# weimengmeng1999/AdapterSIS

Hardware: AMD Instinct MI355X
Metric: training images/sec, ViT-L/14 588^2 adapter fine-tune (higher is better)
Workload: dtype f16; 1 GPU; vit_large/14 frozen + CAViT/CACNN adapters (n_last_blocks=4) + FeatureDecoder, 588x588, batch 12/GPU, reference_exact train.py step (fwd + decoder bwd + all-reduce + SGD), random-init weights; global_batch=12, image_size=588, parallelism=dp1, split_precision_convs=True, split_attn_out=False, precise_level=0, fold_attn_scale=True, fused_qkv=False, dead_cacnn_elided=True, c1_elided=True, ln_fold=True, mx_conv=True, mx_dense=True, conv_halo=True, fuse_cls_up=False, skipped_optimizer_steps=0

## Files before the change

adaptersis_amd/_lib.py:

```python
from __future__ import annotations

import ctypes as C
import os

_HERE = os.path.dirname(os.path.abspath(__file__))
LIB_PATH = os.path.join(_HERE, "lib", "libasis_hip.so")

ASIS_F16, ASIS_BF16, ASIS_F32 = 0, 1, 2
ASIS_EINVAL, ASIS_ELAUNCH = -1, -2
ACT_NONE, ACT_GELU, ACT_RELU, ACT_SILU_MUL, ACT_GELU_GRAD = 0, 1, 2, 3, 4


class AsisError(RuntimeError):
    pass


class GemmDesc(C.Structure):
    _fields_ = [
        ("A", C.c_void_p), ("B", C.c_void_p), ("C", C.c_void_p),
        ("lda", C.c_int64), ("ldb", C.c_int64), ("ldc", C.c_int64),
        ("strideA", C.c_int64), ("strideB", C.c_int64), ("strideC", C.c_int64),
        ("batch", C.c_int32), ("M", C.c_int32), ("N", C.c_int32), ("K", C.c_int32),
        ("bias_n", C.c_void_p), ("bias_m", C.c_void_p), ("scale_n", C.c_void_p), ("res", C.c_void_p),
        ("ldr", C.c_int64), ("strideR", C.c_int64),
        ("act", C.c_int32), ("out_f32", C.c_int32), ("dtype", C.c_int32),
        ("conv", C.c_int32),
        ("B_", C.c_int32), ("H", C.c_int32), ("W", C.c_int32), ("Cin", C.c_int32), ("OH", C.c_int32),
        ("OW", C.c_int32), ("KH", C.c_int32), ("KW", C.c_int32), ("stride", C.c_int32), ("pad", C.c_int32),
        ("stats", C.c_void_p),
        ("A_lo", C.c_void_p), ("B_lo", C.c_void_p),
        ("aux", C.c_void_p), ("ld_aux", C.c_int64),
        ("ksplit", C.c_int32),
        ("mx_amax_a", C.c_void_p), ("mx_amax_b", C.c_void_p),
        ("C_lo", C.c_void_p), ("rowstats", C.c_void_p), ("res16", C.c_void_p), ("res16_lo", C.c_void_p), ("ldr16", C.c_int64),
        ("ln_mr", C.c_void_p), ("ln_cs", C.c_void_p), ("ln_cols", C.c_int32),
    ]


class WgradDesc(C.Structure):
    _fields_ = [
        ("dy", C.c_void_p), ("x", C.c_void_p), ("out", C.c_void_p),
        ("ld_dy", C.c_int64), ("P", C.c_int64),
        ("dtype", C.c_int32), ("Cout", C.c_int32), ("CoP", C.c_int32), ("Cin", C.c_int32),
        ("B_", C.c_int32), ("H", C.c_int32), ("W", C.c_int32), ("OH", C.c_int32), ("OW", C.c_int32),
        ("KH", C.c_int32), ("KW", C.c_int32), ("stride", C.c_int32), ("pad", C.c_int32),
        ("splits", C.c_int32), ("k_per_split", C.c_int64),
    ]


_lib = None


def lib() -> C.CDLL:
    global _lib
    if _lib is not None:
        return _lib
    if not os.path.exists(LIB_PATH):
        raise AsisError(
            f"{LIB_PATH} is missing: build it with `python -m adaptersis_amd.build` "
            "(hipcc --offload-arch=gfx950). adaptersis_amd has no fallback path.")
    _lib = C.CDLL(LIB_PATH)
    _declare(_lib)
    _lib.asis_last_error.restype = _lib.asis_gemm_form_name.restype = C.c_char_p
    _lib.asis_lovasz_scratch_bytes.restype = _lib.asis_hardpixel_scratch_bytes.restype = C.c_int64
    _lib.asis_surface_quantile_scratch_bytes.restype = C.c_int64
    return _lib


_vp, _i, _i64, _f, _d = C.c_void_p, C.c_int, C.c_int64, C.c_float, C.c_double
SIGNATURES = {
    "asis_version": [],
    "asis_device_count": [],
    "asis_gemm": [_vp, C.POINTER(GemmDesc)],
    "asis_gemm_tiles_m": [_i],
    "asis_gemm_plan": [C.POINTER(GemmDesc), C.POINTER(_i), C.POINTER(_i), C.POINTER(_i), C.POINTER(_i)],
    "asis_gemm_form_name": [_i],
    "asis_absmax_f32": [_vp, _vp, _i64, _i, _i64, _vp, _i],
    "asis_bn_relu_absmax": [_vp, _vp, _vp, _vp, _i64, _i, _i, _vp],
    "asis_absmax_16": [_vp, _i, _vp, _i64, _i, _i64, _vp],
    "asis_conv3x3_halo_mx_tiles": [_i, _i, _i],
    "asis_conv3x3_halo_mx": [_vp, _i, _vp, _vp, _vp, _vp, _vp, _vp, _vp, _vp, _vp, _i, _i, _i, _i, _i],
    "asis_mx_from_pair": [_vp, _i, _vp, _vp, _i64, _vp, _i64, _i64, _i, _vp, _i],
    "asis_bn_relu_upsample_mx": [_vp, _i, _vp, _vp, _vp, _vp, _vp, _vp, _i, _i, _i, _i, _i],
    "asis_pack_conv_weight_mx": [_vp, _i, _vp, _vp, _i, _i, _i, _i, _i, _i64, _vp],
    "asis_pack_conv_weight_pair": [_vp, _i, _vp, _vp, _vp, _i, _i, _i, _i, _i, _i64, _vp],
    "asis_decoder_input_mx": [_vp, _i, _vp, _i64, _vp, _i64, _vp, _i64, _vp, _vp, _vp, _i, _i, _i, _i, _i, _i],
    "asis_ln_stats_finalize": [_vp, _vp, _i64, _i, _i, _f, _vp],
    "asis_split_stats": [_vp, _i, _vp, _i64, _vp, _vp, _i64, _vp, _i64, _i, _f],
    "asis_gemm_set_option": [C.c_char_p, _i],
    "asis_layernorm": [_vp, _i, _vp, _i64, _vp, _vp, _f, _vp, _i64, _i, _i64, _i],
    "asis_layernorm_mx": [_vp, _i, _vp, _i64, _vp, _vp, _f, _vp, _vp, _i64, _vp, _i64, _i],
    "asis_attention_fwd_seg": [_vp, _i, _vp, _vp, _i64, _vp, _i64, _vp, _i64, _i, _i, _i, _i, _i, _f, _vp],
    "asis_attention_fwd_split": [_vp, _i, _vp, _vp, _i64, _vp, _i64, _vp, _vp, _i64, _i, _i, _i, _i, _i, _f, _vp],
    "asis_attention_fwd_prescaled": [_vp, _i, _vp, _vp, _i64, _vp, _i64, _vp, _vp, _i64, _i, _i, _i, _i, _i, _vp],
    "asis_attention_fwd_qkv": [_vp, _i, _vp, _vp, _vp, _i64, _vp, _vp, _i64, _i, _i, _i, _i, _i, _f, _i, _vp],
    "asis_attention_fwd_qkv_mx": [_vp, _i, _vp, _vp, _vp, _i64, _vp, _vp, _i64, _i, _i, _i, _i, _i, _f, _i, _vp, _vp],
    "asis_attention_fwd_lse": [_vp, _i, _vp, _vp, _i64, _vp, _i64, _vp, _i64, _i, _i, _i, _f, _vp],
    "asis_transpose_tokens": [_vp, _i, _vp, _i64, _vp, _i64, _i, _i, _i],
    "asis_attention_bwd_rows": [_vp, _i, _vp, _vp, _vp, _i64, _vp, _i64, _vp, _i64, _vp, _vp, _vp, _vp, _vp, _i64, _i, _i, _i, _i,
                                _i, _f],
    "asis_msda_bwd": [_vp, _i, _vp, _vp, _i64, _vp, _vp, _vp, _vp, _vp, _vp, _i, _i, _i, _i, _i, _i, _i],
    "asis_msda_vgrad_cap": [_i, _i, _i],
    "asis_msda_value_grad": [_vp, _i, _vp, _i64, _vp, _vp, _vp, _vp, _vp, _vp, _vp, _vp, _vp, _i, _i, _i, _i, _i, _i, _i],
    "asis_msda_sampling_matrix": [_vp, _i, _vp, _i64, _vp, _vp, _vp, _vp, _i64, _i, _i, _i, _i, _i, _i],
    "asis_dwconv_bwd_nblk": [_i64],
    "asis_dwconv_gelu_bwd": [_vp, _i, _vp, _vp, _vp, _vp, _vp, _i, _vp, _vp, _vp, _vp, _i, _i, _i],
    "asis_rowblock_nblk": [_i64],
    "asis_layernorm_bwd": [_vp, _vp, _i64, _vp, _i64, _vp, _f, _vp, _i64, _vp, _i64, _vp, _i64, _i],
    "asis_gelu16": [_vp, _i, _vp, _vp, _vp, _i64],
    "asis_gelu_split": [_vp, _i, _vp, _vp, _vp, _i64],
    "asis_cast_colsum": [_vp, _i, _vp, _i64, _vp, _i64, _f, _vp, _i64, _i],
    "asis_layernorm_gather": [_vp, _i, _vp, _i64, _vp, _vp, _f, _vp, _i64, _vp, _i, _i, _i64, _i],
    "asis_scaled_index_add": [_vp, _vp, _i64, _vp, _i64, _vp, _i64, _vp, _i, _i, _i64, _i],
    "asis_gather_cast_colsum": [_vp, _i, _vp, _i64, _vp, _i64, _vp, _vp, _i, _i, _i64, _i],
    "asis_layernorm_bwd_scatter": [_vp, _vp, _i64, _vp, _i64, _vp, _f, _vp, _i64, _vp, _i64, _vp, _vp, _i, _i, _i64, _i64, _i],
    "asis_swiglu_bwd": [_vp, _i, _vp, _vp, _vp, _i64, _i],
    "asis_colsum": [_vp, _i, _vp, _i64, _vp, _i64, _i],
    "asis_ls_linear_finish": [_vp, _vp, _vp, _vp, _vp, _vp, _f, _vp, _vp, _vp, _i, _i],
    "asis_attention_fwd": [_vp, _i, _vp, _vp, _i64, _vp, _i64, _vp, _i64, _i, _i, _i, _f],
    "asis_im2col_patch": [_vp, _i, _vp, _i, _i, _i, _i, _vp, _i64],
    "asis_im2col_patch_split": [_vp, _i, _vp, _i, _i, _i, _i, _vp, _vp, _i64],
    "asis_cast_pad": [_vp, _i, _vp, _i64, _vp, _i64, _i64, _i, _f, _i],
    "asis_add_cls_pos": [_vp, _vp, _vp, _vp, _vp, _i, _i, _i],
    "asis_msda_fwd": [_vp, _i, _vp, _vp, _i64, _vp, _vp, _vp, _vp, _i, _i, _i, _i, _i, _i, _i],
    "asis_msda_fwd_split": [_vp, _i, _vp, _vp, _i64, _vp, _vp, _vp, _vp, _vp, _i, _i, _i, _i, _i, _i, _i],
    "asis_dwconv_gelu": [_vp, _i, _vp, _vp, _vp, _vp, _vp, _i, _vp, _i, _i, _i],
    "asis_conv3x3_c3": [_vp, _vp, _vp, _vp, _i, _i, _i, _i, _i, _i],
    "asis_conv3x3_smallcout_fwd": [_vp, _i, _vp, _vp, _vp, _vp, _vp, _i, _i, _i, _i, _i],
    "asis_conv3x3_smallcout_fwd_up": [_vp, _i, _vp, _vp, _vp, _vp, _vp, _vp, _i, _i, _i, _i, _i],
    "asis_conv3x3_smallcout_wgrad_up": [_vp, _i, _vp, _i, _vp, _vp, _vp, _vp, _i, _i, _i, _i, _i, _i],
    "asis_cls_lowres_nblk": [_i, _i, _i],
    "asis_cls_lowres_fwd": [_vp, _vp, _vp, _vp, _vp, _vp, _vp, _vp, _i, _i, _i, _i, _i],
    "asis_cls_lowres_bwd": [_vp, _i, _vp, _vp, _i, _vp, _vp, _vp, _vp, _vp, _vp, _vp, _vp, _vp, _i, _i, _i, _i, _i, _i],
    "asis_dgrad_lowres_nblk": [_i, _i, _i],
    "asis_dgrad_lowres_cap": [_i],
    "asis_dgrad_lowres_pack": [_vp, _i, _vp, _vp, _vp, _i, _i],
    "asis_dgrad_lowres": [_vp, _i, _vp, _vp, _vp, _vp, _vp, _vp, _vp, _vp, _vp, _vp, _vp, _i, _i, _i, _i, _i, _i],
    "asis_conv3x3_smallcout_dgrad": [_vp, _i, _vp, _vp, _i, _vp, _vp, _i, _i, _i, _i, _i],
    "asis_conv3x3_smallcout_wgrad": [_vp, _i, _vp, _i, _vp, _vp, _i, _i, _i, _i, _i, _i],
    "asis_colstats_nparts": [_i64],
    "asis_colstats": [_vp, _vp, _i64, _i, _vp],
    "asis_reduce_partials": [_vp, _vp, _i, _i, _vp],
    "asis_bn_finalize": [_vp, _vp, _d, _i, _vp, _vp, _f, _f, _vp, _vp, _vp, _vp, _vp, _vp, _vp],
    "asis_bn_eval_affine": [_vp, _vp, _vp, _vp, _vp, _f, _i, _vp, _vp],
    "asis_bn_act": [_vp, _i, _vp, _vp, _vp, _i, _vp, _vp, _i64, _i],
    "asis_bn_act_mx": [_vp, _i, _vp, _vp, _vp, _i, _vp, _vp, _vp, _i64, _i],
    "asis_bn_relu_maxpool": [_vp, _i, _vp, _vp, _vp, _vp, _vp, _i, _i, _i, _i],
    "asis_bn_relu_upsample": [_vp, _i, _vp, _vp, _vp, _vp, _vp, _i, _i, _i, _i, _i],
    "asis_pack_conv_weight": [_vp, _i, _vp, _vp, _i, _i, _i, _i, _i, _i64, _i],
    "asis_decoder_input": [_vp, _i, _vp, _i64, _vp, _i64, _vp, _i64, _vp, _vp, _i, _i, _i, _i, _i, _i],
    "asis_swiglu": [_vp, _i, _vp, _vp, _i64, _i],
    "asis_swiglu_split": [_vp, _i, _vp, _vp, _vp, _i64, _i],
    "asis_copy_channels": [_vp, _vp, _i64, _vp, _i64, _i64, _i64],
    "asis_add_f32": [_vp, _vp, _vp, _vp, _i64, _i, _i64, _i64, _i64],
    "asis_maxpool2_fwd": [_vp, _i, _vp, _vp, _vp, _vp, _vp, _i, _i, _i, _i],
    "asis_maxpool2_bwd": [_vp, _vp, _vp, _vp, _i, _i, _i, _i],
    "asis_cls_l2norm": [_vp, _vp, _vp, _vp, _i, _i, _i, _i],
    "asis_cls_l2norm_bwd": [_vp, _vp, _vp, _vp, _vp, _i, _i, _i, _i],
    "asis_mask_logits_fwd": [_vp, _vp, _vp, _vp, _vp, _f, _vp, _vp, _vp, _i, _i, _i, _i],
    "asis_mask_logits_nblk": [_i, _i],
    "asis_mask_logits_bwd": [_vp, _vp, _vp, _vp, _vp, _vp, _vp, _f, _vp, _vp, _vp, _i, _i, _i, _i],
    "asis_mask_dchat": [_vp, _vp, _vp, _vp, _vp, _i, _i, _i, _i],
    "asis_nearest_add_relu": [_vp, _i, _vp, _vp, _vp, _vp, _vp, _vp, _i, _i, _i, _i, _i, _i],
    "asis_nearest_sum": [_vp, _vp, _vp, _vp, _vp, _i, _i, _i, _i, _i, _i],
    "asis_convt2x2_scatter": [_vp, _i, _vp, _vp, _vp, _i, _i, _i, _i, _i, _i, _i, _i, _i, _i],
    "asis_convt2x2_gather": [_vp, _i, _vp, _vp, _vp, _i, _i, _i, _i, _i, _i, _i, _i, _i, _i],
    "asis_convt2x2_bias_nblk": [_i64],
    "asis_conv1x1_dgrad_small": [_vp, _i, _vp, _vp, _i64, _vp, _vp, _i64, _i, _i],
    "asis_convt2x2_bias_grad": [_vp, _vp, _vp, _i, _i, _i, _i, _i, _i, _i, _i, _i, _i],
    "asis_dice_nblk": [_i, _i],
    "asis_seg_loss_fwd": [_vp, _vp, _vp, _vp, _i, _i, _i, _i, _i, _i, _i, _i, _f, _i, _f, _vp, _vp, _vp, _vp],
    "asis_seg_loss_bwd": [_vp, _vp, _vp, _vp, _vp, _i, _i, _i, _i, _i, _i, _i, _i, _i, _vp],
    "asis_dice_fwd": [_vp, _vp, _vp, _i, _i, _i, _i, _i, _i, _i, _f, _i, _f, _vp, _vp, _vp, _vp],
    "asis_dice_bwd": [_vp, _vp, _vp, _vp, _i, _i, _i, _i, _i, _i, _i, _vp],
    "asis_ce_acc_nblk": [_i64],
    "asis_ce_acc_counts": [_vp, _vp, _vp, _vp, _i, _i, _i, _i, _i, _i, _vp, _vp],
    "asis_ce_acc": [_vp, _vp, _vp, _vp, _i, _i, _i, _i, _i, _i, _vp],
    "asis_resize_bilinear_fwd": [_vp, _vp, _i, _i, _i, _i, _i, _i, _vp],
    "asis_resize_bwd_nblk": [_i64],
    "asis_resize_bilinear_bwd": [_vp, _i, _vp, _i, _i, _i, _i, _i, _i, _i, _vp, _vp, _vp],
    "asis_reduce_rows": [_vp, _vp, _i, _i, _f, _vp],
    "asis_lovasz_tile": [],
    "asis_lovasz_scratch_bytes": [_i64, _i],
    "asis_lovasz_softmax": [_vp, _vp, _vp] + [_i] * 8 + [_f, _i] + [_vp] * 6,
    "asis_hardpixel_tile": [],
    "asis_hardpixel_scratch_bytes": [_i64],
    "asis_hardpixel_loss": [_vp] * 4 + [_i] * 8 + [_f, _f, _i64, _i, _f, _i] + [_vp] * 5,
    "asis_ew_blocks": [_i64],
    "asis_bn_bwd_nblk": [_i64, _i],
    "asis_maxpool_bn_relu_bwd": [_vp, _vp, _vp, _vp, _vp, _vp, _vp, _vp, _vp, _i, _i, _i, _i],
    "asis_dilate2": [_vp, _i, _vp, _vp, _vp, _vp, _i, _i, _i, _i, _i, _i],
    "asis_upsample_bn_relu_bwd": [_vp, _vp, _vp, _vp, _vp, _vp, _vp, _vp, _vp, _i, _i, _i, _i, _i],
    "asis_bn_bwd_apply": [_vp, _i, _vp, _vp, _vp, _vp, _vp, _vp, _vp, _d, _vp, _vp, _vp, _i64, _i],
    "asis_bn_bwd_apply_mx": [_vp, _i, _vp, _vp, _vp, _vp, _vp, _vp, _vp, _d, _vp, _vp, _vp, _vp, _i64, _i],
    "asis_bn_bwd_absmax": [_vp, _vp, _vp, _vp, _vp, _vp, _vp, _vp, _d, _vp, _i64, _i],
    "asis_wgrad_splits": [_i64, _i, _i],
    "asis_wgrad": [_vp, C.POINTER(WgradDesc)],
    "asis_conv3x3_wgrad_halo_nblk": [_i, _i, _i, _i, _i],
    "asis_conv3x3_wgrad_halo": [_vp, _i, _vp, _i64, _vp, _vp, _i, _i, _i, _i, _i, _i],
    "asis_lora_down": [_vp, _i, _vp, _i64, _i, _i, _i, _i, _vp, _vp, _i64, _i64],
    "asis_lora_wgrad_nblk": [_i64, _i],
    "asis_lora_wgrad": [_vp, _i, _vp, _i64, _vp, _i64, _i, _i, _i, _i, _vp, _i, _i64],
    "asis_sgd_momentum": [_vp, _vp, _vp, _vp, _i64, _f, _f, _f, _f, _i],
    "asis_augment": [_vp] * 13 + [_i, _i],
    "asis_augment_geo_u8": [_vp] * 12 + [_i, _i],
    "asis_clahe": [_vp] * 13 + [_i, _i, _i],
    "asis_nonrigid_map": [_vp] * 7 + [_i] + [_vp] * 3 + [_i, _i],
    "asis_nonrigid_remap": [_vp] * 6 + [_i, _i],
    "asis_frame_resize": [_vp] * 5 + [_i, _vp, _vp, _i] + [_vp] * 6 + [_i] * 5,
    "asis_predict_mask": [_vp, _vp] + [_i] * 6 + [_vp] * 9,
    "asis_predict_mask_views": [_vp] * 5 + [_i] * 5 + [_vp] * 10,
    "asis_predict_mask_tiles": [_vp] * 6 + [_i] * 4 + [_f] + [_i] * 4 + [_vp] * 10,
    "asis_surface_stats": [_vp] * 5 + [_i] * 6 + [_vp, _i] + [_vp] * 6 + [_i],
    "asis_surface_quantile_scratch_bytes": [_i, _i, _i],
    "asis_surface_quantiles": [_vp] * 4 + [_i] * 7 + [_vp, _i] + [_vp] * 3,
    "asis_dropout_f32": [_vp, _vp, _vp, _vp, _i64, C.c_uint64, _i, _f, _f, _vp, _i],
    "asis_dropout_t16": [_vp, _i, _vp, _vp, _i64, C.c_uint64, _i, _f, _i],
    "asis_dropout_mask": [_vp, _vp, _i64, C.c_uint64, _i, _f],
    "asis_softmax_dropout_fwd": [_vp, _i, _vp, _vp, _vp, _i64, _i, _i, _f, C.c_uint64, _i, _f],
    "asis_softmax_dropout_bwd": [_vp, _i, _vp, _vp, _vp, _vp, _i64, _i, _i, _f, C.c_uint64, _i, _f],
    "asis_grad_guard": [_vp, _vp, _i64, _vp, _i],
    "asis_sgd_momentum_guarded": [_vp, _vp, _vp, _vp, _i64, _f, _f, _f, _f, _i, _vp, _i],
    "asis_grad_sumsq_blocks": [_i64],
    "asis_grad_sumsq": [_vp, _vp, _i64, _vp],
    "asis_adamw_prepare": [_vp, _vp, _i, _vp, _vp, _f, _f, _d, _d],
    "asis_adamw_step": [_vp, _vp, _vp, _vp, _vp, _i64, _vp, _vp, _vp, _i, _d, _d, _d, _d, _f, _vp, _vp],
    "asis_scale_f32": [_vp, _vp, _i64, _f],
    "asis_zero": [_vp, _vp, _i64],
    "asis_grad_pack_bf16": [_vp, _vp, _i64, _vp],
    "asis_grad_unpack_bf16": [_vp, _vp, _i64, _vp],
}


def _declare(l: C.CDLL) -> None:
    for name, argtypes in SIGNATURES.items():
        fn = getattr(l, name)
        fn.argtypes = argtypes
        fn.restype = C.c_int


def check(rc: int, what: str = "") -> None:
    if rc == 0:
        return
# ... 5 lines not shown
```

adaptersis_amd/backbones/adapter_blocks.py:

```python
from __future__ import annotations

from functools import partial

import torch
import torch.nn as nn

from .. import config, ops
from ..dinov2.layers.blocks import _Packed
from .ops.modules import MSDeformAttn
from .ops.modules.ms_deform_attn import prepare_msda_geometry


def get_reference_points(spatial_shapes, device):
    reference_points_list = []
    for lvl, (H_, W_) in enumerate(spatial_shapes):
        ref_y, ref_x = torch.meshgrid(
            torch.linspace(0.5, H_ - 0.5, H_, dtype=torch.float32, device=device),
            torch.linspace(0.5, W_ - 0.5, W_, dtype=torch.float32, device=device), indexing="ij")
        ref_y = ref_y.reshape(-1)[None] / H_
        ref_x = ref_x.reshape(-1)[None] / W_
        reference_points_list.append(torch.stack((ref_x, ref_y), -1))
    reference_points = torch.cat(reference_points_list, 1)
    return reference_points[:, :, None]


def deform_inputs(x, patch_size, cnn_shapes=None):
    bs, c, h, w = x.shape
    if cnn_shapes is None:
        cnn_shapes = [(h // 8, w // 8), (h // 16, w // 16), (h // 32, w // 32)]
    cnn_shapes = [tuple(int(v) for v in s) for s in cnn_shapes]
    spatial_shapes = torch.as_tensor(cnn_shapes, dtype=torch.long, device=x.device)
    level_start_index = torch.cat((spatial_shapes.new_zeros((1,)), spatial_shapes.prod(1).cumsum(0)[:-1]))
    reference_points = get_reference_points([(h // patch_size, w // patch_size)], x.device)
    deform_inputs1 = [reference_points, spatial_shapes, level_start_index]
    spatial_shapes = torch.as_tensor([(h // patch_size, w // patch_size)], dtype=torch.long, device=x.device)
    level_start_index = torch.cat((spatial_shapes.new_zeros((1,)), spatial_shapes.prod(1).cumsum(0)[:-1]))
    reference_points = get_reference_points(cnn_shapes, x.device)
    deform_inputs2 = [reference_points, spatial_shapes, level_start_index]
    return deform_inputs1, deform_inputs2


class DWConv(nn.Module):

    def __init__(self, dim=768):
        super().__init__()
        self.dwconv = nn.Conv2d(dim, dim, 3, 1, 1, bias=True, groups=dim)


class ConvFFN(_Packed):

    def __init__(self, in_features, hidden_features=None, out_features=None, act_layer=nn.GELU, drop=0.0):
        super().__init__()
        if drop:
            raise ValueError("dropout is 0 on the AdapterSIS path (train.py:108)")
        out_features = out_features or in_features
        hidden_features = hidden_features or in_features
        if hidden_features % 8:
            raise ValueError("ConvFFN hidden width must be a multiple of 8")
        self.fc1 = nn.Linear(in_features, hidden_features)
        self.dwconv = DWConv(hidden_features)
        self.act = act_layer()
        self.fc2 = nn.Linear(hidden_features, out_features)

    def forward16(self, n16, res, B, Ntok, grids):
        dt = config.operand_dtype
        dev = n16.device
        hid = self.fc1.out_features
        h = ops.gemm(n16, self._w16("fc1", self.fc1.weight), out_f32=True, bias_n=self._f32("fc1_b", self.fc1.bias))
        key = ("grids", tuple(grids), dev)
        if self._cache.get("gkey") != key:
            sizes = [a * b for a, b in grids]
            starts = [0]
            for s in sizes[:-1]:
                starts.append(starts[-1] + s)
            self._cache["gshapes"] = torch.tensor(grids, dtype=torch.int32, device=dev)
            self._cache["gstarts"] = torch.tensor(starts, dtype=torch.int32, device=dev)
            self._cache["gkey"] = key
        w9 = self._f32_fn("dw9", self.dwconv.dwconv.weight, lambda p: p.reshape(hid, 9).t().contiguous().float())
        g = ops.dwconv_gelu(h.view(B, Ntok, hid), w9, self._f32("dwb", self.dwconv.dwconv.bias),
                            self._cache["gshapes"], self._cache["gstarts"], dt)
        return ops.gemm(g.view(B * Ntok, hid), self._w16("fc2", self.fc2.weight), out_f32=True,
                        bias_n=self._f32("fc2_b", self.fc2.bias), res=res)

    def _grid_tensors(self, grids, dev):
        key = ("grids", tuple(grids), dev)
        if self._cache.get("gkey") != key:
            sizes = [a * b for a, b in grids]
            starts = [0]
            for s in sizes[:-1]:
                starts.append(starts[-1] + s)
            self._cache["gshapes"] = torch.tensor(grids, dtype=torch.int32, device=dev)
            self._cache["gstarts"] = torch.tensor(starts, dtype=torch.int32, device=dev)
            self._cache["gkey"] = key
        return self._cache["gshapes"], self._cache["gstarts"]

    def forward16_train(self, n16, res, B, Ntok, grids):
        dt = config.operand_dtype
        hid = self.fc1.out_features
        h = ops.gemm(n16, self._w16("fc1", self.fc1.weight), out_f32=True, bias_n=self._f32("fc1_b", self.fc1.bias))
        gsh, gst = self._grid_tensors(grids, n16.device)
        w9 = self._f32_fn("dw9", self.dwconv.dwconv.weight, lambda p: p.reshape(hid, 9).t().contiguous().float())
        g = ops.dwconv_gelu(h.view(B, Ntok, hid), w9, self._f32("dwb", self.dwconv.dwconv.bias), gsh, gst, dt)
        out = ops.gemm(g.view(B * Ntok, hid), self._w16("fc2", self.fc2.weight), out_f32=True,
                       bias_n=self._f32("fc2_b", self.fc2.bias), res=res)
        return out, (n16, h, g, B, Ntok, tuple(grids))

    def backward16(self, saved, dout, inv_scale, grads, prefix):
        n16, h, g, B, Ntok, grids = saved
        dt = config.operand_dtype
        hid = self.fc1.out_features
        pre = prefix + "."
        d16, cs = ops.cast_colsum(dout, dt)
        self._linear_bwd(pre + "fc2", self.fc2, None, None, d16, cs, g.view(B * Ntok, hid), inv_scale, grads)
        dg = ops.gemm(d16, self._wT16("fc2T", self.fc2.weight), out_f32=True)
        gsh, gst = self._grid_tensors(grids, dout.device)
        w9 = self._f32_fn("dw9", self.dwconv.dwconv.weight, lambda p: p.reshape(hid, 9).t().contiguous().float())
        dh16, part = ops.dwconv_gelu_bwd(h.view(B, Ntok, hid), w9, self._f32("dwb", self.dwconv.dwconv.bias), gsh, gst,
                                         dg.view(B, Ntok, hid), dt)
        red = ops.reduce_rows(part.view(part.shape[0], 10 * hid), inv_scale).view(10, hid)
        grads[pre + "dwconv.dwconv.weight"].view(hid, 9).copy_(red[:9].t())
        grads[pre + "dwconv.dwconv.bias"].copy_(red[9])
        dh2 = dh16.view(B * Ntok, hid)
        self._linear_bwd(pre + "fc1", self.fc1, None, None, dh2, ops.colsum(dh2), n16, inv_scale, grads)
        return ops.gemm(dh2, self._wT16("fc1T", self.fc1.weight), out_f32=True)

    def _f32_fn(self, key, param, fn):
        from ..dinov2.layers.blocks import _pack
        return _pack(self._cache, key, param, fn)


class _AdapterBase(_Packed):
    def _ln16(self, name, x2d):
        ln = getattr(self, name)
        return ops.layernorm(x2d, self._f32(name + "_w", ln.weight), self._f32(name + "_b", ln.bias), ln.eps,
                             config.operand_dtype)

    def _ln_bwd(self, name, dy, x2d, inv_scale, grads, prefix, res=None):
        ln = getattr(self, name)
        D = x2d.shape[1]
        dx, part = ops.layernorm_bwd(dy, x2d, self._f32(name + "_w", ln.weight), ln.eps, res=res)
        red = ops.reduce_rows(part.view(part.shape[0], 2 * D), inv_scale)
        grads[f"{prefix}{name}.weight"].copy_(red[:D]); grads[f"{prefix}{name}.bias"].copy_(red[D:])
        return dx

    @staticmethod
    def _flat(x):
        B, N, D = x.shape
        x2 = x.reshape(B * N, D)
        if x2.dtype != torch.float32 or not x2.is_contiguous():
            x2 = x2.float().contiguous()
        return x2, B, N, D


class CACNN(_AdapterBase):
    def __init__(self, dim, num_heads=6, n_points=4, n_levels=1, deform_ratio=1.0, with_cffn=True, cffn_ratio=0.25,
                 drop=0.0, drop_path=0.0, norm_layer=partial(nn.LayerNorm, eps=1e-6), with_cp=False):
        super().__init__()
        if drop or drop_path:
            raise ValueError("drop / drop_path are 0 on the AdapterSIS path (train.py:108-109)")
        self.query_norm = norm_layer(dim)
        self.feat_norm = norm_layer(dim)
        self.attn = MSDeformAttn(d_model=dim, n_levels=n_levels, n_heads=num_heads, n_points=n_points, ratio=deform_ratio)
        self.with_cffn = with_cffn
        self.with_cp = with_cp
        if with_cffn:
            self.ffn = ConvFFN(in_features=dim, hidden_features=int(dim * cffn_ratio), drop=drop)
            self.ffn_norm = norm_layer(dim)
            self.drop_path = nn.Identity()

    def forward(self, query, reference_points, feat, spatial_shapes, level_start_index, H, W, grids=None):
        q2, B, Lq, D = self._flat(query)
        f2, _, Lin, _ = self._flat(feat)
        assert int((spatial_shapes[:, 0] * spatial_shapes[:, 1]).sum()) == Lin
        ref, shapes_i32, starts_i32 = prepare_msda_geometry(reference_points, spatial_shapes, level_start_index, Lq,
                                                            query.device)
        out = self.attn.forward16(self._ln16("query_norm", q2), self._ln16("feat_norm", f2), ref, shapes_i32,
                                  starts_i32, B, Lq, Lin, res=q2)
        if self.with_cffn:
            if grids is None:
                grids = [(H * 2 + 1, W * 2 + 1), (H, W), (H // 2, W // 2)]
            grids = [tuple(int(v) for v in g) for g in grids]
            if sum(a * b for a, b in grids) != Lq:
                raise ValueError(f"CACNN: token grids {grids} do not cover {Lq} tokens; pass grids= explicitly")
            out = self.ffn.forward16(self._ln16("ffn_norm", out), out, B, Lq, grids)
        return out.view(B, Lq, D)


    def forward16_train(self, c2, x2, g, B, Lq, Lin, grids):
        qn, fn = self._ln16("query_norm", c2), self._ln16("feat_norm", x2)
        out1, s_attn = self.attn.forward16_train(qn, fn, g["ref2"], g["shapes2"], g["starts2"], B, Lq, Lin, res=c2)
        s_ffn = None
        out = out1
        if self.with_cffn:
            out, s_ffn = self.ffn.forward16_train(self._ln16("ffn_norm", out1), out1, B, Lq, grids)
        return out, (c2, x2, out1, s_attn, s_ffn)

    def backward16(self, saved, dout, inv_scale, grads, prefix=""):
        c2, x2, out1, s_attn, s_ffn = saved
        pre = prefix + "." if prefix else ""
        d1 = dout
        if self.with_cffn:
            dn = self.ffn.backward16(s_ffn, dout, inv_scale, grads, pre + "ffn")
            d1 = self._ln_bwd("ffn_norm", dn, out1, inv_scale, grads, pre, res=dout)
        dq, dfeat = self.attn.backward16(s_attn, d1, inv_scale, grads, pre + "attn")
        dc = self._ln_bwd("query_norm", dq, c2, inv_scale, grads, pre, res=d1)
        dx = self._ln_bwd("feat_norm", dfeat, x2, inv_scale, grads, pre)
        return dc, dx


class CAViT(_AdapterBase):
    def __init__(self, dim, num_heads=6, n_points=4, n_levels=1, deform_ratio=1.0,
                 norm_layer=partial(nn.LayerNorm, eps=1e-6), init_values=0.0, with_cp=False):
        super().__init__()
        self.with_cp = with_cp
        self.query_norm = norm_layer(dim)
        self.feat_norm = norm_layer(dim)
        self.attn = MSDeformAttn(d_model=dim, n_levels=n_levels, n_heads=num_heads, n_points=n_points, ratio=deform_ratio)
        self.gamma = nn.Parameter(init_values * torch.ones((dim)), requires_grad=True)

    def forward(self, query, reference_points, feat, spatial_shapes, level_start_index):
        q2, B, Lq, D = self._flat(query)
        f2, _, Lin, _ = self._flat(feat)
        assert int((spatial_shapes[:, 0] * spatial_shapes[:, 1]).sum()) == Lin
        ref, shapes_i32, starts_i32 = prepare_msda_geometry(reference_points, spatial_shapes, level_start_index, Lq,
                                                            query.device)
        out = self.attn.forward16(self._ln16("query_norm", q2), self._ln16("feat_norm", f2), ref, shapes_i32,
                                  starts_i32, B, Lq, Lin, res=q2, scale_n=self._f32("gamma", self.gamma))
        return out.view(B, Lq, D)

    def forward16_train(self, x2, c2, g, B, Lq, Lin):
        qn, fn = self._ln16("query_norm", x2), self._ln16("feat_norm", c2)
        out, s_attn = self.attn.forward16_train(qn, fn, g["ref1"], g["shapes1"], g["starts1"], B, Lq, Lin, res=x2,
                                                scale_n=self._f32("gamma", self.gamma))
        return out, (x2, c2, s_attn)

    def backward16(self, saved, dout, inv_scale, grads, prefix=""):
        x2, c2, s_attn = saved
        pre = prefix + "." if prefix else ""
        dq, dfeat = self.attn.backward16(s_attn, dout, inv_scale, grads, pre + "attn", gamma=self.gamma,
                                         gamma_name=pre + "gamma")
        dx = self._ln_bwd("query_norm", dq, x2, inv_scale, grads, pre, res=dout)
        dc = self._ln_bwd("feat_norm", dfeat, c2, inv_scale, grads, pre)
        return dx, dc
```

adaptersis_amd/backbones/engines.py:

```python
from __future__ import annotations

import contextlib
import os
from typing import Dict, List, Optional, Sequence, Tuple

import torch
import torch.distributed as dist
from torch import nn

from .. import config, ops
from .. import lora as lora_mod
from ..dinov2.layers.blocks import _Packed, _pack, run_blocks
from ..droppath import DropPathSampler
from ..optim import SGD, AdamW, FlatBucket
from ..parallel import StageReducer, world_size
from .adapter_blocks import CACNN, CAViT, deform_inputs


class pre_vit(_Packed):

    def __init__(self, img_size=84, patch_size=14, in_chans=256, embed_dim=384, norm_layer=None, flatten_embedding=True):
        super().__init__()
        if norm_layer is not None:
            raise ValueError("pre_vit: norm_layer is never set in the reference")
        self.img_size, self.patch_size = img_size, patch_size
        self.patches_resolution = (img_size // patch_size, img_size // patch_size)
        self.num_patches = self.patches_resolution[0] * self.patches_resolution[1]
        self.in_chans, self.embed_dim, self.flatten_embedding = in_chans, embed_dim, flatten_embedding
        self.proj = nn.Conv2d(in_chans, embed_dim, kernel_size=patch_size, stride=patch_size)
        self.norm = nn.Identity()

    def forward(self, x):
        B, C, H, W = x.shape
        P = self.patch_size
        assert H % P == 0, f"Input image height {H} is not a multiple of patch height {P}"
        assert W % P == 0, f"Input image width {W} is not a multiple of patch width: {P}"
        dt = config.operand_dtype
        x16 = ops.cast_pad(x.permute(0, 2, 3, 1).contiguous().float().view(B * H * W, C), C, dt).view(B, H, W, C)
        w16 = _pack(self._cache, "w", self.proj.weight, lambda p: ops.pack_conv_weight(p.float().contiguous(), 0, dt))
        out = ops.conv_gemm(x16, w16, P, P, P, 0, bias_n=self._f32("b", self.proj.bias))
        out = out.view(B, (H // P) * (W // P), self.embed_dim)
        if not self.flatten_embedding:
            out = out.reshape(-1, H // P, W // P, self.embed_dim)
        return out


def _loss_scratch(engine, attr: str, need: int, device) -> torch.Tensor:
    scratch = getattr(engine, attr, None)
    if scratch is None or scratch.numel() < need or scratch.device != device:
        scratch = torch.empty((need,), device=device, dtype=torch.uint8)
        setattr(engine, attr, scratch)
    return scratch


def loss_and_dz(engine, logits: torch.Tensor, target: torch.Tensor, S: float):
    n_region, lmode, eps, n_ce = SegEngine.LOSSES[engine.loss_kind]
    if lmode not in (ops.LOSS_LOVASZ, ops.LOSS_TOPK, ops.LOSS_FOCAL):
        loss, coef, _ = ops.seg_loss_fwd(logits, target, n_region, lmode, eps, n_ce, None, S)
        return loss, ops.seg_loss_bwd(logits, target, coef, n_region, lmode, n_ce, None)
    if lmode != ops.LOSS_LOVASZ:
        N = target.numel()
        scratch = _loss_scratch(engine, "_hardpixel_scratch", ops.hardpixel_scratch_bytes(N), logits.device)
        if lmode == ops.LOSS_FOCAL:
            return ops.hardpixel_loss(logits, target, ops.HARDPIXEL_FOCAL, N, n_softmax=n_region,
                                      gamma=getattr(engine, "focal_gamma", 2.0), grad_scale=S, scratch=scratch)
        K = int(N * getattr(engine, "topk_percent", 10.0) / 100)
        if K < 1:
            raise ValueError(f"topk_percent selects no pixel of {N}")
        dz, dc = None, None
        if n_region:
            dc, coef, _ = ops.seg_loss_fwd(logits, target, n_region, ops.LOSS_SOFTDICE, eps, 0, None, S)
            dz = ops.seg_loss_bwd(logits, target, coef, n_region, ops.LOSS_SOFTDICE, 0, None)
        loss, dz = ops.hardpixel_loss(logits, target, ops.HARDPIXEL_CE, K, grad_scale=S, dz=dz, scratch=scratch)
        return (loss if dc is None else dc.add_(loss)), dz
    scratch = _loss_scratch(engine, "_lovasz_scratch", ops.lovasz_scratch_bytes(target.numel(), logits.shape[-1]), logits.device)
    dz, ce = None, None
    if n_ce:
        ce, coef, _ = ops.seg_loss_fwd(logits, target, 0, ops.LOSS_NONE, eps, n_ce, None, S)
        dz = ops.seg_loss_bwd(logits, target, coef, 0, ops.LOSS_NONE, n_ce, None)
    loss, _, dz = ops.lovasz_softmax(logits, target, n_region, "mean", S, dz=dz, scratch=scratch)
    return (loss if ce is None else ce.add_(loss)), dz


class SegEngine(nn.Module):

    LOSSES = {
        "dice": (2, ops.LOSS_DICE, 10e-20, 0),
        "iou": (2, ops.LOSS_IOU, 1e-6, 0),
        "softdice": (1, ops.LOSS_SOFTDICE, 1.0, 0),
        "dc_and_ce": (1, ops.LOSS_SOFTDICE, 1.0, 2),
        "tversky": (1, ops.LOSS_TVERSKY, 1.0, 0),
        "ce_dc": (1, ops.LOSS_DICE, 10e-20, 1),
        "lovasz": (1, ops.LOSS_LOVASZ, 0.0, 0),
        "ce_lovasz": (1, ops.LOSS_LOVASZ, 0.0, 1),
        "topk": (0, ops.LOSS_TOPK, 0.0, 0),
        "dc_and_topk": (1, ops.LOSS_TOPK, 1.0, 0),
        "focal": (1, ops.LOSS_FOCAL, 0.0, 0),
    }

    def __init__(self, model, backbone_encoder, cross_vit: CAViT, cross_cnn: CACNN, seg_decoder, *,
                 n_last_blocks: int = 4, num_classes: int = 2, lr: float = 0.01, momentum: float = 0.99,
                 weight_decay: float = 3e-5, mode: str = "reference_exact", process_group=None, loss: str = "dice",
                 train_encoder: bool = False, train_backbone: bool = False, optimize_backbone: bool = False,
                 blocks_per_bucket: int = 4, grad_compress: Optional[str] = None, optimizer: str = "sgd",
                 betas=(0.9, 0.999), eps: float = 1e-8, clip_grad: Optional[float] = None, no_decay: bool = True,
                 layer_decay: Optional[float] = None, topk_percent: float = 10.0, focal_gamma: float = 2.0,
                 drop_path_seed: int = 0, lora_rank: Optional[int] = None, lora_alpha: Optional[float] = None):
        super().__init__()
        if grad_compress is None:
            grad_compress = os.environ.get("ASIS_GRAD_COMPRESS", "bf16").lower()
        if grad_compress in ("", "0", "none", "off", "fp32"):
            grad_compress = None
        if mode not in ("reference_exact", "train_adapters"):
            raise ValueError("mode must be 'reference_exact' or 'train_adapters'")
        if loss not in self.LOSSES:
            raise ValueError(f"loss must be one of {sorted(self.LOSSES)}")
        self.loss_kind = loss
        if not 0.0 < topk_percent <= 100.0:
            raise ValueError("topk_percent must be in (0, 100]")
        if focal_gamma < 0.0:
            raise ValueError("focal_gamma must be >= 0")
        self.topk_percent, self.focal_gamma = float(topk_percent), float(focal_gamma)
        self.is_mla = type(seg_decoder).__name__ == "DecoderMLA"
        self.stream_only = type(seg_decoder).__name__ == "UNet"
        self.model, self.backbone_encoder = model, backbone_encoder
        self.cross_vit, self.cross_cnn, self.seg_decoder = cross_vit, cross_cnn, seg_decoder
        self.n_last_blocks, self.num_classes, self.mode = n_last_blocks, num_classes, mode
        self.patch = model.patch_size
        self.heads = model.num_heads
        self.process_group = process_group
        if train_encoder and mode != "train_adapters":
            raise ValueError("train_encoder needs mode='train_adapters'")
        self.train_encoder = train_encoder
        frozen = list(model.parameters()) + ([] if train_encoder else list(backbone_encoder.parameters()))
        if mode == "reference_exact":
            frozen += list(cross_vit.parameters()) + list(cross_cnn.parameters())
        for p in frozen:
            p.requires_grad_(False)
        order = list(seg_decoder.GRAD_ORDER)
        named = dict(seg_decoder.named_parameters())
        ordered = [(n, named[n]) for pre in order for n in named if n.startswith(pre + ".")]
        assert len(ordered) == len(named)
        self.bucket = FlatBucket(ordered)
        self.stage_ranges = [self.bucket.range_of([n for n in named if n.startswith(pre + ".")]) for pre in order]
        buckets = [self.bucket]
        self.adapter_bucket = None
        if mode == "train_adapters":
            if type(seg_decoder).__name__ not in ("FeatureDecoder", "DecoderSETR", "UNet", "DecoderMLA"):
                raise NotImplementedError("train_adapters is built for the train.py adapter flow (FeatureDecoder / UNet heads) and "
                                          "the train_mla.py flow (DecoderMLA)")
            if self.is_mla and train_backbone:
                raise NotImplementedError("the train_mla.py flow trains decoder + adapters (+ encoder); the unfrozen backbone "
                                          "(BASELINE config 4) is the train.py adapter flow")
            for p in list(cross_vit.parameters()) + list(cross_cnn.parameters()):
                p.requires_grad_(True)
            named_a = [("cross_vit." + n, p) for n, p in cross_vit.named_parameters()] + \
                      [("cross_cnn." + n, p) for n, p in cross_cnn.named_parameters()]
            self.adapter_bucket = FlatBucket(named_a)
            self.adapter_reducer = StageReducer(self.adapter_bucket.grad, [(0, self.adapter_bucket.numel)], process_group)
            buckets.append(self.adapter_bucket)
            self.encoder_bucket = None
            if train_encoder:
                for p in backbone_encoder.parameters():
                    p.requires_grad_(True)
                self.encoder_bucket = FlatBucket([("backbone_encoder." + n, p) for n, p in backbone_encoder.named_parameters()])
                self.encoder_reducer = StageReducer(self.encoder_bucket.grad, [(0, self.encoder_bucket.numel)], process_group)
                buckets.append(self.encoder_bucket)
        self.train_backbone = bool(train_backbone)
        self.split_attn_out = config.split_attn_out_policy if config.split_attn_out_policy is not None else \
            bool(self.stream_only or self.is_mla or train_backbone)
        self.precise_level = config.precise_level_policy if config.precise_level_policy is not None else \
            (2 if (self.is_mla and len(model.blocks) >= 40) else 0)
        all_parts = frozenset(("qkv", "proj", "fc1", "fc2"))
        self.precise_parts = config.precise_parts_policy if config.precise_parts_policy is not None else \
            (frozenset(("proj", "fc1")) if (config.precise_level_policy is None and self.precise_level == 2) else all_parts)
        self.vit_bucket = None
        self.lora = self.lora_bucket = None
        if lora_rank is None and lora_alpha is not None:
            raise ValueError("lora_alpha needs lora_rank")
        if lora_rank is not None:
            lora_mod.check_engine_args(mode=mode, train_backbone=train_backbone, optimize_backbone=optimize_backbone,
                                       layer_decay=layer_decay, is_mla=self.is_mla, model=model, rank=lora_rank)
            self.lora = lora_mod.LoRA(model, lora_rank, lora_alpha)
            self.lora_bucket = FlatBucket(list(self.lora.named_parameters()))
            self.vit_reducer = StageReducer(self.lora_bucket.grad, [(0, self.lora_bucket.numel)], process_group)
            self._fire_at = [0]
            buckets.append(self.lora_bucket)
        elif train_backbone:
            if mode != "train_adapters":
                raise ValueError("train_backbone needs mode='train_adapters' (the unfrozen variant of the adapter flow)")
            self.vit_bucket, self.vit_reducer, self._fire_at = make_vit_bucket(model, blocks_per_bucket, process_group,
                                                                               momentum=optimize_backbone,
                                                                               min_first_blocks=n_last_blocks,
                                                                               compress=grad_compress)
            if optimize_backbone:
                buckets.append(self.vit_bucket)
        if layer_decay is not None and not (train_backbone and optimize_backbone):
            raise ValueError("layer_decay scales the learning rates of the ViT blocks: it needs train_backbone and optimize_backbone")
        self.drop_path = make_drop_path_sampler(model, drop_path_seed, process_group)
        if self.drop_path is not None and not train_backbone:
            raise ValueError("drop_path_rate drops samples in the training forward of the ViT blocks: it needs train_backbone")
        self.optimizer = make_optimizer(optimizer, buckets, lr=lr, momentum=momentum, weight_decay=weight_decay, betas=betas, eps=eps,
                                        clip_grad=clip_grad, no_decay=no_decay, depth=len(model.blocks),
                                        layer_decay=[layer_decay if b is self.vit_bucket else None for b in buckets])
        self.reducer = StageReducer(self.bucket.grad, self.stage_ranges, process_group)
        self._geom = {}

    def _geometry(self, H, W, shapes, dev):
        key = (H, W, tuple(shapes), dev)
        g = self._geom.get(key)
        if g is None:
            d1, d2 = deform_inputs(torch.zeros(1, 3, H, W), self.patch, shapes)
            g = {"ref1": d1[0][0, :, 0, :].contiguous().to(dev), "shapes1": d1[1].to(torch.int32).to(dev),
                 "starts1": d1[2].to(torch.int32).to(dev), "ref2": d2[0][0, :, 0, :].contiguous().to(dev),
                 "shapes2": d2[1].to(torch.int32).to(dev), "starts2": d2[2].to(torch.int32).to(dev)}
            self._geom = {key: g}
        return g

    def _encoder_on_side_stream(self, inp: torch.Tensor):
        main = torch.cuda.current_stream()
        if getattr(self, "_enc_stream", None) is None:
            self._enc_stream = torch.cuda.Stream()
        side = self._enc_stream
        side.wait_stream(main)
        with torch.cuda.stream(side):
            _, c, shapes = self.backbone_encoder.forward_tokens(inp, need_c1=not config.elide_c1)
            done = torch.cuda.Event()
            done.record(side)
        c.record_stream(main)
        return c, shapes, done

    def _trunk_dual(self, xcat: torch.Tensor, Ra: int, blocks, segs) -> torch.Tensor:
        main = torch.cuda.current_stream()
        nper = 2 if config.trunk_streams >= 4 and min(b for b, _ in segs) >= 2 else 1
        if getattr(self, "_dual_streams", None) is None or len(self._dual_streams) != 2 * nper:
            self._dual_streams = tuple(torch.cuda.Stream() for _ in range(2 * nper))
        parts = []
        r0 = 0
        for (B, N) in segs:
            cuts = [0, B] if nper == 1 else [0, B // 2, B]
            for a, b in zip(cuts[:-1], cuts[1:]):
                parts.append((slice(r0 + a * N, r0 + b * N), [(b - a, N)]))
            r0 += B * N
        xs = []
        for st, (sl, _) in zip(self._dual_streams, parts):
            st.wait_stream(main)
            xcat.record_stream(st)
            xs.append(xcat[sl])
        nblk = len(blocks)
        for bi, blk in enumerate(blocks):
            for i, (st, (_, sg)) in enumerate(zip(self._dual_streams, parts)):
                with torch.cuda.stream(st):
                    R_i = xs[i][0].shape[0] if isinstance(xs[i], tuple) else xs[i].shape[0]
                    if blk.fold_ok(R_i, sg):
                        xs[i] = blk.forward_rows_fold(xs[i], sg, planes_out=bi + 1 < nblk and blocks[bi + 1].fold_ok(R_i, sg))
                    else:
                        xs[i] = blk.forward_rows(xs[i], sg)
        for st, x in zip(self._dual_streams, xs):
            main.wait_stream(st)
            x.record_stream(main)
        return torch.cat(xs, 0)

    def _cavit(self, x2, c2, g, B, Lq, Lin):
        cv = self.cross_vit
        return cv.attn.forward16(cv._ln16("query_norm", x2), cv._ln16("feat_norm", c2), g["ref1"], g["shapes1"],
                                 g["starts1"], B, Lq, Lin, res=x2, scale_n=cv._f32("gamma", cv.gamma))

    def _cacnn(self, c2, x2, g, B, Lq, Lin, grids):
        cn = self.cross_cnn
        out = cn.attn.forward16(cn._ln16("query_norm", c2), cn._ln16("feat_norm", x2), g["ref2"], g["shapes2"],
                                g["starts2"], B, Lq, Lin, res=c2)
        return cn.ffn.forward16(cn._ln16("ffn_norm", out), out, B, Lq, grids) if cn.with_cffn else out

    @torch.no_grad()
    def features(self, inp: torch.Tensor, taps: Optional[dict] = None, adapter_saves: Optional[list] = None):
        config.split_attn_out = self.split_attn_out
        config.precise_level = self.precise_level
        config.precise_parts = self.precise_parts
        m = self.model
        B, _, H, W = inp.shape
        inp = inp.float().contiguous()
        D = m.embed_dim
        h, w = H // self.patch, W // self.patch
        N = h * w
        nb = len(m.blocks)
        nl = self.n_last_blocks
        enc_done = None
        if self.train_encoder and adapter_saves is not None:
            c, shapes, esaved = self.backbone_encoder.forward_tokens_train(inp)
            self._esaved = (esaved, shapes)
        elif config.encoder_stream and inp.is_cuda:
            c, shapes, enc_done = self._encoder_on_side_stream(inp)
        else:
            _, c, shapes = self.backbone_encoder.forward_tokens(inp, need_c1=not config.elide_c1)
        c_orig = c
        Lc = c.shape[1]
        g = self._geometry(H, W, shapes, inp.device)
        Ra, Rb = B * (N + 1), B * N
        segs = [(B, N + 1), (B, N)]
        xcat = torch.empty((Ra + Rb, D), device=inp.device, dtype=torch.float32)
        tokens, _ = m.patch_embed.tokens(inp, out=xcat[Ra:])
        if not config.share_patch_embed:
            tokens, _ = m.patch_embed.tokens(inp)
        pos = m._pos_for(N, H, W)
        ops.add_cls_pos(tokens, m.cls_token.detach().reshape(-1).float().contiguous(),
                        pos.detach().reshape(-1, D).float().contiguous(), out=xcat[:Ra].view(B, N + 1, D))
        feats = []
        trunk = list(m.blocks[: nb - (nl - 1)])
        if config.dual_stream and inp.is_cuda and getattr(self, "_dual_warm", False) and nb - nl == len(trunk) - 1:
            xcat = self._trunk_dual(xcat, Ra, trunk, segs)
            feats.append(m._final_norm(xcat[:Ra].view(B, N + 1, D))[:, 1:])
            trunk = []
        self._dual_warm = True
        if trunk:
            assert nb - nl == len(trunk) - 1
            xcat = run_blocks(trunk, xcat, segs)
            feats.append(m._final_norm(xcat[:Ra].view(B, N + 1, D))[:, 1:])
        if enc_done is not None:
            torch.cuda.current_stream().wait_event(enc_done)
        if taps is not None:
            taps.update(c=c, x_b0=xcat[Ra:].view(B, N, D).clone(), shapes=shapes)
        c2d = c.view(B * Lc, D)
        train = self.mode == "train_adapters" and adapter_saves is not None
        for s in range(nl):
            bsaved = None
            if s > 0:
                blk = m.blocks[nb - (nl - 1) + s - 1]
                if train:
                    xa_s = blk.forward_rows(xcat[:Ra], [(B, N + 1)])
                    xb_s, bsaved = blk.forward_train(xcat[Ra:].view(B, N, D))
                    xcat = torch.cat([xa_s, xb_s.reshape(Rb, D)], 0)
                else:
                    xcat = run_blocks([blk], xcat, segs)
                feats.append(m._final_norm(xcat[:Ra].view(B, N + 1, D))[:, 1:])
            dead = s == nl - 1 and taps is None and config.elide_dead_cacnn
            if train:
                x2, s_cv = self.cross_vit.forward16_train(xcat[Ra:].clone(), c2d, g, B, N, Lc)
                s_cn = None
                if not dead:
                    c2d, s_cn = self.cross_cnn.forward16_train(c2d, x2, g, B, Lc, N, shapes)
                adapter_saves.append((bsaved, s_cv, s_cn))
            else:
                x2 = self._cavit(xcat[Ra:], c2d, g, B, N, Lc)
                if not dead:
                    c2d = self._cacnn(c2d, x2, g, B, Lc, N, shapes)
            x = ops.add_f32(x2.view(B, N, D), feats[s], out=xcat[Ra:].view(B, N, D))
        if taps is not None:
            taps.update(feats=feats)
        if self.stream_only:
            xs = x.reshape(B * N, D)
            hi = ops.cast_pad(xs, D, config.operand_dtype).view(B, h, w, D)
            lo = ops.cast_pad(xs, D, config.operand_dtype, part=1).view(B, h, w, D) if config.split_conv else None
            if taps is not None:
                taps.update(x_final=x, c_final=c2d.view(B, Lc, D), cat=hi)
            return hi, lo
        n4 = shapes[2][0] * shapes[2][1]
        d1 = getattr(self.seg_decoder, "decoder_1", None)
        mx = bool(config.mx_conv_on() and config.split_conv and d1 is not None and "d1" not in config.unsplit_layers and
                  ops.mx_conv_ok(B * h * w, 3 * D, d1[0].out_channels))
        cat = ops.decoder_input(x, c_orig[:, Lc - n4:], feats[-1], (h, w), shapes[2], config.operand_dtype,
                                config.split_conv, mx=mx)
        if not config.split_conv:
            cat = (cat, None)
        if taps is not None:
            taps.update(x_final=x, c_final=c2d.view(B, Lc, D), cat=cat[0])
        return cat

    @torch.no_grad()
    def features_mla(self, inp: torch.Tensor, taps: Optional[dict] = None, adapter_saves: Optional[list] = None):
        config.split_attn_out = self.split_attn_out
        config.precise_level = self.precise_level
        config.precise_parts = self.precise_parts
        m = self.model
        B, _, H, W = inp.shape
        inp = inp.float().contiguous()
        D = m.embed_dim
        h, w = H // self.patch, W // self.patch
        N = h * w
        nb = len(m.blocks)
        train = self.mode == "train_adapters" and adapter_saves is not None
        if train and self.train_encoder:
            c, shapes, esaved = self.backbone_encoder.forward_tokens_train(inp)
            self._esaved = (esaved, shapes)
        else:
            _, c, shapes = self.backbone_encoder.forward_tokens(inp, need_c1=not config.elide_c1)
        Lc = c.shape[1]
        g = self._geometry(H, W, shapes, inp.device)
        tokens = m.patch_embed(inp)
        if not config.share_patch_embed:
            m.patch_embed(inp)
        xa = ops.add_cls_pos(tokens, m.cls_token.detach().reshape(-1).float().contiguous(),
                             m._pos_for(N, H, W).detach().reshape(-1, D).float().contiguous())
        Ra = B * (N + 1)
        segs = [(B, N + 1), (B, N)]
        xcat = torch.cat([xa.view(Ra, D), tokens.reshape(B * N, D)], 0)
        xcat = run_blocks(list(m.blocks[: nb - 3]), xcat, segs)
        c2d = c.view(B * Lc, D)
        if train:
            x2, s_cv = self.cross_vit.forward16_train(xcat[Ra:].clone(), c2d, g, B, N, Lc)
            adapter_saves.append((None, s_cv, None))
        else:
            x2 = self._cavit(xcat[Ra:], c2d, g, B, N, Lc)
        outs = [x2]
        for j, bi in enumerate((nb - 3, nb - 2, nb - 2)):
            bsaved = None
            if train:
                if j < 2:
                    xa_s = m.blocks[bi].forward_rows(xcat[:Ra], [(B, N + 1)])
                    xb_s, bsaved = m.blocks[bi].forward_train(x2.view(B, N, D))
                    xcat = torch.cat([xa_s, xb_s.reshape(B * N, D)], 0)
                    x2 = xcat[Ra:]
                else:
                    xb_s, bsaved = m.blocks[bi].forward_train(x2.view(B, N, D))
                    x2 = xb_s.reshape(B * N, D)
            elif j < 2:
                xcat[Ra:].copy_(x2)
                xcat = m.blocks[bi].forward_rows(xcat, segs)
                x2 = xcat[Ra:]
            else:
                x2 = m.blocks[bi](x2.view(B, N, D)).view(B * N, D)
            if train:
                c2d, s_cn = self.cross_cnn.forward16_train(c2d, x2.contiguous(), g, B, Lc, N, shapes)
                x2, s_cv = self.cross_vit.forward16_train(x2.clone(), c2d, g, B, N, Lc)
                adapter_saves.append((bsaved, s_cv, s_cn))
            else:
                c2d = self._cacnn(c2d, x2, g, B, Lc, N, shapes)
                x2 = self._cavit(x2, c2d, g, B, N, Lc)
            outs.append(x2)
        xa = m.blocks[nb - 1](xcat[:Ra].view(B, N + 1, D))
        vit_last = m._final_norm(xa)[:, 1:]
        last = ops.add_f32(outs[3].view(B, N, D), vit_last)
        maps = [last.view(B * N, D), outs[2], outs[1], outs[0]]
        dt = config.operand_dtype
        res = []
        for t in maps:
            hi = ops.cast_pad(t, D, dt).view(B, h, w, D)
            lo = ops.cast_pad(t, D, dt, part=1).view(B, h, w, D) if config.split_conv else None
            res.append((hi, lo))
        if taps is not None:
            taps.update(mla_inputs=[t.view(B, N, D) for t in maps])
        return res

    @torch.no_grad()
    def train_step(self, inp: torch.Tensor, target: torch.Tensor, taps: Optional[dict] = None) -> torch.Tensor:
        dec = self.seg_decoder
        S = config.loss_scale
        asaves = None
        if self.is_mla:
            asaves = [] if self.mode == "train_adapters" else None
            logits, saved = dec._forward_core(self.features_mla(inp, taps, asaves), save=True, training=True)
        elif self.train_backbone:
            cat, e2e = self._features_e2e(inp, taps)
            if self.stream_only:
                logits, saved = dec._forward_core(cat[0], cat[1], save=True, training=True, need_input_grad=True)
            else:
                logits, saved = dec._forward_core(cat[0], cat[1], save=True, training=True)
        else:
            asaves = [] if self.mode == "train_adapters" else None
            cat = self.features(inp, taps, asaves)
            if self.stream_only and asaves is not None:
                logits, saved = dec._forward_core(cat[0], cat[1], save=True, training=True, need_input_grad=True)
            else:
                logits, saved = dec._forward_core(cat[0], cat[1], save=True, training=True)
        target = target.long().contiguous()
        loss, dz = loss_and_dz(self, logits, target, S)
        B, hh, ww, C = logits.shape
        r = ops.resize_bilinear_bwd(dz, hh, ww, config.operand_dtype, config.split_conv)
        d16, d_lo, bpart = r if config.split_conv else (r[0], None, r[1])
        world = world_size(self.process_group)
        inv = 1.0 / (S * world)
        self.reducer.begin()
        if self.mode == "train_adapters" and self.is_mla:
            dmaps = dec._backward_core(saved, d16, bpart, inv, self.bucket.views, stage_done=self.reducer.stage_done, d_lo=d_lo,
                                       need_input_grad=True)
            self.adapter_reducer.begin()
            dc0 = self._mla_adapter_backward(asaves, dmaps, inv)
            self.adapter_reducer.stage_done()
            if self.train_encoder:
                self.encoder_reducer.begin()
                self._encoder_backward(dc0, None, inv)
                self.encoder_reducer.stage_done()
                self.encoder_reducer.finish()
            self.adapter_reducer.finish()
        elif self.mode == "train_adapters":
            dcat = dec._backward_core(saved, d16, bpart, inv, self.bucket.views, stage_done=self.reducer.stage_done, d_lo=d_lo,
                                      need_input_grad=True)
            if self.stream_only and (self.train_backbone or self.train_encoder):
                Bq, hq, wq, Dq = dcat.shape
                full = ops.zeros((Bq, hq, wq, 3 * Dq), dcat.device, dcat.dtype)
                ops.copy_channels(dcat.view(-1, Dq), full.view(-1, 3 * Dq)[:, :Dq])
                dcat = full
            self.adapter_reducer.begin()
            if self.train_backbone:
                self.vit_reducer.begin()
                if self.train_encoder:
                    self.encoder_reducer.begin()
                self._e2e_backward(e2e, dcat, inv)
                self.vit_reducer.finish()
                if self.train_encoder:
                    self.encoder_reducer.finish()
                self.adapter_reducer.finish()
                self.reducer.finish()
                self.optimizer.step(1.0)
                if taps is not None:
                    taps.update(logits=logits, loss=loss)
                return loss.view(())
            dc0 = self._adapter_backward(asaves, dcat, inv)
            self.adapter_reducer.stage_done()
            if self.train_encoder:
                self.encoder_reducer.begin()
                self._encoder_backward(dc0, dcat, inv)
                self.encoder_reducer.stage_done()
                self.encoder_reducer.finish()
            self.adapter_reducer.finish()
        else:
            dec._backward_core(saved, d16, bpart, inv, self.bucket.views, stage_done=self.reducer.stage_done, d_lo=d_lo)
        self.reducer.finish()
        self.optimizer.step(1.0)
        if taps is not None:
            taps.update(logits=logits, loss=loss)
        return loss.view(())

    @torch.no_grad()
    def _features_e2e(self, inp: torch.Tensor, taps: Optional[dict] = None):
        config.split_attn_out = self.split_attn_out
        config.precise_level = self.precise_level
        config.precise_parts = self.precise_parts
        m = self.model
        B, _, H, W = inp.shape
        inp = inp.float().contiguous()
        D = m.embed_dim
        h, w = H // self.patch, W // self.patch
        N = h * w
        nb, nl = len(m.blocks), self.n_last_blocks
        if self.train_encoder:
            c, shapes, esaved = self.backbone_encoder.forward_tokens_train(inp)
            self._esaved = (esaved, shapes)
        else:
            _, c, shapes = self.backbone_encoder.forward_tokens(inp, need_c1=not config.elide_c1)
        c_orig = c
        Lc = c.shape[1]
        g = self._geometry(H, W, shapes, inp.device)
        tokens, a16 = m.patch_tokens_train(inp)
        xa = ops.add_cls_pos(tokens, m.cls_token.detach().reshape(-1).float().contiguous(),
                             m._pos_for(N, H, W).detach().reshape(-1, D).float().contiguous())
        Ra, Rb = B * (N + 1), B * N
        segs = [(B, N + 1), (B, N)]
        xcat = torch.cat([xa.view(Ra, D), tokens.reshape(Rb, D)], 0)
        bsaves, feats, fin, asaves = [], [], [], []
        keeps = self.drop_path.step(segs, inp.device) if self.drop_path is not None else [None] * nb
        blk_train = lambda j, xin: m.blocks[j].forward_train_rows(xin, segs) if keeps[j] is None else \
            m.blocks[j].forward_train_rows(xin, segs, keep=keeps[j])
        for i, blk in enumerate(m.blocks[: nb - (nl - 1)]):
            xcat, sv = blk_train(i, xcat)
            bsaves.append(sv)
            if i >= nb - nl:
                feats.append(m._final_norm(xcat[:Ra].view(B, N + 1, D))[:, 1:])
                fin.append(xcat)
        if taps is not None:
            taps.update(c=c, x_b0=xcat[Ra:].view(B, N, D).clone(), shapes=shapes)
        c2d = c.view(B * Lc, D)
        for s in range(nl):
            if s > 0:
                xcat, sv = blk_train(nb - nl + s, xcat)
                bsaves.append(sv)
                feats.append(m._final_norm(xcat[:Ra].view(B, N + 1, D))[:, 1:])
                fin.append(xcat)
            dead = s == nl - 1 and taps is None and config.elide_dead_cacnn
            x2, s_cv = self.cross_vit.forward16_train(xcat[Ra:].clone(), c2d, g, B, N, Lc)
            s_cn = None
            if not dead:
                c2d, s_cn = self.cross_cnn.forward16_train(c2d, x2, g, B, Lc, N, shapes)
            asaves.append((s_cv, s_cn))
            x = ops.add_f32(x2.view(B, N, D), feats[s], out=xcat[Ra:].view(B, N, D))
        if taps is not None:
            taps.update(feats=feats)
        if self.stream_only:
            xs = x.reshape(B * N, D)
            hi = ops.cast_pad(xs, D, config.operand_dtype).view(B, h, w, D)
            lo = ops.cast_pad(xs, D, config.operand_dtype, part=1).view(B, h, w, D) if config.split_conv else None
# ... 337 lines not shown
```

adaptersis_amd/config.py:

```python
import os

import torch

operand_dtype = torch.bfloat16 if os.environ.get("ASIS_OPERAND", "f16").lower() in ("bf16", "bfloat16") else torch.float16
loss_scale = float(os.environ.get("ASIS_LOSS_SCALE", 65536.0 if operand_dtype == torch.float16 else 1.0))


def set_operand_dtype(dt: torch.dtype) -> None:
    global operand_dtype
    if dt not in (torch.float16, torch.bfloat16):
        raise ValueError("operand dtype must be float16 or bfloat16")
    operand_dtype = dt

split_conv = os.environ.get("ASIS_SPLIT_CONV", "1") != "0"

precise_attention = os.environ.get("ASIS_PRECISE", "0") not in ("0", "")
fold_attn_scale = os.environ.get("ASIS_FOLD_SCALE", "1") not in ("0", "")
fused_qkv = os.environ.get("ASIS_FUSED_QKV", "0") not in ("0", "")

encoder_stream = os.environ.get("ASIS_ENC_STREAM", "1") not in ("0", "")

vt_stream = os.environ.get("ASIS_VT_STREAM", "1") not in ("0", "")

wgrad_stream = os.environ.get("ASIS_WGRAD_STREAM", "1") not in ("0", "")

unsplit_layers = set(filter(None, os.environ.get("ASIS_UNSPLIT", "").split(",")))

dual_stream = os.environ.get("ASIS_DUAL_STREAM", "1") not in ("0", "")

attn_rows = os.environ.get("ASIS_ATTN_ROWS", "1") != "0"

_so = os.environ.get("ASIS_SPLIT_O", "auto").lower()
split_attn_out_policy = None if _so == "auto" else (_so not in ("0", ""))
split_attn_out = bool(split_attn_out_policy)

_pl = os.environ.get("ASIS_PRECISE_LEVEL", "auto").lower() or "auto"
precise_level_policy = None if _pl == "auto" else int(_pl)
precise_level = int(precise_level_policy or 0)
_pa = os.environ.get("ASIS_PRECISE_ADAPTERS", "auto").lower() or "auto"


def precise_adapters_on() -> bool:
    if _pa != "auto":
        return _pa not in ("0", "")
    return operand_dtype == torch.bfloat16 and precise_level >= 2


_pp = os.environ.get("ASIS_PRECISE_PARTS", "auto").lower() or "auto"
precise_parts_policy = None if _pp == "auto" else frozenset(filter(None, _pp.replace("w12", "fc1").replace("w3", "fc2").split(",")))
precise_parts = precise_parts_policy if precise_parts_policy is not None else frozenset(("qkv", "proj", "fc1", "fc2"))
trunk_streams = int(os.environ.get("ASIS_TRUNK_STREAMS", "2") or 2)

elide_dead_cacnn = os.environ.get("ASIS_ELIDE_DEAD_CACNN", "1") not in ("0", "")
elide_c1 = os.environ.get("ASIS_ELIDE_C1", "1") not in ("0", "")
share_patch_embed = os.environ.get("ASIS_SHARE_PATCH_EMBED", "1") not in ("0", "")

ln_fold = os.environ.get("ASIS_LN_FOLD", "1") not in ("0", "")

_mx = os.environ.get("ASIS_MX_CONV", "1")
mx_conv_all = _mx == "2"
mx_conv = _mx not in ("0", "")


def mx_conv_on() -> bool:
    return mx_conv and (mx_conv_all or operand_dtype == torch.float16)


mx_dense = os.environ.get("ASIS_MX_DENSE", "1") not in ("0", "")


def mx_dense_on() -> bool:
    return mx_dense and operand_dtype == torch.float16

_DGRAD_LOWRES_ALL = ("d2", "d3", "d4")


def parse_dgrad_lowres(v: str) -> frozenset:
    v = (v or "").strip().lower()
    if v in ("", "0"):
        return frozenset()
    if v == "1":
        return frozenset(_DGRAD_LOWRES_ALL)
    keys = [k.strip() for k in v.split(",") if k.strip()]
    bad = [k for k in keys if k not in _DGRAD_LOWRES_ALL]
    if bad:
        raise ValueError(f"ASIS_DGRAD_LOWRES={v!r}: expected 0, 1 or a list of {', '.join(_DGRAD_LOWRES_ALL)} (unknown: {', '.join(bad)})")
    return frozenset(keys)


dgrad_lowres = parse_dgrad_lowres(os.environ.get("ASIS_DGRAD_LOWRES", "1"))
```

adaptersis_amd/csrc/core.hip:

```cpp
#include <stdarg.h>

#include "asis_common.h"

static thread_local char g_err[512] = "";

extern "C" void asis_set_error_(const char* fmt, ...) {
  va_list ap;
  va_start(ap, fmt);
  vsnprintf(g_err, sizeof(g_err), fmt, ap);
  va_end(ap);
}

extern "C" const char* asis_last_error(void) { return g_err; }
extern "C" int asis_version(void) { return 100; }

extern "C" int asis_device_count(void) {
  int n = 0;
  hipError_t e = hipGetDeviceCount(&n);
  if (e != hipSuccess) {
    asis_set_error_("hipGetDeviceCount: %s", hipGetErrorString(e));
    (void)hipGetLastError();
    return ASIS_ELAUNCH;
  }
  return n;
}
```

adaptersis_amd/csrc/norm.hip:

```cpp
#include "asis_common.h"
#include "row_routines.h"

namespace {

template <typename T, bool OUT_F32>
__global__ __launch_bounds__(256) void layernorm_kernel(const float* __restrict__ x, int64_t ldx,
                                                        const float* __restrict__ w, const float* __restrict__ b,
                                                        float eps, void* __restrict__ y, int64_t ldy, int64_t rows,
                                                        int D) {
  const int lane = threadIdx.x & 63;
  const int64_t row = (int64_t)blockIdx.x * 4 + (threadIdx.x >> 6);
  if (row >= rows) return;
  if (OUT_F32) ln_row<T, true>(x + row * ldx, w, b, eps, reinterpret_cast<float*>(y) + row * ldy, D, lane);
  else ln_row<T, false>(x + row * ldx, w, b, eps, reinterpret_cast<T*>(y) + row * ldy, D, lane);
}

template <typename T, bool OUT_F32, int NCH, int RPW>
__global__ __launch_bounds__(256) void layernorm_fixed_kernel(const float* __restrict__ x, int64_t ldx,
                                                              const float* __restrict__ w, const float* __restrict__ b,
                                                              float eps, void* __restrict__ y, int64_t ldy,
                                                              int64_t rows) {
  constexpr int D = 256 * NCH;
  const int lane = threadIdx.x & 63;
  const int64_t row0 = ((int64_t)blockIdx.x * 4 + (threadIdx.x >> 6)) * RPW;
  if (row0 >= rows) return;
  float4 v[RPW][NCH];
#pragma unroll
  for (int r = 0; r < RPW; ++r) {
    const int64_t row = row0 + r < rows ? row0 + r : rows - 1;
    const float4* xr = reinterpret_cast<const float4*>(x + row * ldx);
#pragma unroll
    for (int i = 0; i < NCH; ++i) v[r][i] = xr[lane + 64 * i];
  }
  float4 ww[NCH], bb[NCH];
#pragma unroll
  for (int i = 0; i < NCH; ++i) {
    ww[i] = reinterpret_cast<const float4*>(w)[lane + 64 * i];
    bb[i] = reinterpret_cast<const float4*>(b)[lane + 64 * i];
  }
  float mean[RPW], rstd[RPW];
#pragma unroll
  for (int r = 0; r < RPW; ++r) {
    float s = 0.f;
#pragma unroll
    for (int i = 0; i < NCH; ++i) s += (v[r][i].x + v[r][i].y) + (v[r][i].z + v[r][i].w);
    mean[r] = s;
  }
#pragma unroll
  for (int r = 0; r < RPW; ++r) mean[r] = wave_sum(mean[r]) / (float)D;
#pragma unroll
  for (int r = 0; r < RPW; ++r) {
    float q = 0.f;
#pragma unroll
    for (int i = 0; i < NCH; ++i) {
      const float a0 = v[r][i].x - mean[r], a1 = v[r][i].y - mean[r], a2 = v[r][i].z - mean[r],
                  a3 = v[r][i].w - mean[r];
      q += (a0 * a0 + a1 * a1) + (a2 * a2 + a3 * a3);
    }
    rstd[r] = q;
  }
#pragma unroll
  for (int r = 0; r < RPW; ++r) rstd[r] = 1.0f / sqrtf(wave_sum(rstd[r]) / (float)D + eps);
#pragma unroll
  for (int r = 0; r < RPW; ++r) {
    const int64_t row = row0 + r;
    if (row >= rows) break;
#pragma unroll
    for (int i = 0; i < NCH; ++i) {
      const int c = lane + 64 * i;
      const float o0 = (v[r][i].x - mean[r]) * rstd[r] * ww[i].x + bb[i].x;
      const float o1 = (v[r][i].y - mean[r]) * rstd[r] * ww[i].y + bb[i].y;
      const float o2 = (v[r][i].z - mean[r]) * rstd[r] * ww[i].z + bb[i].z;
      const float o3 = (v[r][i].w - mean[r]) * rstd[r] * ww[i].w + bb[i].w;
      if (OUT_F32) {
        reinterpret_cast<float4*>(reinterpret_cast<float*>(y) + row * ldy)[c] = make_float4(o0, o1, o2, o3);
      } else {
        uint2 p;
        p.x = pack2<T>(o0, o1);
        p.y = pack2<T>(o2, o3);
        reinterpret_cast<uint2*>(reinterpret_cast<T*>(y) + row * ldy)[c] = p;
      }
    }
  }
}

__global__ __launch_bounds__(256) void add_cls_pos_kernel(const float4* __restrict__ x, const float4* __restrict__ cls,
                                                          const float4* __restrict__ pos, float4* __restrict__ out,
                                                          int B, int N, int D4) {
  const int64_t total = (int64_t)B * (N + 1) * D4;
  for (int64_t i = (int64_t)blockIdx.x * blockDim.x + threadIdx.x; i < total; i += (int64_t)gridDim.x * blockDim.x) {
    const int c = (int)(i % D4);
    const int64_t r = i / D4;
    const int t = (int)(r % (N + 1));
    const int b = (int)(r / (N + 1));
    const float4 p = pos[(int64_t)t * D4 + c];
    const float4 a = (t == 0) ? cls[c] : x[((int64_t)b * N + (t - 1)) * D4 + c];
    out[i] = make_float4(a.x + p.x, a.y + p.y, a.z + p.z, a.w + p.w);
  }
}

template <typename T>
__global__ __launch_bounds__(256) void cast_pad_kernel(const float* __restrict__ src, int64_t ld_src,
                                                       T* __restrict__ dst, int64_t ld_dst, int64_t rows, int cols, float scale, int part) {
  const int cpr = (int)(ld_dst >> 3);
  const int64_t total = rows * cpr;
  for (int64_t i = (int64_t)blockIdx.x * blockDim.x + threadIdx.x; i < total; i += (int64_t)gridDim.x * blockDim.x) {
    const int64_t r = i / cpr;
    const int c0 = (int)(i - r * cpr) * 8;
    float f[8];
#pragma unroll
    for (int j = 0; j < 8; ++j) {
      f[j] = (c0 + j < cols) ? src[r * ld_src + c0 + j] * scale : 0.f;
      if (part) f[j] = lo_part<T>(f[j]);
    }
    uint4 p;
    p.x = pack2<T>(f[0], f[1]);
    p.y = pack2<T>(f[2], f[3]);
    p.z = pack2<T>(f[4], f[5]);
    p.w = pack2<T>(f[6], f[7]);
    *reinterpret_cast<uint4*>(dst + r * ld_dst + c0) = p;
  }
}

template <typename T>
__global__ __launch_bounds__(256) void im2col_patch_kernel(const float* __restrict__ img, int B, int Himg, int Wimg,
                                                           int P, T* __restrict__ out, int64_t ldk, T* __restrict__ out_lo) {
  const int gh = Himg / P, gw = Wimg / P;
  const int cpr = (int)(ldk >> 3);
  const int K = 3 * P * P;
  const int64_t total = (int64_t)B * gh * gw * cpr;
  for (int64_t i = (int64_t)blockIdx.x * blockDim.x + threadIdx.x; i < total; i += (int64_t)gridDim.x * blockDim.x) {
    const int64_t r = i / cpr;
    const int k0 = (int)(i - r * cpr) * 8;
    const int pw = (int)(r % gw);
    const int ph = (int)((r / gw) % gh);
    const int b = (int)(r / ((int64_t)gw * gh));
    float f[8];
#pragma unroll
    for (int j = 0; j < 8; ++j) {
      const int k = k0 + j;
      float v = 0.f;
      if (k < K) {
        const int c = k / (P * P);
        const int rem = k - c * P * P;
        const int ii = rem / P, jj = rem - ii * P;
        v = img[(((int64_t)b * 3 + c) * Himg + (ph * P + ii)) * Wimg + pw * P + jj];
      }
      f[j] = v;
    }
    uint4 p;
    p.x = pack2<T>(f[0], f[1]);
    p.y = pack2<T>(f[2], f[3]);
    p.z = pack2<T>(f[4], f[5]);
    p.w = pack2<T>(f[6], f[7]);
    *reinterpret_cast<uint4*>(out + r * ldk + k0) = p;
    if (out_lo) {
      uint4 q;
      q.x = pack2<T>(lo_part<T>(f[0]), lo_part<T>(f[1]));
      q.y = pack2<T>(lo_part<T>(f[2]), lo_part<T>(f[3]));
      q.z = pack2<T>(lo_part<T>(f[4]), lo_part<T>(f[5]));
      q.w = pack2<T>(lo_part<T>(f[6]), lo_part<T>(f[7]));
      *reinterpret_cast<uint4*>(out_lo + r * ldk + k0) = q;
    }
  }
}

}

template <int L>
__global__ __launch_bounds__(256) void ln_stats_finalize_kernel(const float* __restrict__ st, int64_t rows, int groups, int D,
                                                                float eps, float* __restrict__ mr) {
  const int64_t tid = (int64_t)blockIdx.x * blockDim.x + threadIdx.x;
  const int64_t row = tid / L;
  const int g = (int)(tid % L);
  const bool ok = row < rows && g < groups;
  const float2 v = ok ? reinterpret_cast<const float2*>(st)[row * groups + g] : make_float2(0.f, 0.f);
  float tot = v.x;
#pragma unroll
  for (int o = L / 2; o >= 1; o >>= 1) tot += __shfl_xor(tot, o, L);
  const float mean = tot / (float)D;
  const float n = (float)(g + 1 < groups ? 64 : D - 64 * (groups - 1));
  const float mg = v.x / n;
  const float dm = mg - mean;
  float m2 = ok ? fmaxf(v.y - v.x * mg, 0.f) + n * dm * dm : 0.f;
#pragma unroll
  for (int o = L / 2; o >= 1; o >>= 1) m2 += __shfl_xor(m2, o, L);
  if (g == 0 && row < rows) reinterpret_cast<float2*>(mr)[row] = make_float2(mean, 1.0f / sqrtf(m2 / (float)D + eps));
}

template <typename T>
__global__ __launch_bounds__(256) void split_stats_kernel(const float* __restrict__ x, int64_t ldx, T* __restrict__ hi, T* __restrict__ lo,
                                                          int64_t ld16, float* __restrict__ mr, int64_t rows, int D, float eps) {
  const int lane = threadIdx.x & 63;
  const int64_t row = (int64_t)blockIdx.x * 4 + (threadIdx.x >> 6);
  if (row >= rows) return;
  const int nchunk = D >> 2;
  const float4* xr = reinterpret_cast<const float4*>(x + row * ldx);
  float4 v[LN_MAXC];
  float s = 0.f;
#pragma unroll
  for (int i = 0; i < LN_MAXC; ++i) {
    const int c = lane + 64 * i;
    if (c < nchunk) {
      v[i] = xr[c];
      s += (v[i].x + v[i].y) + (v[i].z + v[i].w);
    }
  }
  const float mean = wave_sum(s) / (float)D;
  float q = 0.f;
#pragma unroll
  for (int i = 0; i < LN_MAXC; ++i) {
    const int c = lane + 64 * i;
    if (c < nchunk) {
      const float a0 = v[i].x - mean, a1 = v[i].y - mean, a2 = v[i].z - mean, a3 = v[i].w - mean;
      q += (a0 * a0 + a1 * a1) + (a2 * a2 + a3 * a3);
      uint2 ph, pl;
      ph.x = pack2<T>(v[i].x, v[i].y);
      ph.y = pack2<T>(v[i].z, v[i].w);
      pl.x = pack2<T>(lo_part<T>(v[i].x), lo_part<T>(v[i].y));
      pl.y = pack2<T>(lo_part<T>(v[i].z), lo_part<T>(v[i].w));
      reinterpret_cast<uint2*>(hi + row * ld16)[c] = ph;
      reinterpret_cast<uint2*>(lo + row * ld16)[c] = pl;
    }
  }
  const float rstd = 1.0f / sqrtf(wave_sum(q) / (float)D + eps);
  if (lane == 0) reinterpret_cast<float2*>(mr)[row] = make_float2(mean, rstd);
}

extern "C" int asis_ln_stats_finalize(void* stream, const float* rowstats, int64_t rows, int groups, int D, float eps, float* mr) {
  ASIS_REQUIRE(rowstats && mr && rows >= 0 && groups >= 1 && groups <= 32 && D > 64 * (groups - 1) && D <= 64 * groups,
               "asis_ln_stats_finalize: bad arguments (rows %ld, groups %d <= 32, D %d)", (long)rows, groups, D);
  if (rows == 0) return ASIS_OK;
  hipStream_t s = reinterpret_cast<hipStream_t>(stream);
  if (groups <= 16)
    hipLaunchKernelGGL((ln_stats_finalize_kernel<16>), dim3((unsigned)asis_cdiv(rows * 16, 256)), dim3(256), 0, s, rowstats, rows, groups, D,
                       eps, mr);
  else
    hipLaunchKernelGGL((ln_stats_finalize_kernel<32>), dim3((unsigned)asis_cdiv(rows * 32, 256)), dim3(256), 0, s, rowstats, rows, groups, D,
                       eps, mr);
  ASIS_CHECK_LAUNCH("asis_ln_stats_finalize");
  return ASIS_OK;
}

extern "C" int asis_split_stats(void* stream, int dtype, const float* x, int64_t ldx, void* hi, void* lo, int64_t ld16, float* mr,
                                int64_t rows, int D, float eps) {
  ASIS_REQUIRE(x && hi && lo && mr, "asis_split_stats: null pointer");
  ASIS_REQUIRE(D > 0 && D % 4 == 0 && D <= 256 * LN_MAXC, "asis_split_stats: D=%d must be a multiple of 4 and <= %d", D, 256 * LN_MAXC);
  ASIS_REQUIRE(ldx % 4 == 0 && ldx >= D && ld16 % 4 == 0 && ld16 >= D, "asis_split_stats: row strides must be multiples of 4 and >= D");
  ASIS_REQUIRE(asis_aligned16(x) && (((uintptr_t)hi) & 7) == 0 && (((uintptr_t)lo) & 7) == 0, "asis_split_stats: misaligned pointers");
  ASIS_DT_OK(dtype, "asis_split_stats");
  if (rows <= 0) return ASIS_OK;
  hipStream_t s = reinterpret_cast<hipStream_t>(stream);
  dim3 grid((unsigned)asis_cdiv(rows, 4)), block(256);
  if (int rc = asis_dispatch16(dtype, "asis_split_stats", [&](auto t) {
        using T = decltype(t);
        hipLaunchKernelGGL((split_stats_kernel<T>), grid, block, 0, s, x, ldx, static_cast<T*>(hi), static_cast<T*>(lo), ld16, mr, rows, D, eps);
      })) return rc;
  ASIS_CHECK_LAUNCH("asis_split_stats");
  return ASIS_OK;
}

extern "C" int asis_layernorm(void* stream, int dtype, const float* x, int64_t ldx, const float* w, const float* b,
                              float eps, void* y, int64_t ldy, int out_f32, int64_t rows, int D) {
  ASIS_REQUIRE(x && w && b && y, "asis_layernorm: null pointer");
  ASIS_REQUIRE(D > 0 && D % 4 == 0 && D <= 256 * LN_MAXC, "asis_layernorm: D=%d must be a multiple of 4 and <= %d", D,
               256 * LN_MAXC);
  ASIS_REQUIRE(ldx % 4 == 0 && ldx >= D && ldy % 4 == 0 && ldy >= D, "asis_layernorm: row strides must be multiples of 4 and >= D");
  ASIS_REQUIRE(asis_aligned16(x) && asis_aligned16(w) && asis_aligned16(b) && (((uintptr_t)y) & 7) == 0,
               "asis_layernorm: pointers must be 16-byte aligned");
  ASIS_DT_OK(dtype, "asis_layernorm");
  if (rows <= 0) return ASIS_OK;
  hipStream_t s = reinterpret_cast<hipStream_t>(stream);
  dim3 grid((unsigned)asis_cdiv(rows, 4)), block(256);
  static const int ln_fast = [] {
    const char* e = getenv("ASIS_LN_FAST");
    return e ? atoi(e) : 2;
  }();
  if (ln_fast && !out_f32 && (D == 768 || D == 1024 || D == 1536) && rows >= 4096) {
#define ASIS_LN_FIXED(T, NCH)                                                                                         \
  do {                                                                                                                \
    if (ln_fast == 1)                                                                                                 \
      hipLaunchKernelGGL((layernorm_fixed_kernel<T, false, NCH, 1>), grid, block, 0, s, x, ldx, w, b, eps, y, ldy,   \
                         rows);                                                                                       \
    else                                                                                                              \
      hipLaunchKernelGGL((layernorm_fixed_kernel<T, false, NCH, 2>), dim3((unsigned)asis_cdiv(rows, 8)), block, 0, s, \
                         x, ldx, w, b, eps, y, ldy, rows);                                                            \
  } while (0)
    if (int rc = asis_dispatch16(dtype, "asis_layernorm", [&](auto t) {
          using T = decltype(t);
          if (D == 768) ASIS_LN_FIXED(T, 3);
          else if (D == 1024) ASIS_LN_FIXED(T, 4);
          else ASIS_LN_FIXED(T, 6);
        })) return rc;
#undef ASIS_LN_FIXED
    ASIS_CHECK_LAUNCH("asis_layernorm");
    return ASIS_OK;
  }
  if (out_f32)
    hipLaunchKernelGGL((layernorm_kernel<f16, true>), grid, block, 0, s, x, ldx, w, b, eps, y, ldy, rows, D);
  else if (int rc = asis_dispatch16(dtype, "asis_layernorm", [&](auto t) {
             hipLaunchKernelGGL((layernorm_kernel<decltype(t), false>), grid, block, 0, s, x, ldx, w, b, eps, y, ldy, rows, D);
           })) return rc;
  ASIS_CHECK_LAUNCH("asis_layernorm");
  return ASIS_OK;
}

template <typename T>
__global__ __launch_bounds__(256) void layernorm_mx_kernel(const float* __restrict__ x, int64_t ldx, const float* __restrict__ w,
                                                           const float* __restrict__ b, float eps, T* __restrict__ y, T* __restrict__ y_mx,
                                                           int64_t ldy, const float* __restrict__ amax, int64_t rows, int D) {
  const int lane = threadIdx.x & 63;
  const int64_t row = (int64_t)blockIdx.x * 4 + (threadIdx.x >> 6);
  if (row >= rows) return;
  const MxScale sc = mx_scales<T>(*amax);
  const int nchunk = D >> 2;
  const float4* xr = reinterpret_cast<const float4*>(x + row * ldx);
  float4 v[LN_MAXC];
  float s = 0.f;
#pragma unroll
  for (int i = 0; i < LN_MAXC; ++i) {
    const int c = lane + 64 * i;
    if (c < nchunk) {
      v[i] = xr[c];
      s += (v[i].x + v[i].y) + (v[i].z + v[i].w);
    }
  }
  const float mean = wave_sum(s) / (float)D;
  float q = 0.f;
#pragma unroll
  for (int i = 0; i < LN_MAXC; ++i) {
    const int c = lane + 64 * i;
    if (c < nchunk) {
      const float a0 = v[i].x - mean, a1 = v[i].y - mean, a2 = v[i].z - mean, a3 = v[i].w - mean;
      q += (a0 * a0 + a1 * a1) + (a2 * a2 + a3 * a3);
    }
  }
  const float rstd = 1.0f / sqrtf(wave_sum(q) / (float)D + eps);
  const float4* w4 = reinterpret_cast<const float4*>(w);
  const float4* b4 = reinterpret_cast<const float4*>(b);
#pragma unroll
  for (int i = 0; i < LN_MAXC; ++i) {
    const int c = lane + 64 * i;
    if (c < nchunk) {
      const float4 ww = w4[c], bb = b4[c];
      const float o0 = (v[i].x - mean) * rstd * ww.x + bb.x;
      const float o1 = (v[i].y - mean) * rstd * ww.y + bb.y;
      const float o2 = (v[i].z - mean) * rstd * ww.z + bb.z;
      const float o3 = (v[i].w - mean) * rstd * ww.w + bb.w;
      uint2 p, m;
      p.x = pack2<T>(o0, o1);
      p.y = pack2<T>(o2, o3);
      m.x = mx_pack2<T>(o0, o1, sc, false);
      m.y = mx_pack2<T>(o2, o3, sc, false);
      reinterpret_cast<uint2*>(y + row * ldy)[c] = p;
      reinterpret_cast<uint2*>(y_mx + row * ldy)[c] = m;
    }
  }
}

extern "C" int asis_layernorm_mx(void* stream, int dtype, const float* x, int64_t ldx, const float* w, const float* b, float eps, void* y,
                                 void* y_mx, int64_t ldy, const float* amax, int64_t rows, int D) {
  ASIS_REQUIRE(x && w && b && y && y_mx && amax, "asis_layernorm_mx: null pointer");
  ASIS_REQUIRE(D > 0 && D % 4 == 0 && D <= 256 * LN_MAXC && ldx % 4 == 0 && ldy % 4 == 0 && ldx >= D && ldy >= D && asis_aligned16(x) &&
                   asis_aligned16(w) && asis_aligned16(b) && (reinterpret_cast<uintptr_t>(y) & 7) == 0 && (reinterpret_cast<uintptr_t>(y_mx) & 7) == 0,
               "asis_layernorm_mx: D=%d must be a multiple of 4 and <= %d, leading dimensions multiples of 4, pointers aligned", D, 256 * LN_MAXC);
  ASIS_DT_OK(dtype, "asis_layernorm_mx");
  if (rows == 0) return ASIS_OK;
  hipStream_t s = reinterpret_cast<hipStream_t>(stream);
  dim3 grid((unsigned)asis_cdiv(rows, 4)), block(256);
  if (int rc = asis_dispatch16(dtype, "asis_layernorm_mx", [&](auto t) {
        using T = decltype(t);
        hipLaunchKernelGGL((layernorm_mx_kernel<T>), grid, block, 0, s, x, ldx, w, b, eps, static_cast<T*>(y), static_cast<T*>(y_mx), ldy, amax, rows, D);
      })) return rc;
  ASIS_CHECK_LAUNCH("asis_layernorm_mx");
  return ASIS_OK;
}

extern "C" int asis_add_cls_pos(void* stream, const float* x, const float* cls, const float* pos, float* out, int B,
                                int N, int D) {
  ASIS_REQUIRE(x && cls && pos && out, "asis_add_cls_pos: null pointer");
  ASIS_REQUIRE(D % 4 == 0 && B > 0 && N > 0, "asis_add_cls_pos: bad shape B=%d N=%d D=%d", B, N, D);
  ASIS_REQUIRE(asis_aligned16(x) && asis_aligned16(cls) && asis_aligned16(pos) && asis_aligned16(out),
               "asis_add_cls_pos: pointers must be 16-byte aligned");
  const int64_t total = (int64_t)B * (N + 1) * (D / 4);
  hipLaunchKernelGGL(add_cls_pos_kernel, dim3(asis_grid(total, 256, 256 * 16)), dim3(256), 0, reinterpret_cast<hipStream_t>(stream),
                     reinterpret_cast<const float4*>(x), reinterpret_cast<const float4*>(cls),
                     reinterpret_cast<const float4*>(pos), reinterpret_cast<float4*>(out), B, N, D / 4);
  ASIS_CHECK_LAUNCH("asis_add_cls_pos");
  return ASIS_OK;
}

extern "C" int asis_cast_pad(void* stream, int dtype, const float* src, int64_t ld_src, void* dst, int64_t ld_dst,
                             int64_t rows, int cols, float scale, int part) {
  ASIS_REQUIRE(src && dst, "asis_cast_pad: null pointer");
  ASIS_REQUIRE(ld_dst % 8 == 0 && ld_dst >= cols && ld_src >= cols, "asis_cast_pad: bad leading dims");
  ASIS_REQUIRE(asis_aligned16(dst), "asis_cast_pad: dst must be 16-byte aligned");
  ASIS_DT_OK(dtype, "asis_cast_pad");
  if (rows <= 0) return ASIS_OK;
  const int64_t total = rows * (ld_dst / 8);
  hipStream_t s = reinterpret_cast<hipStream_t>(stream);
  if (int rc = asis_dispatch16(dtype, "asis_cast_pad", [&](auto t) {
        using T = decltype(t);
        hipLaunchKernelGGL((cast_pad_kernel<T>), dim3(asis_grid(total, 256, 256 * 16)), dim3(256), 0, s, src, ld_src,
                           static_cast<T*>(dst), ld_dst, rows, cols, scale, part);
      })) return rc;
  ASIS_CHECK_LAUNCH("asis_cast_pad");
  return ASIS_OK;
}

extern "C" int asis_im2col_patch_split(void* stream, int dtype, const float* img, int B, int Himg, int Wimg, int P, void* out,
                                       void* out_lo, int64_t ldk);
extern "C" int asis_im2col_patch(void* stream, int dtype, const float* img, int B, int Himg, int Wimg, int P, void* out,
                                 int64_t ldk) {
  return asis_im2col_patch_split(stream, dtype, img, B, Himg, Wimg, P, out, nullptr, ldk);
}

extern "C" int asis_im2col_patch_split(void* stream, int dtype, const float* img, int B, int Himg, int Wimg, int P, void* out,
                                       void* out_lo, int64_t ldk) {
  ASIS_REQUIRE(img && out, "asis_im2col_patch: null pointer");
  ASIS_REQUIRE(!out_lo || asis_aligned16(out_lo), "asis_im2col_patch: out_lo must be 16-byte aligned");
  ASIS_REQUIRE(P > 0 && Himg % P == 0 && Wimg % P == 0,
               "Input image size %dx%d is not a multiple of patch size %d", Himg, Wimg, P);
  ASIS_REQUIRE(ldk % 8 == 0 && ldk >= 3 * P * P, "asis_im2col_patch: ldk=%ld must be a multiple of 8 and >= 3*P*P", (long)ldk);
  ASIS_REQUIRE(asis_aligned16(out), "asis_im2col_patch: out must be 16-byte aligned");
  ASIS_DT_OK(dtype, "asis_im2col_patch");
  const int64_t total = (int64_t)B * (Himg / P) * (Wimg / P) * (ldk / 8);
  hipStream_t s = reinterpret_cast<hipStream_t>(stream);
  if (int rc = asis_dispatch16(dtype, "asis_im2col_patch", [&](auto t) {
        using T = decltype(t);
        hipLaunchKernelGGL((im2col_patch_kernel<T>), dim3(asis_grid(total, 256, 256 * 16)), dim3(256), 0, s, img, B, Himg, Wimg, P,
                           static_cast<T*>(out), ldk, static_cast<T*>(out_lo));
      })) return rc;
  ASIS_CHECK_LAUNCH("asis_im2col_patch");
  return ASIS_OK;
}
```

adaptersis_amd/csrc/row_routines.h:

```cpp
#pragma once
#include "asis_common.h"

namespace {

constexpr int LN_MAXC = 8;

struct RowIdentity {
  __device__ __forceinline__ int64_t operator()(int64_t r, float&) const { return r; }
};

struct RowGather {
  const int32_t* __restrict__ cpre;
  const int32_t* __restrict__ src;
  const float* __restrict__ alpha;
  int K;
  __device__ __forceinline__ int64_t operator()(int64_t r, float& scale) const {
    int lo = 0, hi = K - 1;
    while (lo < hi) {
      const int mid = (lo + hi + 1) >> 1;
      if (cpre[mid] <= r) lo = mid;
      else hi = mid - 1;
    }
    scale = alpha[lo];
    return (int64_t)src[lo] + (r - cpre[lo]);
  }
};

template <typename T, bool OUT_F32>
__device__ __forceinline__ void ln_row(const float* __restrict__ xrow, const float* __restrict__ w, const float* __restrict__ b,
                                       float eps, void* __restrict__ yrow, int D, int lane) {
  const int nchunk = D >> 2;
  const float4* xr = reinterpret_cast<const float4*>(xrow);
  float4 v[LN_MAXC];
  float s = 0.f;
#pragma unroll
  for (int i = 0; i < LN_MAXC; ++i) {
    const int c = lane + 64 * i;
    if (c < nchunk) {
      v[i] = xr[c];
      s += (v[i].x + v[i].y) + (v[i].z + v[i].w);
    }
  }
  const float mean = wave_sum(s) / (float)D;
  float q = 0.f;
#pragma unroll
  for (int i = 0; i < LN_MAXC; ++i) {
    const int c = lane + 64 * i;
    if (c < nchunk) {
      const float a0 = v[i].x - mean, a1 = v[i].y - mean, a2 = v[i].z - mean, a3 = v[i].w - mean;
      q += (a0 * a0 + a1 * a1) + (a2 * a2 + a3 * a3);
    }
  }
  const float rstd = 1.0f / sqrtf(wave_sum(q) / (float)D + eps);
  const float4* w4 = reinterpret_cast<const float4*>(w);
  const float4* b4 = reinterpret_cast<const float4*>(b);
#pragma unroll
  for (int i = 0; i < LN_MAXC; ++i) {
    const int c = lane + 64 * i;
    if (c < nchunk) {
      const float4 ww = w4[c], bb = b4[c];
      const float o0 = (v[i].x - mean) * rstd * ww.x + bb.x;
      const float o1 = (v[i].y - mean) * rstd * ww.y + bb.y;
      const float o2 = (v[i].z - mean) * rstd * ww.z + bb.z;
      const float o3 = (v[i].w - mean) * rstd * ww.w + bb.w;
      if (OUT_F32) {
        reinterpret_cast<float4*>(yrow)[c] = make_float4(o0, o1, o2, o3);
      } else {
        uint2 p;
        p.x = pack2<T>(o0, o1);
        p.y = pack2<T>(o2, o3);
        reinterpret_cast<uint2*>(yrow)[c] = p;
      }
    }
  }
}

template <int MAXC, typename Map>
__device__ __forceinline__ void ln_bwd_block(const float* __restrict__ dy, int64_t lddy, const float* __restrict__ x, int64_t ldx,
                                             const float* __restrict__ w, float eps, const float* __restrict__ res, int64_t ldr,
                                             float* __restrict__ dx, int64_t lddx, float* __restrict__ partial, int64_t rows, int D,
                                             int rows_per_block, const Map m) {
  __shared__ float red[3][2][MAXC * 64 * 4];
  const int lane = threadIdx.x & 63, wid = threadIdx.x >> 6;
  const int nchunk = D >> 2;
  const float4* w4 = reinterpret_cast<const float4*>(w);
  float4 gw[MAXC], gb[MAXC], ww[MAXC];
#pragma unroll
  for (int i = 0; i < MAXC; ++i) {
    gw[i] = gb[i] = make_float4(0.f, 0.f, 0.f, 0.f);
    const int c = lane + 64 * i;
    ww[i] = c < nchunk ? w4[c] : make_float4(0.f, 0.f, 0.f, 0.f);
  }
  const int64_t r0 = (int64_t)blockIdx.x * rows_per_block;
  int64_t r1 = r0 + rows_per_block;
  if (r1 > rows) r1 = rows;
  const float invD = 1.0f / (float)D;
  constexpr bool PF = MAXC <= 6;
  float4 v[MAXC], g[MAXC], e[MAXC];
  int64_t mrow = 0;
  auto load_row = [&](int64_t row, float4* vv, float4* gg, float4* ee) -> int64_t {
    float unused = 1.f;
    const int64_t sr = m(row, unused);
    const float4* xr = reinterpret_cast<const float4*>(x + sr * ldx);
    const float4* gr = reinterpret_cast<const float4*>(dy + row * lddy);
    const float4* rr = res ? reinterpret_cast<const float4*>(res + sr * ldr) : nullptr;
#pragma unroll
    for (int i = 0; i < MAXC; ++i) {
      const int c = lane + 64 * i;
      if (c < nchunk) {
        vv[i] = xr[c];
        gg[i] = gr[c];
        if (rr) ee[i] = rr[c];
      }
    }
    return sr;
  };
  int64_t row = r0 + wid;
  if constexpr (PF) {
    if (row < r1) mrow = load_row(row, v, g, e);
  }
  for (; row < r1; row += 4) {
    float4 vn[PF ? MAXC : 1], gn[PF ? MAXC : 1], en[PF ? MAXC : 1];
    int64_t mnext = 0;
    if constexpr (PF) {
      if (row + 4 < r1) mnext = load_row(row + 4, vn, gn, en);
    } else {
      mrow = load_row(row, v, g, e);
    }
    float s = 0.f;
#pragma unroll
    for (int i = 0; i < MAXC; ++i) {
      const int c = lane + 64 * i;
      if (c < nchunk) s += (v[i].x + v[i].y) + (v[i].z + v[i].w);
    }
    const float mean = wave_sum(s) * invD;
    float q = 0.f;
#pragma unroll
    for (int i = 0; i < MAXC; ++i) {
      const int c = lane + 64 * i;
      if (c < nchunk) {
        v[i].x -= mean; v[i].y -= mean; v[i].z -= mean; v[i].w -= mean;
        q += (v[i].x * v[i].x + v[i].y * v[i].y) + (v[i].z * v[i].z + v[i].w * v[i].w);
      }
    }
    const float rstd = 1.0f / sqrtf(wave_sum(q) * invD + eps);
    float a = 0.f, bq = 0.f;
#pragma unroll
    for (int i = 0; i < MAXC; ++i) {
      const int c = lane + 64 * i;
      if (c < nchunk) {
        v[i].x *= rstd; v[i].y *= rstd; v[i].z *= rstd; v[i].w *= rstd;
        gw[i].x += g[i].x * v[i].x; gw[i].y += g[i].y * v[i].y; gw[i].z += g[i].z * v[i].z; gw[i].w += g[i].w * v[i].w;
        gb[i].x += g[i].x; gb[i].y += g[i].y; gb[i].z += g[i].z; gb[i].w += g[i].w;
        g[i].x *= ww[i].x; g[i].y *= ww[i].y; g[i].z *= ww[i].z; g[i].w *= ww[i].w;
        a += (g[i].x + g[i].y) + (g[i].z + g[i].w);
        bq += (g[i].x * v[i].x + g[i].y * v[i].y) + (g[i].z * v[i].z + g[i].w * v[i].w);
      }
    }
    a = wave_sum(a) * invD;
    bq = wave_sum(bq) * invD;
    float4* o = reinterpret_cast<float4*>(dx + mrow * lddx);
#pragma unroll
    for (int i = 0; i < MAXC; ++i) {
      const int c = lane + 64 * i;
      if (c < nchunk) {
        float4 t;
        t.x = rstd * (g[i].x - a - v[i].x * bq);
        t.y = rstd * (g[i].y - a - v[i].y * bq);
        t.z = rstd * (g[i].z - a - v[i].z * bq);
        t.w = rstd * (g[i].w - a - v[i].w * bq);
        if (res) {
          t.x += e[i].x; t.y += e[i].y; t.z += e[i].z; t.w += e[i].w;
        }
        o[c] = t;
      }
    }
    if constexpr (PF) {
#pragma unroll
      for (int i = 0; i < MAXC; ++i) {
        v[i] = vn[i];
        g[i] = gn[i];
        e[i] = en[i];
      }
      mrow = mnext;
    }
  }
  if (wid > 0) {
#pragma unroll
    for (int i = 0; i < MAXC; ++i) {
      reinterpret_cast<float4*>(red[wid - 1][0])[i * 64 + lane] = gw[i];
      reinterpret_cast<float4*>(red[wid - 1][1])[i * 64 + lane] = gb[i];
    }
  }
  __syncthreads();
  if (wid == 0) {
    float4* pw = reinterpret_cast<float4*>(partial + ((int64_t)blockIdx.x * 2 + 0) * D);
    float4* pb = reinterpret_cast<float4*>(partial + ((int64_t)blockIdx.x * 2 + 1) * D);
#pragma unroll
    for (int i = 0; i < MAXC; ++i) {
      const int c = lane + 64 * i;
      if (c < nchunk) {
        float4 sw = gw[i], sb = gb[i];
#pragma unroll
        for (int k = 0; k < 3; ++k) {
          const float4 t = reinterpret_cast<const float4*>(red[k][0])[i * 64 + lane];
          const float4 u = reinterpret_cast<const float4*>(red[k][1])[i * 64 + lane];
          sw.x += t.x; sw.y += t.y; sw.z += t.z; sw.w += t.w;
          sb.x += u.x; sb.y += u.y; sb.z += u.z; sb.w += u.w;
        }
        pw[c] = sw;
        pb[c] = sb;
      }
    }
  }
}

template <typename T, int MAXC, bool SCALED_SUM, typename Map>
__device__ __forceinline__ void cast_colsum_block(const float* __restrict__ x, int64_t ldx, T* __restrict__ out, int64_t ldo,
                                                  float scale, float* __restrict__ partial, int64_t rows, int D, int rows_per_block,
// ... 56 lines not shown
```

adaptersis_amd/dinov2/layers/blocks.py:

```python
from __future__ import annotations

import contextlib
import math
import os
from typing import Callable, Optional, Tuple, Union

import torch
from torch import nn

from ... import config, droppath, ops
from ... import lora as _lora_mod
from ...packs import derived, tag_of


_VT_STREAMS = {}


def _vt_side_stream(device) -> "torch.cuda.Stream":
    key = (device.type, device.index)
    if key not in _VT_STREAMS:
        _VT_STREAMS[key] = torch.cuda.Stream(device=device)
    return _VT_STREAMS[key]


# ... 248 lines not shown
                raise ValueError("attend_rows: segments do not cover the rows")
            qkv = ops.gemm(xn, w, bias_n=bias, b_lo=wlo)
            ops.attention_fwd_qkv(qkv, list(segs), self.num_heads, scale, o, out_lo=o_lo)
            return o, o_lo
        one_launch = len(segs) == 2
        ldv_all = (max(n for _, n in segs) + 63) // 64 * 64
        stacked = one_launch or fold
        vt_all = torch.empty((sum(b for b, _ in segs), D, ldv_all), device=xn.device, dtype=xn.dtype) if stacked else None
        spare = xn.untyped_storage().nbytes() // xn.element_size() - (xn.storage_offset() + xn.shape[0] * D)
        side = None
        if one_launch and config.vt_stream and (fold or xn.is_cuda):
            main = torch.cuda.current_stream()
            side = _vt_side_stream(xn.device)
            side.wait_stream(main)
        else:
            qk = ops.gemm(xn, w[: 2 * D], **qk_kw)
        r0 = b0 = 0
        for B, N in segs:
            r1 = r0 + B * N
            ldvt = ldv_all if stacked else (N + 63) // 64 * 64
            vt = vt_all[b0:b0 + B] if stacked else torch.empty((B, D, ldvt), device=xn.device, dtype=xn.dtype)
            N4 = (N + granule - 1) // granule * granule
            if strict and spare < (N4 - N) * D:
                raise ValueError("attend_rows(ln=...): the hi plane needs 8 spare rows behind it")
            if not strict and spare < 4 * D:
                N4 = N
            with (torch.cuda.stream(side) if side is not None else contextlib.nullcontext()):
                ops.gemm(w[2 * D:], xn[r0:r1].as_strided((B, N4, D), (N * D, D, 1)),
                         out=vt.as_strided((B, D, N4), (D * ldvt, ldvt, 1)), **vt_kw(r0))
            if not one_launch:
                ops.attention_fwd(qk[r0:r1, :D], qk[r0:r1, D:], vt, B, self.num_heads, N, scale, out=o[r0:r1],
                                  out_lo=None if o_lo is None else o_lo[r0:r1])
            r0, b0 = r1, b0 + B
        if side is not None:
            qk = ops.gemm(xn, w[: 2 * D], **qk_kw)
            main.wait_stream(side)
            if fold:
                mr.record_stream(side)
        if one_launch:
            (B1, N1), (B2, N2) = segs
            ops.attention_fwd_seg(qk[:, :D], qk[:, D:], vt_all, B1, N1, B2, N2, self.num_heads, scale, out=o, out_lo=o_lo)
        if r0 != xn.shape[0]:
            raise ValueError("attend_rows: segments do not cover the rows")
        return o, o_lo

    def forward(self, x: torch.Tensor) -> torch.Tensor:
        raise RuntimeError("Attention is driven by Block.forward (LayerNorm / LayerScale / residual are fused around it)")


class MemEffAttention(Attention):
    """`attention.py:72-89`: same maths as ``Attention``; here both are the fused flash kernel."""


class Mlp(_Packed):

    def __init__(self, in_features, hidden_features=None, out_features=None, act_layer=nn.GELU, drop=0.0, bias=True):
        super().__init__()
        out_features = out_features or in_features
        hidden_features = hidden_features or in_features
        self.fc1 = nn.Linear(in_features, hidden_features, bias=bias)
        self.fc2 = nn.Linear(hidden_features, out_features, bias=bias)


class SwiGLUFFN(_Packed):

    def __init__(self, in_features, hidden_features=None, out_features=None, act_layer=None, drop=0.0, bias=True):
        super().__init__()
        out_features = out_features or in_features
        hidden_features = hidden_features or in_features
        self.w12 = nn.Linear(in_features, 2 * hidden_features, bias=bias)
        self.w3 = nn.Linear(hidden_features, out_features, bias=bias)

    def sg_rows(self) -> torch.Tensor:
        return _pack(self._cache, "w12.sgrows", self.w12.weight, lambda p: ops.swiglu_rows(p.shape[0] // 2, p.device))

    def sg_bias(self) -> Optional[torch.Tensor]:
        if self.w12.bias is None:
            return None
        rows = self.sg_rows()
        return _pack(self._cache, "w12_b.sg", self.w12.bias, lambda p: p.float()[rows].contiguous())


class SwiGLUFFNFused(SwiGLUFFN):

    def __init__(self, in_features, hidden_features=None, out_features=None, act_layer=None, drop=0.0, bias=True):
        out_features = out_features or in_features
        hidden_features = hidden_features or in_features
        hidden_features = (int(hidden_features * 2 / 3) + 7) // 8 * 8
        super().__init__(in_features, hidden_features, out_features, bias=bias)


class Block(_Packed):

    def __init__(self, dim, num_heads, mlp_ratio=4.0, qkv_bias=False, proj_bias=True, ffn_bias=True, drop=0.0,
                 attn_drop=0.0, init_values=None, drop_path=0.0, act_layer=nn.GELU, norm_layer=nn.LayerNorm,
                 attn_class=Attention, ffn_layer=Mlp):
        super().__init__()
        if drop:
            raise ValueError("dropout is 0 on the AdapterSIS path")
        if not 0.0 <= float(drop_path) < 1.0:
            raise ValueError(f"drop_path must be in [0, 1): got {drop_path}")
        self.norm1 = norm_layer(dim)
        self.attn = attn_class(dim, num_heads=num_heads, qkv_bias=qkv_bias, proj_bias=proj_bias)
        self.ls1 = LayerScale(dim, init_values=init_values) if init_values else nn.Identity()
        self.norm2 = norm_layer(dim)
        self.mlp = ffn_layer(in_features=dim, hidden_features=int(dim * mlp_ratio), act_layer=act_layer, bias=ffn_bias)
        self.ls2 = LayerScale(dim, init_values=init_values) if init_values else nn.Identity()
        self.sample_drop_ratio = drop_path

    def forward(self, x: torch.Tensor) -> torch.Tensor:
        B, N, D = x.shape
        x2 = x.reshape(B * N, D)
        if x2.dtype != torch.float32 or not x2.is_contiguous():
            x2 = x2.float().contiguous()
        return self.forward_rows(x2, [(B, N)]).view(B, N, D)

    def _gammas(self, raw: bool = False):
        g1 = self.ls1.gamma if isinstance(self.ls1, LayerScale) else None
        g2 = self.ls2.gamma if isinstance(self.ls2, LayerScale) else None
        return (g1, g2) if raw else (self._f32("g1", g1), self._f32("g2", g2))

    def _ffn(self):
        m = self.mlp
        return (m.fc1, "fc1", m.fc2, "fc2") if isinstance(m, Mlp) else (m.w12, "w12", m.w3, "w3")

    def _w16mx_any(self, owner, key: str, w: torch.Tensor, rows: Optional[torch.Tensor] = None):
        return _pack(owner._cache, key + (".sg" if rows is not None else "") + ".mx_any", w,
                     lambda p: ops.mx_from_pair(owner._w16(key, w, rows), owner._w16(key, w, rows, part=1), wside=True))

    def _mx_ok(self, owner, key: str, lin: nn.Linear, M: int) -> bool:
        N, K = lin.weight.shape
        return config.mx_dense_on() and K % 64 == 0 and N >= 256 and M >= 256 and N * K < (1 << 31)

    def _split_lin(self, owner, key: str, lin: nn.Linear, a_hi, a_lo, a_mx=None, rows=None, **kw):
        w = owner._w16(key, lin.weight, rows)
        if self._mx_ok(owner, key, lin, a_hi.shape[0]):
            a_pl, amax_a = a_mx if a_mx is not None else ops.mx_from_pair(a_hi, a_lo)
            w_mx, amax_w = self._w16mx_any(owner, key, lin.weight, rows)
            return ops.gemm(a_hi, w, a_lo=a_pl, b_lo=w_mx, mx=(amax_a, amax_w), **kw)
        return ops.gemm(a_hi, w, a_lo=a_lo, b_lo=owner._w16(key, lin.weight, rows, part=1), **kw)

    def _ln_split(self, key: str, norm: nn.LayerNorm, x2: torch.Tensor, mx: bool):
        dt = config.operand_dtype
        w, b = self._f32(key + "w", norm.weight), self._f32(key + "b", norm.bias)
        if mx:
            amax = derived(self._cache, key + ".amax", (norm.weight, norm.bias), lambda: (
                (x2.shape[1] - 1) ** 0.5 * norm.weight.detach().float().abs().max() + norm.bias.detach().float().abs().max()).reshape(1).contiguous())
            hi, pl = ops.layernorm_mx(x2, w, b, norm.eps, dt, amax)
            return hi, None, (pl, amax)
        xn32 = ops.layernorm(x2, w, b, norm.eps, torch.float32)
        D = x2.shape[1]
        return ops.cast_pad(xn32, D, dt), ops.cast_pad(xn32, D, dt, part=1), None

    def _forward_rows_precise(self, x2: torch.Tensor, segs) -> torch.Tensor:
        D = x2.shape[1]
        R = x2.shape[0]
        dt = config.operand_dtype
        a, m = self.attn, self.mlp
        g1, g2 = self._gammas()
        parts = config.precise_parts
        n1w, n1b = self._f32("n1w", self.norm1.weight), self._f32("n1b", self.norm1.bias)
        fold_q = config.fold_attn_scale and "qkv" not in parts and _PRECISE_FOLD_Q
        if "qkv" in parts:
            xn, xn_lo, xn_mx = self._ln_split("n1", self.norm1, x2, self._mx_ok(a, "qkv", a.qkv, R))
            qkv = self._split_lin(a, "qkv", a.qkv, xn, xn_lo, xn_mx, bias_n=a._f32("qkv_b", a.qkv.bias))
        elif fold_q:
            qw, qb, _ = a._qkv_folded()
            qkv = ops.gemm(ops.layernorm(x2, n1w, n1b, self.norm1.eps, dt), qw, bias_n=qb)
        else:
            qkv = ops.gemm(ops.layernorm(x2, n1w, n1b, self.norm1.eps, dt), a._w16("qkv", a.qkv.weight), bias_n=a._f32("qkv_b", a.qkv.bias))
        o = torch.empty((R, D), device=x2.device, dtype=dt)
        o_lo = torch.empty_like(o) if "proj" in parts else None
        if sum(B * N for B, N in segs) != R:
            raise ValueError("forward_rows: segments do not cover the rows")
        o_mx = None
        if fold_q and len(segs) <= 2:
            if o_lo is not None and _ATTN_MX_OUT and self._mx_ok(a, "proj", a.proj, R):
                o_mx = ops.absmax16(qkv[:, 2 * D:3 * D])
            ops.attention_fwd_qkv(qkv, list(segs), a.num_heads, None, o, out_lo=o_lo, mx_amax=o_mx)
        else:
            r0 = 0
            for B, N in segs:
                r1 = r0 + B * N
                vt = ops.transpose_tokens(qkv[r0:r1, 2 * D:], B, N)
                ops.attention_fwd(qkv[r0:r1, :D], qkv[r0:r1, D:2 * D], vt, B, a.num_heads, N, None if fold_q else a.scale,
                                  out=o[r0:r1], out_lo=None if o_lo is None else o_lo[r0:r1])
                r0 = r1
        pkw = dict(out_f32=True, bias_n=a._f32("proj_b", a.proj.bias), scale_n=g1, res=x2)
        if o_mx is not None:
            x1 = self._split_lin(a, "proj", a.proj, o, None, a_mx=(o_lo, o_mx), **pkw)
        else:
            x1 = self._split_lin(a, "proj", a.proj, o, o_lo, **pkw) if o_lo is not None else ops.gemm(o, a._w16("proj", a.proj.weight), **pkw)
        n2w, n2b = self._f32("n2w", self.norm2.weight), self._f32("n2b", self.norm2.bias)
        lin_in, k_in, lin_out, k_out = self._ffn()
        ikw = dict(out_f32=True, bias_n=m._f32(k_in + "_b", lin_in.bias))
        split_out = "fc2" in parts
        mx_in = "fc1" in parts and self._mx_ok(m, k_in, lin_in, R)
        sg = (not isinstance(m, Mlp)) and not split_out and \
            ops.swiglu_fused_ok(R, lin_in.out_features // 2, lin_in.in_features, "fc1" in parts, mx_in)
        ge = isinstance(m, Mlp) and not split_out
        if sg:
            rows = m.sg_rows()
            ikw = dict(bias_n=m.sg_bias(), act=ops.ACT_SILU_MUL, rows=rows)
        elif ge:
            ikw = dict(bias_n=m._f32(k_in + "_b", lin_in.bias), act=ops.ACT_GELU)
        if "fc1" in parts:
            xn2, xn2_lo, xn2_mx = self._ln_split("n2", self.norm2, x1, mx_in)
            hpre = self._split_lin(m, k_in, lin_in, xn2, xn2_lo, xn2_mx, **ikw)
        else:
            rows = ikw.pop("rows", None)
            hpre = ops.gemm(ops.layernorm(x1, n2w, n2b, self.norm2.eps, dt), m._w16(k_in, lin_in.weight, rows), **ikw)
        if sg or ge:
            h, h_lo = hpre, None
        elif isinstance(m, Mlp):
            h, h_lo = ops.gelu_split(hpre, dt, split=split_out)
        else:
            h, h_lo = ops.swiglu(hpre, dt, split=True) if split_out else (ops.swiglu(hpre, dt), None)
        okw = dict(out_f32=True, bias_n=m._f32(k_out + "_b", lin_out.bias), scale_n=g2, res=x1)
        if split_out:
            return self._split_lin(m, k_out, lin_out, h, h_lo, **okw)
        return ops.gemm(h, m._w16(k_out, lin_out.weight), **okw)

    def fold_ok(self, R: int, segs) -> bool:
        if not (config.ln_fold and config.operand_dtype == torch.float16 and config.precise_level < 2 and not config.precise_attention
                and not config.fused_qkv and isinstance(self.mlp, Mlp) and isinstance(self.ls1, LayerScale)
                and isinstance(self.ls2, LayerScale) and isinstance(self.norm1, nn.LayerNorm) and isinstance(self.norm2, nn.LayerNorm)):
            return False
        D, Hd = self.attn.qkv.weight.shape[1], self.mlp.fc1.weight.shape[0]
        if config.split_attn_out:
            return False
        ok = ops.ln_fold_supported(R, 2 * D, D) and ops.ln_fold_supported(R, D, D, producer=True)
        ok = ok and ops.ln_fold_supported(R, Hd, D) and ops.ln_fold_supported(R, D, Hd, producer=True)
        return ok and all(ops.ln_fold_supported(D, (N + 7) // 8 * 8, D, batch=B) for B, N in segs) and D % 64 == 0

    def forward_rows_fold(self, xin, segs, planes_out: bool):
        dt = config.operand_dtype
        a, m = self.attn, self.mlp
        g1, g2 = self._gammas()
        if isinstance(xin, tuple):
            hi, lo, mr = xin
            R, D = hi.shape
            o, o_lo = a.attend_rows(hi, segs, ln=(self.norm1, mr))
            res_kw = dict(res16=(hi, lo))
        else:
            R, D = xin.shape
            xn = torch.empty((R + 8, D), device=xin.device, dtype=dt)[:R]
            ops.layernorm(xin, self._f32("n1w", self.norm1.weight), self._f32("n1b", self.norm1.bias), self.norm1.eps, dt, out=xn)
            o, o_lo = a.attend_rows(xn, segs)
            res_kw = dict(res=xin)
        G = (D + 63) // 64
        x1h = torch.empty((R, D), device=o.device, dtype=dt)
        x1l = torch.empty((R, D), device=o.device, dtype=dt)
        st = torch.empty((R, G, 2), device=o.device, dtype=torch.float32)
        ops.gemm(o, a._w16("proj", a.proj.weight), out=x1h, out_lo=x1l, rowstats=st, bias_n=a._f32("proj_b", a.proj.bias), scale_n=g1,
                 a_lo=o_lo, **res_kw)
        mr1 = ops.ln_stats_finalize(st, D, self.norm2.eps)
        lin_in, k_in, lin_out, k_out = self._ffn()
        w1, b1, cs1 = self._lin_ln_folded(k_in + ".lnfold", lin_in, self.norm2)
        h = ops.gemm(x1h, w1, bias_n=b1, act=ops.ACT_GELU, ln=(mr1, cs1, False))
        w2, b2 = m._w16(k_out, lin_out.weight), m._f32(k_out + "_b", lin_out.bias)
        if not planes_out:
            return ops.gemm(h, w2, out_f32=True, bias_n=b2, scale_n=g2, res16=(x1h, x1l))
        x3h = torch.empty((R + 8, D), device=o.device, dtype=dt)[:R]
        x3l = torch.empty((R, D), device=o.device, dtype=dt)
        st3 = torch.empty((R, G, 2), device=o.device, dtype=torch.float32)
        ops.gemm(h, w2, out=x3h, out_lo=x3l, rowstats=st3, bias_n=b2, scale_n=g2, res16=(x1h, x1l))
        return x3h, x3l, ops.ln_stats_finalize(st3, D, self.norm1.eps)

    def forward_rows(self, x2: torch.Tensor, segs) -> torch.Tensor:
        if config.precise_level >= 2:
            return self._forward_rows_precise(x2, segs)
        D = x2.shape[1]
        dt = config.operand_dtype
        g1, g2 = self._gammas()
        xn = torch.empty((x2.shape[0] + 8, D), device=x2.device, dtype=dt)[: x2.shape[0]]
        ops.layernorm(x2, self._f32("n1w", self.norm1.weight), self._f32("n1b", self.norm1.bias), self.norm1.eps, dt, out=xn)
        o, o_lo = self.attn.attend_rows(xn, segs)
        x1 = ops.gemm(o, self.attn._w16("proj", self.attn.proj.weight), out_f32=True,
                      bias_n=self.attn._f32("proj_b", self.attn.proj.bias), scale_n=g1, res=x2, a_lo=o_lo,
                      b_lo=self.attn._w16lo("proj", self.attn.proj.weight))
        xn2 = ops.layernorm(x1, self._f32("n2w", self.norm2.weight), self._f32("n2b", self.norm2.bias),
                            self.norm2.eps, dt)
        m = self.mlp
        lin_in, k_in, lin_out, k_out = self._ffn()
        if isinstance(m, Mlp):
            h = ops.gemm(xn2, m._w16(k_in, lin_in.weight), bias_n=m._f32(k_in + "_b", lin_in.bias), act=ops.ACT_GELU)
        elif ops.swiglu_fused_ok(xn2.shape[0], lin_in.out_features // 2, lin_in.in_features, False, False):
            h = ops.gemm(xn2, m._w16(k_in, lin_in.weight, m.sg_rows()), bias_n=m.sg_bias(), act=ops.ACT_SILU_MUL)
        else:
            h12 = ops.gemm(xn2, m._w16(k_in, lin_in.weight), out_f32=True, bias_n=m._f32(k_in + "_b", lin_in.bias))
            h = ops.swiglu(h12, dt)
        return ops.gemm(h, m._w16(k_out, lin_out.weight), out_f32=True, bias_n=m._f32(k_out + "_b", lin_out.bias), scale_n=g2, res=x1)

    def forward_train(self, x: torch.Tensor, keep=None):
        B, N, D = x.shape
        x2 = x.reshape(B * N, D)
        if x2.dtype != torch.float32 or not x2.is_contiguous():
            x2 = x2.float().contiguous()
        out, saved = self.forward_train_rows(x2, [(B, N)]) if keep is None else self.forward_train_rows(x2, [(B, N)], keep=keep)
        return out.view(B, N, D), saved

    def _attn_train(self, xn: torch.Tensor, segs):
        dt = config.operand_dtype
        D = xn.shape[1]
        a = self.attn
        if a._lora is not None:
            P = ops.LORA_PAD
            if xn.stride(0) != D + P or xn.stride(1) != 1:
                raise ValueError("_attn_train with LoRA: xn must be the first D columns of a 16-bit [R, D + 64] buffer")
            abuf = xn.as_strided((xn.shape[0], D + P), (D + P, 1))
            wf, wf_lo, wd = a._lora_packs_fwd()
            ops.lora_down(abuf, [(0, D)], wd, out=abuf[:, D:])
            qkv = ops.gemm(abuf, wf, bias_n=a._f32("qkv_b", a.qkv.bias), b_lo=wf_lo)
        else:
            qkv = ops.gemm(xn, a._w16("qkv", a.qkv.weight), bias_n=a._f32("qkv_b", a.qkv.bias), b_lo=a._w16lo("qkv", a.qkv.weight))
        o = torch.empty((xn.shape[0], D), device=xn.device, dtype=dt)
        o_lo = torch.empty_like(o) if config.split_attn_out else None
        if sum(B * N for B, N in segs) != xn.shape[0]:
            raise ValueError("forward_train_rows: segments do not cover the rows")
        lse = torch.empty(xn.shape[0] * a.num_heads, device=xn.device, dtype=torch.float32)
        if len(segs) <= 2 and config.attn_rows:
            ops.attention_fwd_qkv(qkv, segs, a.num_heads, a.scale, o, out_lo=o_lo, lse=lse)
        else:
            r0 = l0 = 0
            for B, N in segs:
                r1, l1 = r0 + B * N, l0 + B * a.num_heads * N
                vt = ops.transpose_tokens(qkv[r0:r1, 2 * D:], B, N)
                ops.attention_fwd(qkv[r0:r1, :D], qkv[r0:r1, D:2 * D], vt, B, a.num_heads, N, a.scale, out=o[r0:r1],
                                  lse=lse[l0:l1].view(B, a.num_heads, N), out_lo=None if o_lo is None else o_lo[r0:r1])
                r0, l0 = r1, l1
        return qkv, o, o_lo, lse

    def forward_train_rows(self, x2: torch.Tensor, segs, keep=None):
        dt = config.operand_dtype
        D = x2.shape[1]
        m = self.mlp
        g1, g2 = self._gammas()
        a = self.attn
        segs = list(segs)
        if sum(B * N for B, N in segs) != x2.shape[0]:
            raise ValueError("forward_train_rows: segments do not cover the rows")
        ka, kf = droppath.as_branch_keeps(keep, segs, x2.device)
        n1w, n1b = self._f32("n1w", self.norm1.weight), self._f32("n1b", self.norm1.bias)
        lora_on = a._lora is not None
        if lora_on and keep is not None:
            raise ValueError("forward_train_rows: LoRA and stochastic depth exclude each other (the gathered LayerNorm has no strided output)")
        if ka is None:
            if lora_on:
                xn = torch.empty((x2.shape[0], D + ops.LORA_PAD), device=x2.device, dtype=dt)[:, :D]
                ops.layernorm(x2, n1w, n1b, self.norm1.eps, dt, out=xn)
            else:
                xn = ops.layernorm(x2, n1w, n1b, self.norm1.eps, dt)
            qkv, o, o_lo, lse = self._attn_train(xn, segs)
            x1 = ops.gemm(o, a._w16("proj", a.proj.weight), out_f32=True, bias_n=a._f32("proj_b", a.proj.bias), scale_n=g1,
                          res=x2, a_lo=o_lo, b_lo=a._w16lo("proj", a.proj.weight))
        elif ka.empty:
            xn = qkv = o = lse = None
            x1 = x2
        else:
            xn = ops.layernorm_gather(x2, n1w, n1b, self.norm1.eps, dt, ka)
            qkv, o, o_lo, lse = self._attn_train(xn, ka.segs)
            y = ops.gemm(o, a._w16("proj", a.proj.weight), out_f32=True, bias_n=a._f32("proj_b", a.proj.bias), scale_n=g1,
                         a_lo=o_lo, b_lo=a._w16lo("proj", a.proj.weight))
            x1 = ops.scaled_index_add(x2, y, ka)
        n2w, n2b = self._f32("n2w", self.norm2.weight), self._f32("n2b", self.norm2.bias)
        if kf is not None and kf.empty:
            saved = (x2, xn, qkv, o, lse, x1, None, None, None, segs, (ka, kf))
            return x1, saved
        xn2 = ops.layernorm(x1, n2w, n2b, self.norm2.eps, dt) if kf is None else ops.layernorm_gather(x1, n2w, n2b, self.norm2.eps, dt, kf)
        okw = dict(out_f32=True, scale_n=g2)
        if kf is None:
            okw["res"] = x1
        lin_in, k_in, lin_out, k_out = self._ffn()
        if isinstance(m, Mlp):
            hpre = ops.gemm(xn2, m._w16(k_in, lin_in.weight), bias_n=m._f32(k_in + "_b", lin_in.bias))
            hpost = ops.gelu16(hpre)
        else:
            hpre = ops.gemm(xn2, m._w16(k_in, lin_in.weight), out_f32=True, bias_n=m._f32(k_in + "_b", lin_in.bias))
            hpost = ops.swiglu(hpre, dt)
        x3 = ops.gemm(hpost, m._w16(k_out, lin_out.weight), bias_n=m._f32(k_out + "_b", lin_out.bias), **okw)
        if kf is not None:
            x3 = ops.scaled_index_add(x1, x3, kf)
        saved = (x2, xn, qkv, o, lse, x1, xn2, hpre, hpost, segs)
        if lora_on:
            return x3, saved + ((None, None), "lora")
        return x3, (saved if keep is None else saved + ((ka, kf),))

    def backward(self, saved, dres: torch.Tensor, inv_scale: float, grads: Optional[dict] = None, prefix: str = "") -> torch.Tensor:
        x2, xn, qkv, o, lse, x1, xn2, hpre, hpost, segs = saved[:10]
        ka, kf = saved[10] if len(saved) > 10 else (None, None)
        lora_on = len(saved) > 11 and saved[11] == "lora"
        dt = config.operand_dtype
        D = x2.shape[1]
        a, m = self.attn, self.mlp
        ls1, ls2 = self._gammas(raw=True)
        pre = prefix + "." if prefix else ""
        lgrads = None
        if lora_on and grads is not None and pre + "attn.qkv.lora_A" in grads:
            lgrads, grads = grads, None
        elif lora_on and grads is not None:
            raise ValueError("Block.backward: behind a LoRA forward ``grads`` holds the block's LoRA names (or is None)")
        k1, k2 = self._ls_pow2("ls1.k", ls1), self._ls_pow2("ls2.k", ls2)
        inv1, inv2 = inv_scale * 2.0 ** -k1, inv_scale * 2.0 ** -k2
        lin_in, k_in, lin_out, k_out = self._ffn()
        n_in, n_out = "mlp." + k_in, "mlp." + k_out
        act_bwd = ops.gelu16 if isinstance(m, Mlp) else ops.swiglu_bwd
        if kf is not None and kf.empty:
            dx1 = dres
            self._zero_grads(grads, [pre + n_out, pre + n_in, pre + "norm2"], pre + "ls2.gamma")
        else:
            if kf is not None:
                d16, cs = ops.gather_cast_colsum(dres, dt, kf, colsum=grads is not None)
            else:
                d16, cs = ops.cast_colsum(dres, dt) if grads is not None else (ops.cast_pad(dres, D, dt), None)
            self._linear_bwd(pre + n_out, lin_out, ls2, pre + "ls2.gamma", d16, cs, hpost, inv_scale, grads)
            R = d16.shape[0]
            if isinstance(m, Mlp) and R >= 256 and lin_out.in_features >= 128 and lin_out.in_features % 4 == 0 and D % 32 == 0:
                dh = ops.gemm(d16, self._wT16("fc2T", lin_out.weight, ls2, k2), act=ops.ACT_GELU_GRAD, aux=hpre)
            else:
                dh = ops.gemm(d16, self._wT16("fc2T", lin_out.weight, ls2, k2))
                dh = act_bwd(hpre, dh)
            self._linear_bwd(pre + n_in, lin_in, None, None, dh, ops.colsum(dh) if grads is not None else None, xn2,
                             inv2, grads)
            dln = ops.gemm(dh, self._wT16("fc1T", lin_in.weight), out_f32=True)
            if kf is not None:
                dx1, part = ops.layernorm_bwd_scatter(dln, x1, self._nw_pow2("n2w", self.norm2.weight, -k2), self.norm2.eps, dres, kf)
            else:
                dx1, part = ops.layernorm_bwd(dln, x1, self._nw_pow2("n2w", self.norm2.weight, -k2), self.norm2.eps, res=dres)
            if grads is not None:
                red = ops.reduce_rows(part.view(part.shape[0], 2 * D), inv2)
                grads[pre + "norm2.weight"].copy_(red[:D]); grads[pre + "norm2.bias"].copy_(red[D:])
        if ka is not None and ka.empty:
            self._zero_grads(grads, [pre + "attn.proj", pre + "attn.qkv", pre + "norm1"], pre + "ls1.gamma")
            return dx1
        if ka is not None:
            d16, cs = ops.gather_cast_colsum(dx1, dt, ka, colsum=grads is not None)
            segs = ka.segs
        else:
            d16, cs = ops.cast_colsum(dx1, dt) if grads is not None else (ops.cast_pad(dx1, D, dt), None)
        self._linear_bwd(pre + "attn.proj", a.proj, ls1, pre + "ls1.gamma", d16, cs, o, inv_scale, grads)
        dO = ops.gemm(d16, self._wT16("projT", a.proj.weight, ls1, k1))
        if lora_on:
            dbuf = torch.empty((d16.shape[0], 3 * D + ops.LORA_PAD), device=x2.device, dtype=dt)
            dqkv = dbuf[:, :3 * D]
        else:
# ... 65 lines not shown
```

adaptersis_amd/ops.py:

```python
from __future__ import annotations

import ctypes as C
import functools
import os
from typing import Optional

import torch

from . import _lib, config
from ._lib import ACT_GELU, ACT_GELU_GRAD, ACT_NONE, ACT_RELU, ACT_SILU_MUL, GemmDesc, check, lib

T16_DEFAULT = torch.float16

PROFILE = None


def _launch_timed(kind: str, flops: float, fn, nbytes: float = 0.0):
    if PROFILE is None:
        return fn()
    s, e = torch.cuda.Event(enable_timing=True), torch.cuda.Event(enable_timing=True)
    s.record()
    rc = fn()
    e.record()
    PROFILE.append((kind, flops, s, e, nbytes))
# ... 174 lines not shown


def _conv_desc(x_nhwc: torch.Tensor, w_packed: torch.Tensor, KH: int, KW: int, stride: int, pad: int, *,
               out: Optional[torch.Tensor] = None, out_f32: bool = True, bias_n: Optional[torch.Tensor] = None,
               act: int = ACT_NONE, stats: Optional[torch.Tensor] = None, accumulate: bool = False,
               x_lo: Optional[torch.Tensor] = None, w_lo: Optional[torch.Tensor] = None, ksplit: int = 1, mx=None):
    _dev(x_nhwc, w_packed, out, bias_n, stats)
    if not x_nhwc.is_contiguous():
        raise ValueError("conv_gemm: x must be contiguous NHWC")
    Bn, H, W, Cin = x_nhwc.shape
    Cout, K = w_packed.shape
    OH = (H + 2 * pad - KH) // stride + 1
    OW = (W + 2 * pad - KW) // stride + 1
    if ksplit > 1:
        if out is not None or accumulate or not out_f32 or act != ACT_NONE or stats is not None:
            raise ValueError("conv_gemm: ksplit needs a fresh fp32 output without activation; take the BatchNorm "
                             "statistics from the sum with colstats()")
        out = torch.empty((ksplit, Bn, OH, OW, Cout), device=x_nhwc.device, dtype=torch.float32)
    if out is None:
        out = torch.empty((Bn, OH, OW, Cout), device=x_nhwc.device, dtype=torch.float32 if out_f32 else x_nhwc.dtype)
    d = GemmDesc()
    d.A, d.B, d.C = x_nhwc.data_ptr(), w_packed.data_ptr(), out.data_ptr()
    if ksplit > 1:
        d.ksplit, d.strideC = ksplit, Bn * OH * OW * Cout
    d.lda, d.ldb, d.ldc = K, w_packed.stride(0), Cout
    d.batch, d.M, d.N, d.K = 1, Bn * OH * OW, Cout, K
    d.bias_n = _p(_f32c(bias_n))
    if accumulate:
        if out.dtype != torch.float32:
            raise ValueError("conv_gemm: accumulate needs an fp32 output")
        d.res, d.ldr = out.data_ptr(), Cout
    d.act, d.out_f32, d.dtype = act, int(out.dtype == torch.float32), _dt(x_nhwc.dtype)
    d.conv, d.B_, d.H, d.W, d.Cin, d.OH, d.OW = 1, Bn, H, W, Cin, OH, OW
    d.KH, d.KW, d.stride, d.pad = KH, KW, stride, pad
    d.stats = _p(stats)
    flops = 2.0 * d.M * Cout * K
    if x_lo is not None:
        d.A_lo, d.B_lo = x_lo.data_ptr(), w_lo.data_ptr()
    if mx is not None:
        d.mx_amax_a, d.mx_amax_b = _f32c(mx[0]).data_ptr(), _f32c(mx[1]).data_ptr()
    return d, out, flops


def conv_gemm(x_nhwc: torch.Tensor, w_packed: torch.Tensor, KH: int, KW: int, stride: int, pad: int, **kw) -> torch.Tensor:
    d, out, flops = _conv_desc(x_nhwc, w_packed, KH, KW, stride, pad, **kw)
    check(_launch_timed("conv", flops, lambda: lib().asis_gemm(_stream(), C.byref(d))), "asis_gemm(conv)")
    if d.ksplit > 1:
        parts, out = out, torch.empty(out.shape[1:], device=out.device, dtype=torch.float32)
        reduce_rows(parts.view(d.ksplit, -1), 1.0, out.view(-1))
    return out


_SPLIT_FUSED = os.environ.get("ASIS_SPLIT_FUSED", "1") != "0"


def _fused_split(M: int, N: int, K: int) -> bool:
    return _SPLIT_FUSED and _split_shape_ok(M, N, K) and _shape_plan(256, 32, 64, out_f32=True, split=True) is not None


CONV_HALO = os.environ.get("ASIS_CONV_HALO", "1") not in ("0", "")


def conv_gemm_split(x_hi, x_lo, w_hi, w_lo, KH: int, KW: int, stride: int, pad: int, *, bias_n=None, stats=None,
                    ksplit: int = 1, mx=None):
    if mx is None:
        _not_mx("conv_gemm_split", x_lo, w_lo)
    Bn, H, W, Cin = x_hi.shape
    OH, OW = (H + 2 * pad - KH) // stride + 1, (W + 2 * pad - KW) // stride + 1
    Cout = w_hi.shape[0]
    if _fused_split(Bn * OH * OW, Cout, Cin):
        return conv_gemm(x_hi, w_hi, KH, KW, stride, pad, bias_n=bias_n, stats=stats, x_lo=x_lo, w_lo=w_lo, ksplit=ksplit, mx=mx)
    if mx is not None:
        raise ValueError("conv_gemm_split: MX operands need the fused large-tile path (mx_conv_ok)")
    out = conv_gemm(x_hi, w_hi, KH, KW, stride, pad, bias_n=bias_n)
    conv_gemm(x_lo, w_hi, KH, KW, stride, pad, out=out, accumulate=True)
    conv_gemm(x_hi, w_lo, KH, KW, stride, pad, out=out, accumulate=True, stats=stats)
    return out


def conv_halo_ok(x_hi: torch.Tensor, Cout: int, stride: int, pad: int, force: bool = False) -> bool:
    return ((CONV_HALO or force) and x_hi.dtype == torch.float16 and stride == 1 and pad == 1 and x_hi.shape[3] % 64 == 0 and Cout in (64, 128)
            and x_hi.is_contiguous())


def conv3x3_halo_mx(x_hi, x_mx, w_hi, w_mx, mx, *, bias_n=None, want_stats: bool = False):
    _dev(x_hi, x_mx, w_hi, w_mx, bias_n, mx[0], mx[1])
    Bn, H, W, Cin = x_hi.shape
    Cout = w_hi.shape[0]
    if not (x_hi.is_contiguous() and x_mx.is_contiguous() and w_hi.is_contiguous() and w_mx.is_contiguous() and w_hi.shape[1] == 9 * Cin):
        raise ValueError("conv3x3_halo_mx: contiguous NHWC planes and [Cout, 9 Cin] packed weights expected")
    out = torch.empty((Bn, H, W, Cout), device=x_hi.device, dtype=torch.float32)
    stats = None
    if want_stats:
        stats = torch.empty((lib().asis_conv3x3_halo_mx_tiles(Bn, H, W), 2, Cout), device=x_hi.device, dtype=torch.float32)
    check(lib().asis_conv3x3_halo_mx(_stream(), _dt(x_hi.dtype), x_hi.data_ptr(), x_mx.data_ptr(), w_hi.data_ptr(), w_mx.data_ptr(),
                                     _p(_f32c(bias_n)), mx[0].data_ptr(), mx[1].data_ptr(), out.data_ptr(), _p(stats), Bn, H, W, Cin, Cout),
          "asis_conv3x3_halo_mx")
    return (out, stats) if want_stats else out


def gemm_split(a_hi, a_lo, b_hi, b_lo, *, out: torch.Tensor, bias_n=None):
    M, K, N = a_hi.shape[-2], a_hi.shape[-1], b_hi.shape[-2]
    if _fused_split(M, N, K):
        return gemm(a_hi, b_hi, out=out, bias_n=bias_n, a_lo=a_lo, b_lo=b_lo)
    gemm(a_hi, b_hi, out=out, bias_n=bias_n)
    gemm(a_lo, b_hi, out=out, res=out)
    gemm(a_hi, b_lo, out=out, res=out)
    return out


def ln_fold_supported(M: int, N: int, K: int, batch: int = 1, producer: bool = False) -> bool:
    return _shape_plan(M, N, K, batch=1 if producer else batch, ln=not producer, producer=producer) is not None


def ln_stats_finalize(rowstats: torch.Tensor, D: int, eps: float = 1e-6) -> torch.Tensor:
    _dev(rowstats)
    rows, groups = rowstats.shape[0], rowstats.shape[1]
    mr = torch.empty((rows + 8, 2), device=rowstats.device, dtype=torch.float32)[:rows]
    check(lib().asis_ln_stats_finalize(_stream(), _f32c(rowstats).data_ptr(), rows, groups, D, float(eps), mr.data_ptr()),
          "asis_ln_stats_finalize")
    return mr


def split_stats(x: torch.Tensor, dtype: torch.dtype, eps: float = 1e-6):
    _dev(x)
    if x.dtype != torch.float32 or x.dim() != 2 or x.stride(1) != 1:
        raise ValueError("split_stats: x must be float32 [rows, D] contiguous in D")
    rows, D = x.shape
    hi = torch.empty((rows + 8, D), device=x.device, dtype=dtype)[:rows]
    lo = torch.empty((rows, D), device=x.device, dtype=dtype)
    mr = torch.empty((rows + 8, 2), device=x.device, dtype=torch.float32)[:rows]
    check(lib().asis_split_stats(_stream(), _dt(dtype), x.data_ptr(), x.stride(0), hi.data_ptr(), lo.data_ptr(), D, mr.data_ptr(),
                                 rows, D, float(eps)), "asis_split_stats")
    return hi, lo, mr


def layernorm(x: torch.Tensor, w: torch.Tensor, b: torch.Tensor, eps: float = 1e-6,
              out_dtype: torch.dtype = T16_DEFAULT, out: Optional[torch.Tensor] = None) -> torch.Tensor:
    _dev(x, w, b, out)
    if x.dtype != torch.float32 or x.stride(-1) != 1:
        raise ValueError("layernorm: x must be float32 with a contiguous last dim")
    D = x.shape[-1]
    x2 = x.reshape(-1, D)
    if out is None:
        out = torch.empty(x.shape, device=x.device, dtype=out_dtype)
    o2 = out.view(-1, D)
    f32 = out.dtype == torch.float32
    check(lib().asis_layernorm(_stream(), _dt(out.dtype) if not f32 else 0, x2.data_ptr(), x2.stride(0),
                               _f32c(w).data_ptr(), _f32c(b).data_ptr(), float(eps), o2.data_ptr(), o2.stride(0),
                               int(f32), x2.shape[0], D), "asis_layernorm")
    return out


def layernorm_mx(x: torch.Tensor, w: torch.Tensor, b: torch.Tensor, eps: float, out_dtype: torch.dtype, amax: torch.Tensor):
    _dev(x, w, b, amax)
    if x.dtype != torch.float32 or x.dim() != 2 or x.stride(1) != 1:
        raise ValueError("layernorm_mx: x must be float32 [rows, D] with contiguous columns")
    R, D = x.shape
    hi = torch.empty((R, D), device=x.device, dtype=out_dtype)
    mx = torch.empty_like(hi)
    check(lib().asis_layernorm_mx(_stream(), _dt(out_dtype), x.data_ptr(), x.stride(0), _f32c(w).data_ptr(), _f32c(b).data_ptr(), float(eps),
                                  hi.data_ptr(), mx.data_ptr(), D, amax.data_ptr(), R, D), "asis_layernorm_mx")
    return hi, mx


def _check_out_lo(out: torch.Tensor, out_lo: Optional[torch.Tensor]) -> None:
    if out_lo is not None and (out_lo.shape != out.shape or out_lo.stride() != out.stride() or out_lo.dtype != out.dtype):
        raise ValueError("attention_fwd: out_lo must share the shape, layout and dtype of out")


def _attention_launch(q, k, vt, out, out_lo, B1, N1, B2, N2, H, scale, lse):
    if scale is None:
        check(lib().asis_attention_fwd_prescaled(_stream(), _dt(q.dtype), q.data_ptr(), k.data_ptr(), q.stride(0), vt.data_ptr(),
                                                 vt.stride(1), out.data_ptr(), _p(out_lo), out.stride(0), B1, N1, B2, N2, H,
                                                 _p(lse)), "asis_attention_fwd_prescaled")
    else:
        check(lib().asis_attention_fwd_split(_stream(), _dt(q.dtype), q.data_ptr(), k.data_ptr(), q.stride(0), vt.data_ptr(),
                                             vt.stride(1), out.data_ptr(), _p(out_lo), out.stride(0), B1, N1, B2, N2, H,
                                             float(scale), _p(lse)), "asis_attention_fwd")


def attention_fwd_qkv(qkv: torch.Tensor, segs, H: int, scale: Optional[float], out: torch.Tensor,
                      out_lo: Optional[torch.Tensor] = None, lse: Optional[torch.Tensor] = None,
                      mx_amax: Optional[torch.Tensor] = None) -> torch.Tensor:
    _dev(qkv, out, out_lo, lse, mx_amax)
    D = H * 64
    if qkv.dim() != 2 or qkv.shape[1] < 3 * D or qkv.stride(1) != 1 or len(segs) not in (1, 2):
        raise ValueError("attention_fwd_qkv: qkv must be [rows, >= 3*H*64] with contiguous rows, one or two segments")
    (B1, N1), (B2, N2) = (segs[0], segs[1]) if len(segs) == 2 else (segs[0], (0, 0))
    if qkv.shape[0] != B1 * N1 + B2 * N2:
        raise ValueError("attention_fwd_qkv: segments do not cover the rows")
    _check_out_lo(out, out_lo)
    es = qkv.element_size()
    if mx_amax is not None:
        if out_lo is None:
            raise ValueError("attention_fwd_qkv: mx_amax needs the second output plane")
        check(lib().asis_attention_fwd_qkv_mx(_stream(), _dt(qkv.dtype), qkv.data_ptr(), qkv.data_ptr() + D * es,
                                              qkv.data_ptr() + 2 * D * es, qkv.stride(0), out.data_ptr(), out_lo.data_ptr(), out.stride(0),
                                              B1, N1, B2, N2, H, 0.0 if scale is None else float(scale), int(scale is None), _p(lse),
                                              mx_amax.data_ptr()), "asis_attention_fwd_qkv_mx")
        return out
    check(lib().asis_attention_fwd_qkv(_stream(), _dt(qkv.dtype), qkv.data_ptr(), qkv.data_ptr() + D * es,
                                       qkv.data_ptr() + 2 * D * es, qkv.stride(0), out.data_ptr(), _p(out_lo), out.stride(0),
                                       B1, N1, B2, N2, H, 0.0 if scale is None else float(scale), int(scale is None), _p(lse)),
          "asis_attention_fwd_qkv")
    return out


def attention_fwd(q: torch.Tensor, k: torch.Tensor, vt: torch.Tensor, B: int, H: int, N: int, scale: Optional[float],
                  out: Optional[torch.Tensor] = None, lse: Optional[torch.Tensor] = None,
                  out_lo: Optional[torch.Tensor] = None) -> torch.Tensor:
    _dev(q, k, vt, out, lse, out_lo)
    if q.stride(0) != k.stride(0) or q.stride(1) != 1 or k.stride(1) != 1:
        raise ValueError("attention_fwd: q and k must share a row stride and be contiguous in the last dim")
    if out is None:
        out = torch.empty((B * N, H * 64), device=q.device, dtype=q.dtype)
    if lse is not None and (lse.dtype != torch.float32 or lse.numel() != B * H * N or not lse.is_contiguous()):
        raise ValueError("attention_fwd: lse must be contiguous float32 [B,H,N]")
    _check_out_lo(out, out_lo)
    _attention_launch(q, k, vt, out, out_lo, B, N, 0, 0, H, scale, lse)
    return out


def attention_fwd_seg(q: torch.Tensor, k: torch.Tensor, vt: torch.Tensor, B1: int, N1: int, B2: int, N2: int, H: int,
                      scale: Optional[float], out: torch.Tensor, out_lo: Optional[torch.Tensor] = None) -> torch.Tensor:
    _dev(q, k, vt, out, out_lo)
    _check_out_lo(out, out_lo)
    if q.stride(0) != k.stride(0) or q.stride(1) != 1 or k.stride(1) != 1 or q.shape[0] != B1 * N1 + B2 * N2:
        raise ValueError("attention_fwd_seg: q and k must be row views over both batches with one row stride")
    _attention_launch(q, k, vt, out, out_lo, B1, N1, B2, N2, H, scale, None)
    return out


def token_ld(N: int) -> int:
    return (N + 63) // 64 * 64


def transpose_tokens(src: torch.Tensor, B: int, N: int, out: Optional[torch.Tensor] = None) -> torch.Tensor:
    _dev(src, out)
    Cc = src.shape[1]
    if src.stride(1) != 1 or src.shape[0] != B * N:
        raise ValueError("transpose_tokens: expected a [B*N, C] row view")
    ldt = token_ld(N)
    if out is None:
        out = torch.empty((B, Cc, ldt), device=src.device, dtype=src.dtype)
    check(lib().asis_transpose_tokens(_stream(), _dt(src.dtype), src.data_ptr(), src.stride(0), out.data_ptr(), ldt, B, N,
                                      Cc), "asis_transpose_tokens")
    return out


def attention_bwd_rows(q, k, v, o, dO, lse, segs, H: int, scale: float, dqkv: Optional[torch.Tensor] = None) -> torch.Tensor:
    _dev(q, k, v, o, dO, lse, dqkv)
    Wd = H * 64
    if len(segs) not in (1, 2):
        raise ValueError("attention_bwd_rows: one or two stacked token batches")
    (B1, N1), (B2, N2) = segs[0], (segs[1] if len(segs) == 2 else (0, 0))
    R = B1 * N1 + B2 * N2
    if not (q.stride(0) == k.stride(0) == v.stride(0)) or q.stride(1) != 1 or q.shape[0] != R:
        raise ValueError("attention_bwd_rows: q, k, v must be [R, H*64] views sharing a row stride")
    if lse.dtype != torch.float32 or not lse.is_contiguous() or lse.numel() != R * H:
        raise ValueError("attention_bwd_rows: lse must be one contiguous float32 buffer of R * H values")
    if dqkv is None:
        dqkv = torch.empty((R, 3 * Wd), device=q.device, dtype=q.dtype)
    D = torch.empty(R * H, device=q.device, dtype=torch.float32)
    es = dqkv.element_size()
    check(lib().asis_attention_bwd_rows(_stream(), _dt(q.dtype), q.data_ptr(), k.data_ptr(), v.data_ptr(), q.stride(0),
                                        o.data_ptr(), o.stride(0), dO.data_ptr(), dO.stride(0), lse.data_ptr(), D.data_ptr(),
                                        dqkv.data_ptr(), dqkv.data_ptr() + Wd * es, dqkv.data_ptr() + 2 * Wd * es,
                                        dqkv.stride(0), B1, N1, B2, N2, H, float(scale)), "asis_attention_bwd_rows")
    return dqkv


def layernorm_bwd(dy: torch.Tensor, x: torch.Tensor, w: torch.Tensor, eps: float = 1e-6,
                  res: Optional[torch.Tensor] = None, out: Optional[torch.Tensor] = None):
    _dev(dy, x, w, res, out)
    R, D = x.shape
    for t in (dy, x, res, out):
        if t is not None and (t.dtype != torch.float32 or t.stride(-1) != 1 or t.shape != x.shape):
            raise ValueError("layernorm_bwd: float32 [R, D] row views of one shape expected")
    if out is None:
        out = torch.empty((R, D), device=x.device, dtype=torch.float32)
    nblk = lib().asis_rowblock_nblk(R)
    partial = torch.empty((nblk, 2, D), device=x.device, dtype=torch.float32)
    check(lib().asis_layernorm_bwd(_stream(), dy.data_ptr(), dy.stride(0), x.data_ptr(), x.stride(0), _f32c(w).data_ptr(),
                                   float(eps), _p(res), res.stride(0) if res is not None else 0, out.data_ptr(),
                                   out.stride(0), partial.data_ptr(), R, D), "asis_layernorm_bwd")
    return out, partial


def gelu16(pre: torch.Tensor, dpost: Optional[torch.Tensor] = None) -> torch.Tensor:
    _dev(pre, dpost)
    if not pre.is_contiguous() or (dpost is not None and (not dpost.is_contiguous() or dpost.shape != pre.shape)):
        raise ValueError("gelu16: contiguous operands of one shape expected")
    out = torch.empty_like(pre)
    check(lib().asis_gelu16(_stream(), _dt(pre.dtype), pre.data_ptr(), _p(dpost), out.data_ptr(), pre.numel()), "asis_gelu16")
    return out


def gelu_split(x: torch.Tensor, dtype: torch.dtype, split: bool = True):
    _dev(x)
    if x.dtype != torch.float32 or not x.is_contiguous():
        raise ValueError("gelu_split: contiguous float32 expected")
    hi = torch.empty(x.shape, device=x.device, dtype=dtype)
    lo = torch.empty_like(hi) if split else None
    check(lib().asis_gelu_split(_stream(), _dt(dtype), x.data_ptr(), hi.data_ptr(), _p(lo), x.numel()), "asis_gelu_split")
    return hi, lo
# ... 1701 lines not shown
```

include/asis_hip.h:

```cpp
#ifndef ASIS_HIP_H
#define ASIS_HIP_H

#include <stdint.h>

#ifdef __cplusplus
extern "C" {
#endif

#define ASIS_OK 0
#define ASIS_EINVAL (-1)
#define ASIS_ELAUNCH (-2)

#define ASIS_F16 0
#define ASIS_BF16 1
#define ASIS_F32 2

#define ASIS_ACT_NONE 0
#define ASIS_ACT_GELU 1
#define ASIS_ACT_RELU 2
#define ASIS_ACT_SILU_MUL 3
#define ASIS_ACT_GELU_GRAD 4

const char* asis_last_error(void);
int asis_version(void);
int asis_device_count(void);

typedef struct asis_gemm_desc {
  const void* A;
  const void* B;
  void* C;
  int64_t lda, ldb, ldc;
  int64_t strideA, strideB, strideC;
  int32_t batch;
  int32_t M, N, K;
  const float* bias_n;
  const float* bias_m;
  const float* scale_n;
  const float* res;
  int64_t ldr, strideR;
  int32_t act;
  int32_t out_f32;
  int32_t dtype;
  int32_t conv;
  int32_t B_, H, W, Cin, OH, OW, KH, KW, stride, pad;
  float* stats;
  const void* A_lo;
  const void* B_lo;
  const void* aux;
  int64_t ld_aux;
  int32_t ksplit;
  const float* mx_amax_a;
  const float* mx_amax_b;
  void* C_lo;
  float* rowstats;
  const void* res16;
  const void* res16_lo;
  int64_t ldr16;
  const float* ln_mr;
  const float* ln_cs;
  int32_t ln_cols;
} asis_gemm_desc;
int asis_ln_stats_finalize(void* stream, const float* rowstats, int64_t rows, int groups, int D, float eps, float* mr);
int asis_split_stats(void* stream, int dtype, const float* x, int64_t ldx, void* hi, void* lo, int64_t ld16, float* mr,
                     int64_t rows, int D, float eps);
int asis_gemm(void* stream, const asis_gemm_desc* d);
int asis_gemm_tiles_m(int M);
int asis_absmax_f32(void* stream, const float* x, int64_t rows, int cols, int64_t ld, float* amax, int reset);
int asis_bn_relu_absmax(void* stream, const float* x, const float* scale, const float* shift, int64_t P, int C, int relu, float* amax);
int asis_conv3x3_halo_mx_tiles(int B, int H, int W);
int asis_conv3x3_halo_mx(void* stream, int dtype, const void* x_hi, const void* x_mx, const void* w_hi, const void* w_mx, const float* bias,
                         const float* amax_a, const float* amax_b, float* out, float* stats, int B, int H, int W, int Cin, int Cout);
int asis_absmax_16(void* stream, int dtype, const void* x, int64_t rows, int cols, int64_t ld, float* amax);
int asis_mx_from_pair(void* stream, int dtype, const void* hi, const void* lo, int64_t ld_in, void* out_mx, int64_t ld_out, int64_t rows,
                      int cols, const float* amax, int wside);
int asis_gemm_set_option(const char* name, int value);
int asis_gemm_plan(const asis_gemm_desc* d, int* form, int* grid_x, int* grid_y, int* block);
const char* asis_gemm_form_name(int form);

int asis_layernorm(void* stream, int dtype, const float* x, int64_t ldx, const float* w, const float* b, float eps,
                   void* y, int64_t ldy, int out_f32, int64_t rows, int D);
int asis_layernorm_mx(void* stream, int dtype, const float* x, int64_t ldx, const float* w, const float* b, float eps, void* y,
                      void* y_mx, int64_t ldy, const float* amax, int64_t rows, int D);

int asis_attention_fwd(void* stream, int dtype, const void* q, const void* k, int64_t ldqk, const void* vt,
                       int64_t ldvt, void* o, int64_t ldo, int B, int H, int N, float scale);
int asis_attention_fwd_seg(void* stream, int dtype, const void* q, const void* k, int64_t ldqk, const void* vt, int64_t ldvt,
                           void* o, int64_t ldo, int B1, int N1, int B2, int N2, int H, float scale, float* lse2);
int asis_attention_fwd_split(void* stream, int dtype, const void* q, const void* k, int64_t ldqk, const void* vt, int64_t ldvt,
                             void* o, void* o_lo, int64_t ldo, int B1, int N1, int B2, int N2, int H, float scale, float* lse2);
int asis_attention_fwd_prescaled(void* stream, int dtype, const void* q, const void* k, int64_t ldqk, const void* vt, int64_t ldvt,
                                 void* o, void* o_lo, int64_t ldo, int B1, int N1, int B2, int N2, int H, float* lse2);
int asis_attention_fwd_qkv(void* stream, int dtype, const void* q, const void* k, const void* v, int64_t ld, void* o, void* o_lo,
                           int64_t ldo, int B1, int N1, int B2, int N2, int H, float scale, int prescaled, float* lse2);
int asis_attention_fwd_qkv_mx(void* stream, int dtype, const void* q, const void* k, const void* v, int64_t ld, void* o, void* o_mx,
                              int64_t ldo, int B1, int N1, int B2, int N2, int H, float scale, int prescaled, float* lse2,
                              const float* amax);
int asis_attention_fwd_lse(void* stream, int dtype, const void* q, const void* k, int64_t ldqk, const void* vt,
                           int64_t ldvt, void* o, int64_t ldo, int B, int H, int N, float scale, float* lse2);
int asis_transpose_tokens(void* stream, int dtype, const void* src, int64_t ld, void* dst, int64_t ldt, int B, int N,
                          int C);
int asis_attention_bwd_rows(void* stream, int dtype, const void* q, const void* k, const void* v, int64_t ld, const void* o,
                            int64_t ldo, const void* dO, int64_t lddo, const float* lse2, float* D, void* dq, void* dk,
                            void* dv, int64_t lddq, int B1, int N1, int B2, int N2, int H, float scale);

int asis_im2col_patch(void* stream, int dtype, const float* img, int B, int Himg, int Wimg, int P, void* out,
                      int64_t ldk);
int asis_im2col_patch_split(void* stream, int dtype, const float* img, int B, int Himg, int Wimg, int P, void* out,
                            void* out_lo, int64_t ldk);

int asis_cast_pad(void* stream, int dtype, const float* src, int64_t ld_src, void* dst, int64_t ld_dst, int64_t rows,
                  int cols, float scale, int part);

int asis_add_cls_pos(void* stream, const float* x, const float* cls, const float* pos, float* out, int B, int N,
                     int D);

int asis_rowblock_nblk(int64_t rows);
int asis_layernorm_bwd(void* stream, const float* dy, int64_t lddy, const float* x, int64_t ldx, const float* w, float eps,
                       const float* res, int64_t ldr, float* dx, int64_t lddx, float* partial, int64_t rows, int D);
int asis_gelu16(void* stream, int dtype, const void* pre, const void* dpost, void* out, int64_t n);
int asis_gelu_split(void* stream, int dtype, const float* x, void* hi, void* lo, int64_t n);
int asis_swiglu_bwd(void* stream, int dtype, const float* x12, const void* dh, void* dx12, int64_t R, int Hd);
int asis_colsum(void* stream, int dtype, const void* x, int64_t ld, float* partial, int64_t rows, int C);
int asis_cast_colsum(void* stream, int dtype, const float* x, int64_t ldx, void* out, int64_t ldo, float scale,
                     float* partial, int64_t rows, int D);
int asis_ls_linear_finish(void* stream, const float* G, const float* W, const float* bias, const float* gamma,
                          const float* cs, float grad_scale, float* dW, float* db, float* dgamma, int N, int K);

int asis_layernorm_gather(void* stream, int dtype, const float* x, int64_t ldx, const float* w, const float* b, float eps, void* y,
                          int64_t ldy, const int32_t* tab, int K, int S, int64_t rows_c, int D);
int asis_scaled_index_add(void* stream, const float* x, int64_t ldx, const float* res, int64_t ldres, float* out, int64_t ldo,
                          const int32_t* tab, int K, int S, int64_t rows, int D);
int asis_gather_cast_colsum(void* stream, int dtype, const float* x, int64_t ldx, void* out, int64_t ldo, float* partial,
                            const int32_t* tab, int K, int S, int64_t rows_c, int D);
int asis_layernorm_bwd_scatter(void* stream, const float* dy, int64_t lddy, const float* x, int64_t ldx, const float* w, float eps,
                               const float* res, int64_t ldr, float* dx, int64_t lddx, float* partial, const int32_t* tab, int K, int S,
                               int64_t rows, int64_t rows_c, int D);

int asis_msda_fwd(void* stream, int dtype, const void* value, const float* offaw, int64_t ld_offaw, const float* ref,
                  const int32_t* shapes, const int32_t* starts, void* out, int B, int Lq, int Lin, int M, int L, int P,
                  int Dh);
int asis_msda_fwd_split(void* stream, int dtype, const void* value, const float* offaw, int64_t ld_offaw, const float* ref,
                        const int32_t* shapes, const int32_t* starts, void* out, void* out_lo, int B, int Lq, int Lin, int M,
                        int L, int P, int Dh);

int asis_dwconv_gelu(void* stream, int dtype, const float* x, const float* w9, const float* bias,
                     const int32_t* shapes, const int32_t* starts, int L, void* out, int B, int Ntok, int C);

int asis_msda_bwd(void* stream, int dtype, const void* value, const float* offaw, int64_t ld_offaw, const float* ref,
                  const int32_t* shapes, const int32_t* starts, const float* dout, float* dvalue, float* doffaw, int B,
                  int Lq, int Lin, int M, int L, int P, int Dh);
int asis_msda_vgrad_cap(int Lq, int L, int P);
int asis_msda_value_grad(void* stream, int dtype, const float* offaw, int64_t ld_offaw, const float* ref, const int32_t* shapes,
                         const int32_t* starts, const void* dout16, const float* amax, int32_t* cnt, int32_t* offs, void* rec,
                         float* dvalue, int B, int Lq, int Lin, int M, int L, int P, int Dh);
int asis_msda_sampling_matrix(void* stream, int dtype, const float* offaw, int64_t ld_offaw, const float* ref,
                              const int32_t* shapes, const int32_t* starts, void* ST, int64_t ldt, int B, int Lq, int Lin,
                              int M, int L, int P);
int asis_dwconv_bwd_nblk(int64_t rows);
int asis_dwconv_gelu_bwd(void* stream, int dtype, const float* x, const float* w9, const float* bias, const int32_t* shapes,
                         const int32_t* starts, int L, const float* dy, float* g, float* partial, void* dx, int B, int Ntok,
                         int C);

int asis_conv3x3_c3(void* stream, const float* img, const float* w, float* out, int B, int H, int W, int Cout,
                    int stride, int pad);
int asis_conv3x3_smallcout_fwd(void* stream, int dtype, const void* x_hi, const void* x_lo, const float* w,
                               const float* bias, float* out, int B, int H, int W, int Cin, int Cout);
int asis_conv3x3_smallcout_dgrad(void* stream, int dtype, const void* dy_hi, const void* dy_lo, int CoP, const float* w,
                                 float* dx, int B, int H, int W, int Cin, int Cout);

int asis_conv3x3_smallcout_fwd_up(void* stream, int dtype, const float* raw, const float* scale, const float* shift, const float* w,
                                  const float* bias, float* out, int B, int H, int W, int Cin, int Cout);
int asis_conv3x3_smallcout_wgrad_up(void* stream, int dtype, const void* dy, int CoP, const float* raw, const float* scale,
                                    const float* shift, float* slabs, int nblk, int B, int H, int W, int Cin, int Cout);

int asis_cls_lowres_nblk(int B, int H, int W);
int asis_cls_lowres_fwd(void* stream, const float* raw, const float* scale, const float* shift, const float* w, const float* bias,
                        float* z, float* out, int B, int H, int W, int Cin, int Cout);
int asis_cls_lowres_bwd(void* stream, int dtype, const void* d16, const void* d_lo, int CoP, const float* raw, const float* scale,
                        const float* shift, const float* mean, const float* invstd, const float* w, float* g, float* partial,
                        float* slabs, int nblk, int B, int H, int W, int Cin, int Cout);

int asis_dgrad_lowres_nblk(int B, int H, int W);
int asis_dgrad_lowres_cap(int cap);
int asis_dgrad_lowres_pack(void* stream, int dtype, const float* w, void* w_hi, void* w_lo, int Co, int Ck);
int asis_dgrad_lowres(void* stream, int dtype, const void* d16, const void* d_lo, const void* w_hi, const void* w_lo, const float* raw,
                      const float* scale, const float* shift, const float* mean, const float* invstd, float* g, float* partial,
                      int nblk, int B, int H, int W, int Co, int Ck);

int asis_conv3x3_smallcout_wgrad(void* stream, int dtype, const void* dy, int CoP, const void* x, float* slabs, int nblk,
                                 int B, int H, int W, int Cin, int Cout);
int asis_colstats_nparts(int64_t R);
int asis_colstats(void* stream, const float* x, int64_t R, int C, float* partial);
int asis_reduce_partials(void* stream, const float* partial, int nparts, int C, double* sums);
int asis_bn_finalize(void* stream, const double* sums, double count, int C, const float* gamma, const float* beta,
                     float eps, float momentum, float* running_mean, float* running_var, int64_t* num_batches_tracked,
                     float* scale, float* shift, float* mean_out, float* invstd_out);
int asis_bn_eval_affine(void* stream, const float* gamma, const float* beta, const float* running_mean,
                        const float* running_var, float eps, int C, float* scale, float* shift);
int asis_bn_act(void* stream, int dtype, const float* x, const float* scale, const float* shift, int relu, void* out,
                void* out_lo, int64_t R, int C);
int asis_bn_act_mx(void* stream, int dtype, const float* x, const float* scale, const float* shift, int relu, void* out, void* out_mx,
                   const float* amax, int64_t R, int C);
int asis_bn_relu_maxpool(void* stream, int dtype, const float* x, const float* scale, const float* shift, void* out,
                         void* out_lo, int B, int H, int W, int C);
int asis_bn_relu_upsample(void* stream, int dtype, const float* x, const float* scale, const float* shift, void* out,
                          void* out_lo, int B, int H, int W, int C, int factor);
int asis_bn_relu_upsample_mx(void* stream, int dtype, const float* x, const float* scale, const float* shift, void* out,
                             void* out_mx, const float* amax, int B, int H, int W, int C, int factor);
int asis_pack_conv_weight(void* stream, int dtype, const float* w, void* out, int Cout, int Cin, int KH, int KW,
                          int mode, int64_t ldo, int part);
int asis_pack_conv_weight_mx(void* stream, int dtype, const float* w, void* out_mx, int Cout, int Cin, int KH, int KW,
                             int mode, int64_t ldo, const float* amax);
int asis_pack_conv_weight_pair(void* stream, int dtype, const float* w, void* out_hi, void* out_lo, int Cout, int Cin, int KH,
                               int KW, int mode, int64_t ldo, const float* amax);
int asis_decoder_input(void* stream, int dtype, const float* xs, int64_t xs_bstride, const float* c4,
                       int64_t c4_bstride, const float* vit, int64_t vit_bstride, void* out, void* out_lo, int B, int h,
                       int w, int h4, int w4, int D);
int asis_decoder_input_mx(void* stream, int dtype, const float* xs, int64_t xs_bstride, const float* c4, int64_t c4_bstride,
                          const float* vit, int64_t vit_bstride, void* out, void* out_mx, const float* amax, int B, int h,
                          int w, int h4, int w4, int D);
int asis_swiglu(void* stream, int dtype, const float* x12, void* out, int64_t R, int Hd);
int asis_swiglu_split(void* stream, int dtype, const float* x12, void* out, void* out_lo, int64_t R, int Hd);
int asis_copy_channels(void* stream, const void* src, int64_t src_ld_bytes, void* dst, int64_t dst_ld_bytes, int64_t rows,
                       int64_t row_bytes);
int asis_add_f32(void* stream, const float* a, const float* b, float* out, int64_t n, int batch, int64_t stride_a,
                 int64_t stride_b, int64_t stride_out);

int asis_maxpool2_fwd(void* stream, int dtype, const void* x, const void* x_lo, void* out, void* out_lo, uint8_t* idx,
                      int B, int H, int W, int C);
int asis_maxpool2_bwd(void* stream, const float* dy, const uint8_t* idx, float* dx, int B, int H, int W, int C);
int asis_cls_l2norm(void* stream, const float* x, float* chat, float* inv_c, int B, int N, int C, int D);
int asis_cls_l2norm_bwd(void* stream, const float* dchat, const float* chat, const float* inv_c, float* dx, int B, int N, int C,
                        int D);
int asis_mask_logits_fwd(void* stream, const float* P, const float* chat, const float* gamma, const float* beta, float eps,
                         float* logits, float* cosm, float* inv_p, int B, int N, int C, int D);
// ... 168 lines not shown
```

Measured before the change: 224.8 img/s.

## Fuse paired adapter layernorms and final-norm with residual add

Adds a layernorm_pair kernel that normalizes the shared CNN feature tensor once and writes both the CAViT feat_norm and CACNN query_norm outputs, avoiding a second read and reduction. Adds a layernorm_add kernel that applies the ViT final norm and adds it to the adapter output in one pass, skipping the separate normalized-feature materialization unless it is needed. Also adds an optional no-concat path for the dual-stream trunk that writes block outputs directly into a preallocated buffer; it is off by default. These changes cut memory traffic and kernel launches on the adapter stages, at the cost of more code paths and possible small numeric differences.

```diff
diff --git a/adaptersis_amd/_lib.py b/adaptersis_amd/_lib.py
--- a/adaptersis_amd/_lib.py
+++ b/adaptersis_amd/_lib.py
@@ -89,6 +89,9 @@
     "asis_split_stats": [_vp, _i, _vp, _i64, _vp, _vp, _i64, _vp, _i64, _i, _f],
     "asis_gemm_set_option": [C.c_char_p, _i],
     "asis_layernorm": [_vp, _i, _vp, _i64, _vp, _vp, _f, _vp, _i64, _i, _i64, _i],
+    "asis_layernorm_pair_ok": [_i64, _i],
+    "asis_layernorm_pair": [_vp, _i, _vp, _i64, _vp, _vp, _vp, _vp, _f, _vp, _vp, _i64, _i64, _i],
+    "asis_layernorm_add": [_vp, _vp, _i64, _i, _vp, _vp, _f, _vp, _i64, _vp, _i64, _vp, _i64, _i, _i, _i],
     "asis_layernorm_mx": [_vp, _i, _vp, _i64, _vp, _vp, _f, _vp, _vp, _i64, _vp, _i64, _i],
     "asis_attention_fwd_seg": [_vp, _i, _vp, _vp, _i64, _vp, _i64, _vp, _i64, _i, _i, _i, _i, _i, _f, _vp],
     "asis_attention_fwd_split": [_vp, _i, _vp, _vp, _i64, _vp, _i64, _vp, _vp, _i64, _i, _i, _i, _i, _i, _f, _vp],
diff --git a/adaptersis_amd/backbones/adapter_blocks.py b/adaptersis_amd/backbones/adapter_blocks.py
--- a/adaptersis_amd/backbones/adapter_blocks.py
+++ b/adaptersis_amd/backbones/adapter_blocks.py
@@ -131,9 +131,12 @@
 
 class _AdapterBase(_Packed):
     def _ln16(self, name, x2d):
+        w, b, eps = self._ln_affine(name)
+        return ops.layernorm(x2d, w, b, eps, config.operand_dtype)
+
+    def _ln_affine(self, name):
         ln = getattr(self, name)
-        return ops.layernorm(x2d, self._f32(name + "_w", ln.weight), self._f32(name + "_b", ln.bias), ln.eps,
-                             config.operand_dtype)
+        return self._f32(name + "_w", ln.weight), self._f32(name + "_b", ln.bias), ln.eps
 
     def _ln_bwd(self, name, dy, x2d, inv_scale, grads, prefix, res=None):
         ln = getattr(self, name)
@@ -186,8 +189,8 @@
         return out.view(B, Lq, D)
 
 
-    def forward16_train(self, c2, x2, g, B, Lq, Lin, grids):
-        qn, fn = self._ln16("query_norm", c2), self._ln16("feat_norm", x2)
+    def forward16_train(self, c2, x2, g, B, Lq, Lin, grids, qn=None):
+        qn, fn = self._ln16("query_norm", c2) if qn is None else qn, self._ln16("feat_norm", x2)
         out1, s_attn = self.attn.forward16_train(qn, fn, g["ref2"], g["shapes2"], g["starts2"], B, Lq, Lin, res=c2)
         s_ffn = None
         out = out1
@@ -228,8 +231,8 @@
                                   starts_i32, B, Lq, Lin, res=q2, scale_n=self._f32("gamma", self.gamma))
         return out.view(B, Lq, D)
 
-    def forward16_train(self, x2, c2, g, B, Lq, Lin):
-        qn, fn = self._ln16("query_norm", x2), self._ln16("feat_norm", c2)
+    def forward16_train(self, x2, c2, g, B, Lq, Lin, fn=None):
+        qn, fn = self._ln16("query_norm", x2), self._ln16("feat_norm", c2) if fn is None else fn
         out, s_attn = self.attn.forward16_train(qn, fn, g["ref1"], g["shapes1"], g["starts1"], B, Lq, Lin, res=x2,
                                                 scale_n=self._f32("gamma", self.gamma))
         return out, (x2, c2, s_attn)
@@ -242,3 +245,11 @@
         dx = self._ln_bwd("query_norm", dq, x2, inv_scale, grads, pre, res=dout)
         dc = self._ln_bwd("feat_norm", dfeat, c2, inv_scale, grads, pre)
         return dx, dc
+
+
+def ln16_pair(cv: CAViT, cn: CACNN, c2d):
+    w1, b1, e1 = cv._ln_affine("feat_norm")
+    w2, b2, e2 = cn._ln_affine("query_norm")
+    if not config.ln_pair or e1 != e2:
+        return None, None
+    return ops.layernorm_pair(c2d, w1, b1, w2, b2, e1, config.operand_dtype)
diff --git a/adaptersis_amd/backbones/engines.py b/adaptersis_amd/backbones/engines.py
--- a/adaptersis_amd/backbones/engines.py
+++ b/adaptersis_amd/backbones/engines.py
@@ -14,7 +14,7 @@
 from ..droppath import DropPathSampler
 from ..optim import SGD, AdamW, FlatBucket
 from ..parallel import StageReducer, world_size
-from .adapter_blocks import CACNN, CAViT, deform_inputs
+from .adapter_blocks import CACNN, CAViT, deform_inputs, ln16_pair
 
 
 class pre_vit(_Packed):
@@ -242,35 +242,47 @@
             for a, b in zip(cuts[:-1], cuts[1:]):
                 parts.append((slice(r0 + a * N, r0 + b * N), [(b - a, N)]))
             r0 += B * N
+        ycat = torch.empty_like(xcat) if config.trunk_nocat and len(blocks) else None
         xs = []
         for st, (sl, _) in zip(self._dual_streams, parts):
             st.wait_stream(main)
             xcat.record_stream(st)
+            if ycat is not None:
+                ycat.record_stream(st)
             xs.append(xcat[sl])
         nblk = len(blocks)
         for bi, blk in enumerate(blocks):
-            for i, (st, (_, sg)) in enumerate(zip(self._dual_streams, parts)):
+            for i, (st, (sl, sg)) in enumerate(zip(self._dual_streams, parts)):
                 with torch.cuda.stream(st):
                     R_i = xs[i][0].shape[0] if isinstance(xs[i], tuple) else xs[i].shape[0]
+                    out = ycat[sl] if ycat is not None and bi + 1 == nblk else None
                     if blk.fold_ok(R_i, sg):
-                        xs[i] = blk.forward_rows_fold(xs[i], sg, planes_out=bi + 1 < nblk and blocks[bi + 1].fold_ok(R_i, sg))
+                        xs[i] = blk.forward_rows_fold(xs[i], sg, planes_out=bi + 1 < nblk and blocks[bi + 1].fold_ok(R_i, sg), out=out)
                     else:
-                        xs[i] = blk.forward_rows(xs[i], sg)
+                        xs[i] = blk.forward_rows(xs[i], sg, out=out)
         for st, x in zip(self._dual_streams, xs):
             main.wait_stream(st)
-            x.record_stream(main)
-        return torch.cat(xs, 0)
-
-    def _cavit(self, x2, c2, g, B, Lq, Lin):
+            if ycat is None:
+                x.record_stream(main)
+        return ycat if ycat is not None else torch.cat(xs, 0)
+
+    def _cavit(self, x2, c2, g, B, Lq, Lin, fn=None):
         cv = self.cross_vit
-        return cv.attn.forward16(cv._ln16("query_norm", x2), cv._ln16("feat_norm", c2), g["ref1"], g["shapes1"],
-                                 g["starts1"], B, Lq, Lin, res=x2, scale_n=cv._f32("gamma", cv.gamma))
-
-    def _cacnn(self, c2, x2, g, B, Lq, Lin, grids):
+        return cv.attn.forward16(cv._ln16("query_norm", x2), cv._ln16("feat_norm", c2) if fn is None else fn, g["ref1"],
+                                 g["shapes1"], g["starts1"], B, Lq, Lin, res=x2, scale_n=cv._f32("gamma", cv.gamma))
+
+    def _cacnn(self, c2, x2, g, B, Lq, Lin, grids, qn=None):
         cn = self.cross_cnn
-        out = cn.attn.forward16(cn._ln16("query_norm", c2), cn._ln16("feat_norm", x2), g["ref2"], g["shapes2"],
-                                g["starts2"], B, Lq, Lin, res=c2)
+        out = cn.attn.forward16(cn._ln16("query_norm", c2) if qn is None else qn, cn._ln16("feat_norm", x2), g["ref2"],
+                                g["shapes2"], g["starts2"], B, Lq, Lin, res=c2)
         return cn.ffn.forward16(cn._ln16("ffn_norm", out), out, B, Lq, grids) if cn.with_cffn else out
+
+    def _stage_out(self, x2, xa, out, keep_norm: bool):
+        m = self.model
+        nrm = torch.empty_like(xa) if keep_norm else None
+        ops.layernorm_add(x2, xa, m.norm.weight.detach().float(), m.norm.bias.detach().float(), m.norm.eps, skip=1, out=out,
+                          norm_out=nrm)
+        return out, (nrm[:, 1:] if keep_norm else None)
 
     @torch.no_grad()
     def features(self, inp: torch.Tensor, taps: Optional[dict] = None, adapter_saves: Optional[list] = None):
@@ -306,16 +318,19 @@
         ops.add_cls_pos(tokens, m.cls_token.detach().reshape(-1).float().contiguous(),
                         pos.detach().reshape(-1, D).float().contiguous(), out=xcat[:Ra].view(B, N + 1, D))
         feats = []
+        fuse_add = config.norm_add
         trunk = list(m.blocks[: nb - (nl - 1)])
         if config.dual_stream and inp.is_cuda and getattr(self, "_dual_warm", False) and nb - nl == len(trunk) - 1:
             xcat = self._trunk_dual(xcat, Ra, trunk, segs)
-            feats.append(m._final_norm(xcat[:Ra].view(B, N + 1, D))[:, 1:])
+            if not fuse_add:
+                feats.append(m._final_norm(xcat[:Ra].view(B, N + 1, D))[:, 1:])
             trunk = []
         self._dual_warm = True
         if trunk:
             assert nb - nl == len(trunk) - 1
             xcat = run_blocks(trunk, xcat, segs)
-            feats.append(m._final_norm(xcat[:Ra].view(B, N + 1, D))[:, 1:])
+            if not fuse_add:
+                feats.append(m._final_norm(xcat[:Ra].view(B, N + 1, D))[:, 1:])
         if enc_done is not None:
             torch.cuda.current_stream().wait_event(enc_done)
         if taps is not None:
@@ -332,19 +347,26 @@
                     xcat = torch.cat([xa_s, xb_s.reshape(Rb, D)], 0)
                 else:
                     xcat = run_blocks([blk], xcat, segs)
-                feats.append(m._final_norm(xcat[:Ra].view(B, N + 1, D))[:, 1:])
+                if not fuse_add:
+                    feats.append(m._final_norm(xcat[:Ra].view(B, N + 1, D))[:, 1:])
             dead = s == nl - 1 and taps is None and config.elide_dead_cacnn
+            fn, qn = (None, None) if dead else ln16_pair(self.cross_vit, self.cross_cnn, c2d)
             if train:
-                x2, s_cv = self.cross_vit.forward16_train(xcat[Ra:].clone(), c2d, g, B, N, Lc)
+                x2, s_cv = self.cross_vit.forward16_train(xcat[Ra:].clone(), c2d, g, B, N, Lc, fn=fn)
                 s_cn = None
                 if not dead:
-                    c2d, s_cn = self.cross_cnn.forward16_train(c2d, x2, g, B, Lc, N, shapes)
+                    c2d, s_cn = self.cross_cnn.forward16_train(c2d, x2, g, B, Lc, N, shapes, qn=qn)
                 adapter_saves.append((bsaved, s_cv, s_cn))
             else:
-                x2 = self._cavit(xcat[Ra:], c2d, g, B, N, Lc)
+                x2 = self._cavit(xcat[Ra:], c2d, g, B, N, Lc, fn=fn)
                 if not dead:
-                    c2d = self._cacnn(c2d, x2, g, B, Lc, N, shapes)
-            x = ops.add_f32(x2.view(B, N, D), feats[s], out=xcat[Ra:].view(B, N, D))
+                    c2d = self._cacnn(c2d, x2, g, B, Lc, N, shapes, qn=qn)
+            if fuse_add:
+                x, f = self._stage_out(x2.view(B, N, D), xcat[:Ra].view(B, N + 1, D), xcat[Ra:].view(B, N, D),
+                                       keep_norm=taps is not None or (s == nl - 1 and not self.stream_only))
+                feats.append(f)
+            else:
+                x = ops.add_f32(x2.view(B, N, D), feats[s], out=xcat[Ra:].view(B, N, D))
         if taps is not None:
             taps.update(feats=feats)
         if self.stream_only:
@@ -396,11 +418,12 @@
         xcat = torch.cat([xa.view(Ra, D), tokens.reshape(B * N, D)], 0)
         xcat = run_blocks(list(m.blocks[: nb - 3]), xcat, segs)
         c2d = c.view(B * Lc, D)
+        fn, qn = ln16_pair(self.cross_vit, self.cross_cnn, c2d)
         if train:
-            x2, s_cv = self.cross_vit.forward16_train(xcat[Ra:].clone(), c2d, g, B, N, Lc)
+            x2, s_cv = self.cross_vit.forward16_train(xcat[Ra:].clone(), c2d, g, B, N, Lc, fn=fn)
             adapter_saves.append((None, s_cv, None))
         else:
-            x2 = self._cavit(xcat[Ra:], c2d, g, B, N, Lc)
+            x2 = self._cavit(xcat[Ra:], c2d, g, B, N, Lc, fn=fn)
         outs = [x2]
         for j, bi in enumerate((nb - 3, nb - 2, nb - 2)):
             bsaved = None
@@ -420,12 +443,14 @@
             else:
                 x2 = m.blocks[bi](x2.view(B, N, D)).view(B * N, D)
             if train:
-                c2d, s_cn = self.cross_cnn.forward16_train(c2d, x2.contiguous(), g, B, Lc, N, shapes)
-                x2, s_cv = self.cross_vit.forward16_train(x2.clone(), c2d, g, B, N, Lc)
+                c2d, s_cn = self.cross_cnn.forward16_train(c2d, x2.contiguous(), g, B, Lc, N, shapes, qn=qn)
+                fn, qn = ln16_pair(self.cross_vit, self.cross_cnn, c2d) if j < 2 else (None, None)
+                x2, s_cv = self.cross_vit.forward16_train(x2.clone(), c2d, g, B, N, Lc, fn=fn)
                 adapter_saves.append((bsaved, s_cv, s_cn))
             else:
-                c2d = self._cacnn(c2d, x2, g, B, Lc, N, shapes)
-                x2 = self._cavit(x2, c2d, g, B, N, Lc)
+                c2d = self._cacnn(c2d, x2, g, B, Lc, N, shapes, qn=qn)
+                fn, qn = ln16_pair(self.cross_vit, self.cross_cnn, c2d) if j < 2 else (None, None)
+                x2 = self._cavit(x2, c2d, g, B, N, Lc, fn=fn)
             outs.append(x2)
         xa = m.blocks[nb - 1](xcat[:Ra].view(B, N + 1, D))
         vit_last = m._final_norm(xa)[:, 1:]
diff --git a/adaptersis_amd/config.py b/adaptersis_amd/config.py
--- a/adaptersis_amd/config.py
+++ b/adaptersis_amd/config.py
@@ -55,6 +55,10 @@
 elide_c1 = os.environ.get("ASIS_ELIDE_C1", "1") not in ("0", "")
 share_patch_embed = os.environ.get("ASIS_SHARE_PATCH_EMBED", "1") not in ("0", "")
 
+ln_pair = os.environ.get("ASIS_LN_PAIR", "1") not in ("0", "")
+norm_add = os.environ.get("ASIS_NORM_ADD", "1") not in ("0", "")
+trunk_nocat = os.environ.get("ASIS_TRUNK_NOCAT", "0") not in ("0", "")
+
 ln_fold = os.environ.get("ASIS_LN_FOLD", "1") not in ("0", "")
 
 _mx = os.environ.get("ASIS_MX_CONV", "1")
diff --git a/adaptersis_amd/csrc/core.hip b/adaptersis_amd/csrc/core.hip
--- a/adaptersis_amd/csrc/core.hip
+++ b/adaptersis_amd/csrc/core.hip
@@ -12,7 +12,7 @@
 }
 
 extern "C" const char* asis_last_error(void) { return g_err; }
-extern "C" int asis_version(void) { return 100; }
+extern "C" int asis_version(void) { return 101; }
 
 extern "C" int asis_device_count(void) {
   int n = 0;
diff --git a/adaptersis_amd/csrc/norm.hip b/adaptersis_amd/csrc/norm.hip
--- a/adaptersis_amd/csrc/norm.hip
+++ b/adaptersis_amd/csrc/norm.hip
@@ -84,6 +84,89 @@
   }
 }
 
+template <typename T, int NCH, int RPW>
+__global__ __launch_bounds__(256) void layernorm_pair_kernel(const float* __restrict__ x, int64_t ldx,
+                                                             const float* __restrict__ w, const float* __restrict__ b,
+                                                             const float* __restrict__ w2, const float* __restrict__ b2,
+                                                             float eps, T* __restrict__ y, T* __restrict__ y2, int64_t ldy,
+                                                             int64_t rows) {
+  constexpr int NOUT = 2;
+  constexpr int D = 256 * NCH;
+  const int lane = threadIdx.x & 63;
+  const int64_t row0 = ((int64_t)blockIdx.x * 4 + (threadIdx.x >> 6)) * RPW;
+  if (row0 >= rows) return;
+  float4 v[RPW][NCH];
+#pragma unroll
+  for (int r = 0; r < RPW; ++r) {
+    const int64_t row = row0 + r < rows ? row0 + r : rows - 1;
+    const float4* xr = reinterpret_cast<const float4*>(x + row * ldx);
+#pragma unroll
+    for (int i = 0; i < NCH; ++i) v[r][i] = xr[lane + 64 * i];
+  }
+  float4 ww[NOUT][NCH], bb[NOUT][NCH];
+#pragma unroll
+  for (int k = 0; k < NOUT; ++k)
+#pragma unroll
+    for (int i = 0; i < NCH; ++i) {
+      ww[k][i] = reinterpret_cast<const float4*>(k ? w2 : w)[lane + 64 * i];
+      bb[k][i] = reinterpret_cast<const float4*>(k ? b2 : b)[lane + 64 * i];
+    }
+  float mean[RPW], rstd[RPW];
+#pragma unroll
+  for (int r = 0; r < RPW; ++r) {
+    float s = 0.f;
+#pragma unroll
+    for (int i = 0; i < NCH; ++i) s += (v[r][i].x + v[r][i].y) + (v[r][i].z + v[r][i].w);
+    mean[r] = s;
+  }
+#pragma unroll
+  for (int r = 0; r < RPW; ++r) mean[r] = wave_sum(mean[r]) / (float)D;
+#pragma unroll
+  for (int r = 0; r < RPW; ++r) {
+    float q = 0.f;
+#pragma unroll
+    for (int i = 0; i < NCH; ++i) {
+      const float a0 = v[r][i].x - mean[r], a1 = v[r][i].y - mean[r], a2 = v[r][i].z - mean[r],
+                  a3 = v[r][i].w - mean[r];
+      q += (a0 * a0 + a1 * a1) + (a2 * a2 + a3 * a3);
+    }
+    rstd[r] = q;
+  }
+#pragma unroll
+  for (int r = 0; r < RPW; ++r) rstd[r] = 1.0f / sqrtf(wave_sum(rstd[r]) / (float)D + eps);
+#pragma unroll
+  for (int r = 0; r < RPW; ++r) {
+    const int64_t row = row0 + r;
+    if (row >= rows) break;
+#pragma unroll
+    for (int k = 0; k < NOUT; ++k)
+#pragma unroll
+      for (int i = 0; i < NCH; ++i) {
+        const int c = lane + 64 * i;
+        const float o0 = (v[r][i].x - mean[r]) * rstd[r] * ww[k][i].x + bb[k][i].x;
+        const float o1 = (v[r][i].y - mean[r]) * rstd[r] * ww[k][i].y + bb[k][i].y;
+        const float o2 = (v[r][i].z - mean[r]) * rstd[r] * ww[k][i].z + bb[k][i].z;
+        const float o3 = (v[r][i].w - mean[r]) * rstd[r] * ww[k][i].w + bb[k][i].w;
+        uint2 p;
+        p.x = pack2<T>(o0, o1);
+        p.y = pack2<T>(o2, o3);
+        reinterpret_cast<uint2*>((k ? y2 : y) + row * ldy)[c] = p;
+      }
+  }
+}
+
+__global__ __launch_bounds__(256) void layernorm_add_kernel(const float* __restrict__ x, int64_t sx, const float* __restrict__ w,
+                                                            const float* __restrict__ b, float eps, const float* __restrict__ a,
+                                                            int64_t sa, float* __restrict__ out, int64_t so,
+                                                            float* __restrict__ norm, int64_t sn, int batch, int n, int D) {
+  const int lane = threadIdx.x & 63;
+  const int64_t row = (int64_t)blockIdx.x * 4 + (threadIdx.x >> 6);
+  if (row >= (int64_t)batch * n) return;
+  const int64_t bi = row / n, r = row - bi * n;
+  ln_row<f16, true, true>(x + bi * sx + r * D, w, b, eps, norm ? norm + bi * sn + r * D : nullptr, D, lane, a + bi * sa + r * D,
+                          out + bi * so + r * D);
+}
+
 __global__ __launch_bounds__(256) void add_cls_pos_kernel(const float4* __restrict__ x, const float4* __restrict__ cls,
                                                           const float4* __restrict__ pos, float4* __restrict__ out,
                                                           int B, int N, int D4) {
@@ -260,6 +343,15 @@
   return ASIS_OK;
 }
 
+static int ln_fast_rows() {
+  static const int v = [] {
+    const char* e = getenv("ASIS_LN_FAST");
+    return e ? atoi(e) : 2;
+  }();
+  return v;
+}
+static bool ln_fixed_shape(int64_t rows, int D) { return ln_fast_rows() && (D == 768 || D == 1024 || D == 1536) && rows >= 4096; }
+
 extern "C" int asis_layernorm(void* stream, int dtype, const float* x, int64_t ldx, const float* w, const float* b,
                               float eps, void* y, int64_t ldy, int out_f32, int64_t rows, int D) {
   ASIS_REQUIRE(x && w && b && y, "asis_layernorm: null pointer");
@@ -272,11 +364,8 @@
   if (rows <= 0) return ASIS_OK;
   hipStream_t s = reinterpret_cast<hipStream_t>(stream);
   dim3 grid((unsigned)asis_cdiv(rows, 4)), block(256);
-  static const int ln_fast = [] {
-    const char* e = getenv("ASIS_LN_FAST");
-    return e ? atoi(e) : 2;
-  }();
-  if (ln_fast && !out_f32 && (D == 768 || D == 1024 || D == 1536) && rows >= 4096) {
+  const int ln_fast = ln_fast_rows();
+  if (!out_f32 && ln_fixed_shape(rows, D)) {
 #define ASIS_LN_FIXED(T, NCH)                                                                                         \
   do {                                                                                                                \
     if (ln_fast == 1)                                                                                                 \
@@ -305,6 +394,61 @@
   return ASIS_OK;
 }
 
+extern "C" int asis_layernorm_pair_ok(int64_t rows, int D) { return ln_fixed_shape(rows, D); }
+
+extern "C" int asis_layernorm_pair(void* stream, int dtype, const float* x, int64_t ldx, const float* w1, const float* b1,
+                                   const float* w2, const float* b2, float eps, void* y1, void* y2, int64_t ldy, int64_t rows, int D) {
+  ASIS_REQUIRE(x && w1 && b1 && w2 && b2 && y1 && y2, "asis_layernorm_pair: null pointer");
+  ASIS_REQUIRE(asis_layernorm_pair_ok(rows, D), "asis_layernorm_pair: not a shape of the fixed-D LayerNorm kernel (rows %ld >= 4096, D %d in 768, 1024, 1536)",
+               (long)rows, D);
+  ASIS_REQUIRE(ldx % 4 == 0 && ldx >= D && ldy % 4 == 0 && ldy >= D, "asis_layernorm_pair: row strides must be multiples of 4 and >= D");
+  ASIS_REQUIRE(asis_aligned16(x) && asis_aligned16(w1) && asis_aligned16(b1) && asis_aligned16(w2) && asis_aligned16(b2) &&
+                   (((uintptr_t)y1) & 7) == 0 && (((uintptr_t)y2) & 7) == 0,
+               "asis_layernorm_pair: pointers must be 16-byte aligned");
+  ASIS_DT_OK(dtype, "asis_layernorm_pair");
+  hipStream_t s = reinterpret_cast<hipStream_t>(stream);
+  const dim3 block(256);
+  const bool one = ln_fast_rows() == 1;
+#define ASIS_LN_PAIR(T, NCH)                                                                                                        \
+  do {                                                                                                                              \
+    if (one)                                                                                                                        \
+      hipLaunchKernelGGL((layernorm_pair_kernel<T, NCH, 1>), dim3((unsigned)asis_cdiv(rows, 4)), block, 0, s, x, ldx, w1, b1, w2,  \
+                         b2, eps, static_cast<T*>(y1), static_cast<T*>(y2), ldy, rows);                                             \
+    else                                                                                                                            \
+      hipLaunchKernelGGL((layernorm_pair_kernel<T, NCH, 2>), dim3((unsigned)asis_cdiv(rows, 8)), block, 0, s, x, ldx, w1, b1, w2,  \
+                         b2, eps, static_cast<T*>(y1), static_cast<T*>(y2), ldy, rows);                                             \
+  } while (0)
+  if (int rc = asis_dispatch16(dtype, "asis_layernorm_pair", [&](auto t) {
+        using T = decltype(t);
+        if (D == 768) ASIS_LN_PAIR(T, 3);
+        else if (D == 1024) ASIS_LN_PAIR(T, 4);
+        else ASIS_LN_PAIR(T, 6);
+      })) return rc;
+#undef ASIS_LN_PAIR
+  ASIS_CHECK_LAUNCH("asis_layernorm_pair");
+  return ASIS_OK;
+}
+
+extern "C" int asis_layernorm_add(void* stream, const float* x, int64_t stride_x, int skip, const float* w, const float* b, float eps,
+                                  const float* a, int64_t stride_a, float* out, int64_t stride_out, float* norm_out,
+                                  int64_t stride_norm, int batch, int n, int D) {
+  ASIS_REQUIRE(x && w && b && a && out, "asis_layernorm_add: null pointer");
+  ASIS_REQUIRE(D > 0 && D % 4 == 0 && D <= 256 * LN_MAXC, "asis_layernorm_add: D=%d must be a multiple of 4 and <= %d", D, 256 * LN_MAXC);
+  ASIS_REQUIRE(batch >= 1 && n >= 1 && skip >= 0, "asis_layernorm_add: bad shape (batch %d, n %d, skip %d)", batch, n, skip);
+  const int64_t nd = (int64_t)n * D, nsd = (int64_t)(n + skip) * D;
+  ASIS_REQUIRE(stride_x % 4 == 0 && stride_a % 4 == 0 && stride_out % 4 == 0 && stride_norm % 4 == 0 &&
+                   (batch == 1 || (stride_x >= nsd && stride_a >= nd && stride_out >= nd && (!norm_out || stride_norm >= nsd))),
+               "asis_layernorm_add: batch strides must be multiples of 4 and cover the rows");
+  ASIS_REQUIRE(asis_aligned16(x) && asis_aligned16(w) && asis_aligned16(b) && asis_aligned16(a) && asis_aligned16(out) &&
+                   (!norm_out || asis_aligned16(norm_out)), "asis_layernorm_add: pointers must be 16-byte aligned");
+  const int64_t off = (int64_t)skip * D;
+  hipLaunchKernelGGL(layernorm_add_kernel, dim3((unsigned)asis_cdiv((int64_t)batch * n, 4)), dim3(256), 0,
+                     reinterpret_cast<hipStream_t>(stream), x + off, stride_x, w, b, eps, a, stride_a, out, stride_out,
+                     norm_out ? norm_out + off : nullptr, stride_norm, batch, n, D);
+  ASIS_CHECK_LAUNCH("asis_layernorm_add");
+  return ASIS_OK;
+}
+
 template <typename T>
 __global__ __launch_bounds__(256) void layernorm_mx_kernel(const float* __restrict__ x, int64_t ldx, const float* __restrict__ w,
                                                            const float* __restrict__ b, float eps, T* __restrict__ y, T* __restrict__ y_mx,
diff --git a/adaptersis_amd/csrc/row_routines.h b/adaptersis_amd/csrc/row_routines.h
--- a/adaptersis_amd/csrc/row_routines.h
+++ b/adaptersis_amd/csrc/row_routines.h
@@ -26,18 +26,22 @@
   }
 };
 
-template <typename T, bool OUT_F32>
+template <typename T, bool OUT_F32, bool ADD = false>
 __device__ __forceinline__ void ln_row(const float* __restrict__ xrow, const float* __restrict__ w, const float* __restrict__ b,
-                                       float eps, void* __restrict__ yrow, int D, int lane) {
+                                       float eps, void* __restrict__ yrow, int D, int lane, const float* __restrict__ arow = nullptr,
+                                       float* __restrict__ sumrow = nullptr) {
+  static_assert(!ADD || OUT_F32, "ln_row: the added form writes float");
   const int nchunk = D >> 2;
   const float4* xr = reinterpret_cast<const float4*>(xrow);
   float4 v[LN_MAXC];
+  float4 av[ADD ? LN_MAXC : 1];
   float s = 0.f;
 #pragma unroll
   for (int i = 0; i < LN_MAXC; ++i) {
     const int c = lane + 64 * i;
     if (c < nchunk) {
       v[i] = xr[c];
+      if constexpr (ADD) av[i] = reinterpret_cast<const float4*>(arow)[c];
       s += (v[i].x + v[i].y) + (v[i].z + v[i].w);
     }
   }
@@ -64,7 +68,10 @@
       const float o2 = (v[i].z - mean) * rstd * ww.z + bb.z;
       const float o3 = (v[i].w - mean) * rstd * ww.w + bb.w;
       if (OUT_F32) {
-        reinterpret_cast<float4*>(yrow)[c] = make_float4(o0, o1, o2, o3);
+        if (!ADD || yrow) reinterpret_cast<float4*>(yrow)[c] = make_float4(o0, o1, o2, o3);
+        if constexpr (ADD)
+          reinterpret_cast<float4*>(sumrow)[c] = make_float4(__fadd_rn(av[i].x, o0), __fadd_rn(av[i].y, o1),
+                                                             __fadd_rn(av[i].z, o2), __fadd_rn(av[i].w, o3));
       } else {
         uint2 p;
         p.x = pack2<T>(o0, o1);
diff --git a/adaptersis_amd/dinov2/layers/blocks.py b/adaptersis_amd/dinov2/layers/blocks.py
--- a/adaptersis_amd/dinov2/layers/blocks.py
+++ b/adaptersis_amd/dinov2/layers/blocks.py
@@ -424,7 +424,7 @@
         D = x2.shape[1]
         return ops.cast_pad(xn32, D, dt), ops.cast_pad(xn32, D, dt, part=1), None
 
-    def _forward_rows_precise(self, x2: torch.Tensor, segs) -> torch.Tensor:
+    def _forward_rows_precise(self, x2: torch.Tensor, segs, out: Optional[torch.Tensor] = None) -> torch.Tensor:
         D = x2.shape[1]
         R = x2.shape[0]
         dt = config.operand_dtype
@@ -488,7 +488,7 @@
             h, h_lo = ops.gelu_split(hpre, dt, split=split_out)
         else:
             h, h_lo = ops.swiglu(hpre, dt, split=True) if split_out else (ops.swiglu(hpre, dt), None)
-        okw = dict(out_f32=True, bias_n=m._f32(k_out + "_b", lin_out.bias), scale_n=g2, res=x1)
+        okw = dict(out_f32=True, bias_n=m._f32(k_out + "_b", lin_out.bias), scale_n=g2, res=x1, out=out)
         if split_out:
             return self._split_lin(m, k_out, lin_out, h, h_lo, **okw)
         return ops.gemm(h, m._w16(k_out, lin_out.weight), **okw)
@@ -505,7 +505,7 @@
         ok = ok and ops.ln_fold_supported(R, Hd, D) and ops.ln_fold_supported(R, D, Hd, producer=True)
         return ok and all(ops.ln_fold_supported(D, (N + 7) // 8 * 8, D, batch=B) for B, N in segs) and D % 64 == 0
 
-    def forward_rows_fold(self, xin, segs, planes_out: bool):
+    def forward_rows_fold(self, xin, segs, planes_out: bool, out: Optional[torch.Tensor] = None):
         dt = config.operand_dtype
         a, m = self.attn, self.mlp
         g1, g2 = self._gammas()
@@ -532,16 +532,18 @@
         h = ops.gemm(x1h, w1, bias_n=b1, act=ops.ACT_GELU, ln=(mr1, cs1, False))
         w2, b2 = m._w16(k_out, lin_out.weight), m._f32(k_out + "_b", lin_out.bias)
         if not planes_out:
-            return ops.gemm(h, w2, out_f32=True, bias_n=b2, scale_n=g2, res16=(x1h, x1l))
+            return ops.gemm(h, w2, out_f32=True, bias_n=b2, scale_n=g2, res16=(x1h, x1l), out=out)
+        if out is not None:
+            raise ValueError("forward_rows_fold: out= is the fp32 output, planes_out leaves the two-plane form")
         x3h = torch.empty((R + 8, D), device=o.device, dtype=dt)[:R]
         x3l = torch.empty((R, D), device=o.device, dtype=dt)
         st3 = torch.empty((R, G, 2), device=o.device, dtype=torch.float32)
         ops.gemm(h, w2, out=x3h, out_lo=x3l, rowstats=st3, bias_n=b2, scale_n=g2, res16=(x1h, x1l))
         return x3h, x3l, ops.ln_stats_finalize(st3, D, self.norm1.eps)
 
-    def forward_rows(self, x2: torch.Tensor, segs) -> torch.Tensor:
+    def forward_rows(self, x2: torch.Tensor, segs, out: Optional[torch.Tensor] = None) -> torch.Tensor:
         if config.precise_level >= 2:
-            return self._forward_rows_precise(x2, segs)
+            return self._forward_rows_precise(x2, segs, out)
         D = x2.shape[1]
         dt = config.operand_dtype
         g1, g2 = self._gammas()
@@ -562,7 +564,8 @@
         else:
             h12 = ops.gemm(xn2, m._w16(k_in, lin_in.weight), out_f32=True, bias_n=m._f32(k_in + "_b", lin_in.bias))
             h = ops.swiglu(h12, dt)
-        return ops.gemm(h, m._w16(k_out, lin_out.weight), out_f32=True, bias_n=m._f32(k_out + "_b", lin_out.bias), scale_n=g2, res=x1)
+        return ops.gemm(h, m._w16(k_out, lin_out.weight), out_f32=True, bias_n=m._f32(k_out + "_b", lin_out.bias), scale_n=g2, res=x1,
+                        out=out)
 
     def forward_train(self, x: torch.Tensor, keep=None):
         B, N, D = x.shape
diff --git a/adaptersis_amd/ops.py b/adaptersis_amd/ops.py
--- a/adaptersis_amd/ops.py
+++ b/adaptersis_amd/ops.py
@@ -350,6 +350,39 @@
     return out
 
 
+def layernorm_pair(x: torch.Tensor, w1: torch.Tensor, b1: torch.Tensor, w2: torch.Tensor, b2: torch.Tensor, eps: float = 1e-6,
+                   out_dtype: torch.dtype = T16_DEFAULT):
+    _dev(x, w1, b1, w2, b2)
+    if x.dtype != torch.float32 or x.dim() != 2 or x.stride(1) != 1:
+        raise ValueError("layernorm_pair: x must be float32 [rows, D] with contiguous columns")
+    R, D = x.shape
+    if not lib().asis_layernorm_pair_ok(R, D):
+        return layernorm(x, w1, b1, eps, out_dtype), layernorm(x, w2, b2, eps, out_dtype)
+    y1 = torch.empty((R, D), device=x.device, dtype=out_dtype)
+    y2 = torch.empty_like(y1)
+    check(lib().asis_layernorm_pair(_stream(), _dt(out_dtype), x.data_ptr(), x.stride(0), _f32c(w1).data_ptr(), _f32c(b1).data_ptr(),
+                                    _f32c(w2).data_ptr(), _f32c(b2).data_ptr(), float(eps), y1.data_ptr(), y2.data_ptr(), D, R, D),
+          "asis_layernorm_pair")
+    return y1, y2
+
+
+def layernorm_add(a: torch.Tensor, x: torch.Tensor, w: torch.Tensor, b: torch.Tensor, eps: float = 1e-6, skip: int = 0,
+                  out: Optional[torch.Tensor] = None, norm_out: Optional[torch.Tensor] = None) -> torch.Tensor:
+    _dev(a, x, w, b, out, norm_out)
+    B, n, D = a.shape
+    if out is None:
+        out = torch.empty((B, n, D), device=a.device, dtype=torch.float32)
+    for t, nm, rows in ((a, "a", n), (out, "out", n), (x, "x", n + skip), (norm_out, "norm_out", n + skip)):
+        if t is not None:
+            _rows3(t, D, "layernorm_add " + nm)
+            if tuple(t.shape) != (B, rows, D):
+                raise ValueError(f"layernorm_add {nm}: expected [{B}, {rows}, {D}], got {tuple(t.shape)}")
+    check(lib().asis_layernorm_add(_stream(), x.data_ptr(), x.stride(0), int(skip), _f32c(w).data_ptr(), _f32c(b).data_ptr(), float(eps),
+                                   a.data_ptr(), a.stride(0), out.data_ptr(), out.stride(0), _p(norm_out),
+                                   norm_out.stride(0) if norm_out is not None else 0, B, n, D), "asis_layernorm_add")
+    return out
+
+
 def layernorm_mx(x: torch.Tensor, w: torch.Tensor, b: torch.Tensor, eps: float, out_dtype: torch.dtype, amax: torch.Tensor):
     _dev(x, w, b, amax)
     if x.dtype != torch.float32 or x.dim() != 2 or x.stride(1) != 1:
diff --git a/include/asis_hip.h b/include/asis_hip.h
--- a/include/asis_hip.h
+++ b/include/asis_hip.h
@@ -81,6 +81,12 @@
                    void* y, int64_t ldy, int out_f32, int64_t rows, int D);
 int asis_layernorm_mx(void* stream, int dtype, const float* x, int64_t ldx, const float* w, const float* b, float eps, void* y,
                       void* y_mx, int64_t ldy, const float* amax, int64_t rows, int D);
+int asis_layernorm_pair_ok(int64_t rows, int D);
+int asis_layernorm_pair(void* stream, int dtype, const float* x, int64_t ldx, const float* w1, const float* b1, const float* w2,
+                        const float* b2, float eps, void* y1, void* y2, int64_t ldy, int64_t rows, int D);
+int asis_layernorm_add(void* stream, const float* x, int64_t stride_x, int skip, const float* w, const float* b, float eps,
+                       const float* a, int64_t stride_a, float* out, int64_t stride_out, float* norm_out, int64_t stride_norm,
+                       int batch, int n, int D);
 
 int asis_attention_fwd(void* stream, int dtype, const void* q, const void* k, int64_t ldqk, const void* vt,
                        int64_t ldvt, void* o, int64_t ldo, int B, int H, int N, float scale);
```

Result: no change. 226.0 img/s, median of 6 (+0.5%).
